# GlaireDaggers/Pretty-Fast-Video

Measured on AMD Instinct MI355X. Metric: macroblocks/s (encode+decode) 1080p YUV420, higher is better.
Workload: dtype i32 (encoder transforms evaluated in exact f32; decoders i32)

## Files before the change

include/pfv_hip_ext.h:

```cpp
#ifndef PFV_HIP_EXT_H
#define PFV_HIP_EXT_H

#include "pfv_hip_core.h"

#ifdef __cplusplus
extern "C" {
#endif

PFV_API int pfv_ctx_create_prio(int device, int priority, pfv_ctx **out);
PFV_API int pfv_ctx_pci_bus_id(pfv_ctx *ctx, char *out, int len);
PFV_API int pfv_device_sync(pfv_ctx *ctx);
PFV_API void *pfv_ctx_stream(pfv_ctx *ctx);

typedef enum pfv_option {
    PFV_OPT_ENC_TRANSFORM = 1, PFV_OPT_TILE_COMPACTION = 2, PFV_OPT_LANE_MAPPING = 3, PFV_OPT_ENTROPY_DECODE = 4,
    PFV_OPT_ENTDEC_LANE_BITS = 5, PFV_OPT_ENTDEC_LAUNCHES = 6, PFV_OPT_ENTDEC_INNER_ROUNDS = 7
} pfv_option;
enum { PFV_ENTROPY_DECODE_AUTO = 0, PFV_ENTROPY_DECODE_HOST = 1, PFV_ENTROPY_DECODE_DEVICE = 2 };
enum { PFV_LANES_AUTO = 0, PFV_LANES_PER_MB_8 = 1, PFV_LANES_PER_MB_16 = 2 };
enum { PFV_ENC_TRANSFORM_AUTO = 0, PFV_ENC_TRANSFORM_INT = 1 };
PFV_API int pfv_ctx_set_option(pfv_ctx *ctx, int option, int value);
PFV_API int pfv_ctx_get_option(pfv_ctx *ctx, int option, int *value);

typedef struct pfv_event pfv_event;
PFV_API int pfv_event_create(pfv_ctx *ctx, pfv_event **out);
PFV_API int pfv_event_record(pfv_event *e);
PFV_API int pfv_event_elapsed_ms(pfv_event *start, pfv_event *stop, float *ms);
PFV_API void pfv_event_destroy(pfv_event *e);
PFV_API int pfv_ctx_wait_event(pfv_ctx *ctx, pfv_event *e);

typedef struct pfv_graph pfv_graph;
PFV_API int pfv_graph_begin(pfv_ctx *ctx);
PFV_API int pfv_graph_end(pfv_ctx *ctx, pfv_graph **out);
PFV_API int pfv_graph_launch(pfv_graph *g);
PFV_API void pfv_graph_destroy(pfv_graph *g);

PFV_API int pfv_blit_dev(pfv_ctx *ctx, uint8_t *dst, int dst_w, int dst_h, const uint8_t *src, int src_w, int src_h,
                         int dx, int dy, int sx, int sy, int sw, int sh);

PFV_API int pfv_reduce_dev(pfv_ctx *ctx, uint8_t *dst, const uint8_t *src, int src_w, int src_h);
PFV_API int pfv_double_dev(pfv_ctx *ctx, uint8_t *dst, const uint8_t *src, int src_w, int src_h);
PFV_API int pfv_rgb_to_yuv420_dev(pfv_ctx *ctx, const uint8_t *rgb_dev, int width, int height, uint8_t *frame_dev);
PFV_API int pfv_yuv420_to_rgb_dev(pfv_ctx *ctx, const uint8_t *frame_dev, int width, int height, uint8_t *rgb_dev);

typedef struct pfv_comm pfv_comm;
enum { PFV_COMM_SUM = 0, PFV_COMM_MAX = 1 };
PFV_API int pfv_comm_unique_id(uint8_t id_out[128]);
PFV_API int pfv_comm_init(pfv_ctx *ctx, int rank, int world, const uint8_t id[128], pfv_comm **out);
PFV_API int pfv_comm_rank(const pfv_comm *c);
PFV_API int pfv_comm_world(const pfv_comm *c);
PFV_API int pfv_comm_broadcast_dev(pfv_comm *c, void *buf_dev, size_t bytes, int root);
PFV_API int pfv_comm_allreduce_f64_dev(pfv_comm *c, double *buf_dev, size_t count, int op);
PFV_API int pfv_comm_allgather_dev(pfv_comm *c, const void *send_dev, void *recv_dev, size_t bytes_per_rank);
PFV_API int pfv_comm_allreduce_f64(pfv_comm *c, double *values, size_t count, int op);
PFV_API int pfv_comm_barrier(pfv_comm *c);
PFV_API void pfv_comm_destroy(pfv_comm *c);

PFV_API int pfv_synth_frames_dev(pfv_ctx *ctx, int width, int height, int n_streams, const uint64_t *seeds, int t,
                                 uint8_t *frames_dev);
enum { PFV_SYNTH_PAN = 0, PFV_SYNTH_LOW_MOTION = 1, PFV_SYNTH_STATIC = 2 };
PFV_API int pfv_synth_frames_kind_dev(pfv_ctx *ctx, int width, int height, int n_streams, const uint64_t *seeds, int t, int kind,
                                      uint8_t *frames_dev);

PFV_API int pfv_dev_alloc(pfv_ctx *ctx, size_t bytes, void **out);
PFV_API int pfv_dev_free(pfv_ctx *ctx, void *p);
PFV_API int pfv_dev_copy(pfv_ctx *ctx, void *dst_dev, const void *src_dev, size_t bytes);
PFV_API int pfv_host_alloc(pfv_ctx *ctx, size_t bytes, void **out);
PFV_API int pfv_host_free(pfv_ctx *ctx, void *p);
PFV_API int pfv_dev_upload(pfv_ctx *ctx, void *dst_dev, const void *src_host, size_t bytes);
PFV_API int pfv_dev_download(pfv_ctx *ctx, void *dst_host, const void *src_dev, size_t bytes);

PFV_API int pfv_enc_iframe_dev(pfv_enc_session *s, const uint8_t *frames_dev, int16_t *coef_dev);
PFV_API int pfv_enc_pframe_dev(pfv_enc_session *s, const uint8_t *frames_dev, int8_t *mv_dev, uint8_t *has_coef_dev,
                               int16_t *coef_dev);
PFV_API int pfv_enc_session_set_frame_stride(pfv_enc_session *s, size_t stride_bytes);
PFV_API int pfv_enc_session_set_window(pfv_enc_session *s, int first, int count);
PFV_API const uint8_t *pfv_enc_prev_frame_dev(pfv_enc_session *s, int stream);

PFV_API size_t pfv_payload_worst_case(int width, int height);
PFV_API int pfv_enc_entropy_enable(pfv_enc_session *s, size_t payload_cap);
PFV_API int pfv_enc_entropy_set_async(pfv_enc_session *s, int on);
PFV_API int pfv_enc_entropy_join(pfv_enc_session *s);
PFV_API int pfv_enc_pack_iframe_dev(pfv_enc_session *s, const int16_t *coef_dev);
PFV_API int pfv_enc_pack_pframe_dev(pfv_enc_session *s, const int8_t *mv_dev, const uint8_t *has_coef_dev,
                                    const int16_t *coef_dev);
PFV_API int pfv_enc_payload_sizes(pfv_enc_session *s, uint32_t *sizes_out);
PFV_API int pfv_enc_payloads_fetch(pfv_enc_session *s, uint8_t *out, size_t cap, uint32_t *sizes_out, uint64_t *offsets_out);
PFV_API const uint8_t *pfv_enc_payload_dev(pfv_enc_session *s, int stream);
PFV_API size_t pfv_enc_payload_capacity(pfv_enc_session *s);
PFV_API int pfv_enc_payload_fetch(pfv_enc_session *s, int stream, uint8_t *out_host, size_t nbytes);
PFV_API int pfv_dec_iframe_dev(pfv_dec_session *s, const int16_t *coef_dev, const uint8_t qidx[3]);
PFV_API int pfv_dec_pframe_dev(pfv_dec_session *s, const int8_t *mv_dev, const uint8_t *has_coef_dev,
                               const int16_t *coef_dev, const uint8_t qidx[3]);
PFV_API int pfv_dec_iframe_sparse(pfv_dec_session *s, const uint32_t *idx, const int16_t *val, size_t n, const uint8_t qidx[3]);
PFV_API int pfv_dec_pframe_sparse(pfv_dec_session *s, const int8_t *mv, const uint8_t *has_coef, const uint32_t *idx,
                                  const int16_t *val, size_t n, const uint8_t qidx[3]);
PFV_API int pfv_dec_iframe_lists_dev(pfv_dec_session *s, const uint32_t *const *entries_dev, const uint32_t *counts_dev, const uint8_t qidx[3]);
PFV_API int pfv_dec_pframe_lists_dev(pfv_dec_session *s, const int8_t *mv_dev, const uint8_t *has_coef_dev, const uint32_t *const *entries_dev,
                                     const uint32_t *counts_dev, const uint8_t qidx[3]);
PFV_API int pfv_coef_lists_from_dense(const int16_t *coef, const uint8_t *has_coef, int total_blocks, uint32_t *entries_out, size_t cap,
                                      uint32_t *counts_out, size_t *n_out);
PFV_API int pfv_dec_get_frame_dev(pfv_dec_session *s, uint8_t *frames_out_dev);
PFV_API int pfv_dec_set_output_dev(pfv_dec_session *s, uint8_t *frames_out_dev);
PFV_API int pfv_dec_set_output_strided_dev(pfv_dec_session *s, uint8_t *frames_out_dev, size_t stride_bytes);
PFV_API int pfv_dec_session_set_window(pfv_dec_session *s, int first, int count);
PFV_API int pfv_encoder_set_device_entropy(pfv_encoder *e, int on);
enum { PFV_FRAME_PACKED = 0, PFV_FRAME_PADDED = 1 };
PFV_API int pfv_frames_sse_dev(pfv_ctx *ctx, int width, int height, int n_streams, const uint8_t *a_dev, int a_layout, size_t a_stride,
                               const uint8_t *b_dev, int b_layout, size_t b_stride, uint64_t *sse_dev, uint32_t *mb_sse_dev);
PFV_API int pfv_frames_sse(pfv_ctx *ctx, int width, int height, int n_streams, const uint8_t *a, const uint8_t *b, uint64_t *sse_out,
                           uint32_t *mb_sse_out);
PFV_API double pfv_psnr(uint64_t sse, uint64_t n_samples);
PFV_API int pfv_enc_distortion_dev(pfv_enc_session *s, const uint8_t *frames_dev, uint64_t *sse_dev, uint32_t *mb_sse_dev);
PFV_API int pfv_dec_distortion_dev(pfv_dec_session *s, const uint8_t *frames_dev, uint64_t *sse_dev, uint32_t *mb_sse_dev);
typedef struct pfv_frame_report {
    int32_t  type;
    uint32_t packet_bytes;
    uint64_t sse[3];
    double   psnr[3];
    double   psnr_yuv;
} pfv_frame_report;
PFV_API int pfv_encoder_set_frame_report(pfv_encoder *e, int on);
PFV_API int pfv_encoder_frame_report(pfv_encoder *e, pfv_frame_report *out);

PFV_API int pfv_frames_ssim_dev(pfv_ctx *ctx, int width, int height, int n_streams, const uint8_t *a_dev, int a_layout, size_t a_stride,
                                const uint8_t *b_dev, int b_layout, size_t b_stride, int64_t *ssim_q24_dev, int32_t *mb_ssim_q24_dev);
PFV_API int pfv_frames_ssim(pfv_ctx *ctx, int width, int height, int n_streams, const uint8_t *a, const uint8_t *b, int64_t *ssim_q24_out,
                            int32_t *mb_out);
PFV_API int pfv_ssim_windows(int width, int height, uint32_t out[3]);
PFV_API double pfv_ssim(int64_t q24_sum, uint64_t windows);
PFV_API int pfv_enc_ssim_dev(pfv_enc_session *s, const uint8_t *frames_dev, int64_t *ssim_q24_dev, int32_t *mb_dev);
PFV_API int pfv_dec_ssim_dev(pfv_dec_session *s, const uint8_t *frames_dev, int64_t *ssim_q24_dev, int32_t *mb_dev);
typedef struct pfv_frame_ssim {
    int64_t  q24[3];
    uint32_t windows[3];
    double   ssim[3];
    double   ssim_all;
} pfv_frame_ssim;
PFV_API int pfv_encoder_set_frame_ssim(pfv_encoder *e, int on);
PFV_API int pfv_encoder_frame_ssim(pfv_encoder *e, pfv_frame_ssim *out);

PFV_API int pfv_deblock_strength(const int32_t qtable[64]);
PFV_API int pfv_frames_deblock_dev(pfv_ctx *ctx, int width, int height, int n_streams, const uint8_t *src_dev, int src_layout, size_t src_stride,
                                   uint8_t *dst_dev, size_t dst_stride, const uint8_t strength[3]);
PFV_API int pfv_frames_deblock(pfv_ctx *ctx, int width, int height, int n_streams, const uint8_t *src, uint8_t *dst, const uint8_t strength[3]);
enum { PFV_DEBLOCK_OFF = 0, PFV_DEBLOCK_AUTO = 1, PFV_DEBLOCK_FIXED = 2 };
PFV_API int pfv_dec_set_deblock(pfv_dec_session *s, int mode, const uint8_t strength[3]);
PFV_API int pfv_decoder_set_deblock(pfv_decoder *d, int mode, const uint8_t strength[3]);

enum { PFV_PIX_RGB8 = 0, PFV_PIX_RGBA8 = 1, PFV_PIX_BGRA8 = 2 };
PFV_API size_t pfv_rgb_row_bytes(int width, int format);
PFV_API int pfv_frames_to_rgb_dev(pfv_ctx *ctx, int width, int height, int n_streams, const uint8_t *src_dev, int src_layout, size_t src_stride,
                                  uint8_t *dst_dev, int format, size_t dst_pitch, size_t dst_stride);
PFV_API int pfv_frames_to_rgb(pfv_ctx *ctx, int width, int height, int n_streams, const uint8_t *src, uint8_t *dst, int format);
PFV_API int pfv_dec_get_frame_rgb_dev(pfv_dec_session *s, uint8_t *dst_dev, int format, size_t pitch, size_t stride);
PFV_API int pfv_dec_get_frame_rgb(pfv_dec_session *s, uint8_t *dst_host, int format);
PFV_API int pfv_dec_set_output_rgb_dev(pfv_dec_session *s, uint8_t *dst_dev, int format, size_t pitch, size_t stride);
PFV_API int pfv_decoder_set_output_rgb(pfv_decoder *d, int on, int format);

enum { PFV_CHROMA_POINT = 0, PFV_CHROMA_BOX = 1 };
PFV_API int pfv_frames_from_rgb_dev(pfv_ctx *ctx, int width, int height, int n_streams, const uint8_t *src_dev, int format, size_t src_pitch,
                                    size_t src_stride, uint8_t *dst_dev, size_t dst_stride, int chroma);
PFV_API int pfv_frames_from_rgb(pfv_ctx *ctx, int width, int height, int n_streams, const uint8_t *src, uint8_t *dst, int format, int chroma);
PFV_API int pfv_enc_ingest_rgb_dev(pfv_enc_session *s, const uint8_t *pictures_dev, int format, size_t pitch, size_t stride, int chroma,
                                   const uint8_t **frames_dev_out);
PFV_API int pfv_encoder_set_input_rgb(pfv_encoder *e, int on, int format, int chroma);

enum { PFV_SCALE_BILINEAR = 0, PFV_SCALE_BICUBIC = 1, PFV_SCALE_LANCZOS3 = 2 };
typedef struct pfv_scaler pfv_scaler;
PFV_API int pfv_scale_taps(int kind, int n_src, int n_dst);
PFV_API int pfv_scale_table(int kind, int n_src, int n_dst, int32_t *first, int16_t *coef);
PFV_API pfv_scaler *pfv_scaler_create(pfv_ctx *ctx, int sw, int sh, int dw, int dh, int kind, int *err);
PFV_API void pfv_scaler_destroy(pfv_scaler *sc);
PFV_API int pfv_scaler_run_dev(pfv_scaler *sc, int n_streams, const uint8_t *src_dev, int src_layout, size_t src_stride, uint8_t *dst_dev,
                               size_t dst_stride);
PFV_API int pfv_frames_scale(pfv_ctx *ctx, int sw, int sh, int dw, int dh, int n_streams, const uint8_t *src, uint8_t *dst, int kind);
PFV_API int pfv_dec_set_output_scaled_dev(pfv_dec_session *s, pfv_scaler *sc, uint8_t *dst_dev, size_t stride);
PFV_API int pfv_decoder_set_output_size(pfv_decoder *d, int w, int h, int kind);
PFV_API int pfv_enc_scale_dev(pfv_enc_session *s, pfv_scaler *sc, const uint8_t *frames_dev, size_t src_stride, const uint8_t **frames_dev_out);
PFV_API int pfv_encoder_set_input_size(pfv_encoder *e, int src_w, int src_h, int kind);

typedef struct pfv_denoiser pfv_denoiser;
PFV_API pfv_denoiser *pfv_denoiser_create(pfv_ctx *ctx, int width, int height, int n_streams, int *err);
PFV_API void pfv_denoiser_destroy(pfv_denoiser *dn);
PFV_API int pfv_denoiser_set_strength(pfv_denoiser *dn, const uint8_t spatial[3], const uint8_t temporal[3]);
PFV_API int pfv_denoiser_reset(pfv_denoiser *dn, int first_stream, int n);
PFV_API int pfv_denoiser_run_dev(pfv_denoiser *dn, int first_stream, int n, const uint8_t *src_dev, int src_layout, size_t src_stride, uint8_t *dst_dev,
                                 size_t dst_stride, int commit);
// ... 160 lines not shown
```

pretty-fast-video_amd/_lib.py:

```python
from __future__ import annotations

import ctypes
import os
from ctypes import POINTER, c_char_p, c_float, c_int, c_size_t, c_uint8, c_void_p

_HERE = os.path.dirname(os.path.abspath(__file__))
DEFAULT_LIB = os.path.join(_HERE, "libpfv_hip.so")

PFV_OK = 0
PFV_ERR_BAD_ARG = -1
PFV_ERR_HIP = -2
PFV_ERR_NOMEM = -3
PFV_ERR_BAD_MV = -4
PFV_ERR_NO_DEVICE = -5
PFV_ERR_FORMAT = -6
PFV_ERR_VERSION = -7
PFV_ERR_IO = -8
PFV_ERR_STATE = -9

PFV_COMM_SUM, PFV_COMM_MAX = 0, 1
PFV_OPT_ENC_TRANSFORM = 1
PFV_OPT_TILE_COMPACTION = 2
PFV_OPT_LANE_MAPPING = 3
PFV_LANES_AUTO, PFV_LANES_PER_MB_8, PFV_LANES_PER_MB_16 = 0, 1, 2
PFV_OPT_ENTROPY_DECODE = 4
PFV_OPT_ENTDEC_LANE_BITS, PFV_OPT_ENTDEC_LAUNCHES, PFV_OPT_ENTDEC_INNER_ROUNDS = 5, 6, 7
PFV_ENTROPY_DECODE_AUTO, PFV_ENTROPY_DECODE_HOST, PFV_ENTROPY_DECODE_DEVICE = 0, 1, 2
PFV_ENC_TRANSFORM_AUTO, PFV_ENC_TRANSFORM_INT = 0, 1
PFV_FRAME_PACKED, PFV_FRAME_PADDED = 0, 1
PFV_DEBLOCK_OFF, PFV_DEBLOCK_AUTO, PFV_DEBLOCK_FIXED = 0, 1, 2
PFV_PIX_RGB8, PFV_PIX_RGBA8, PFV_PIX_BGRA8 = 0, 1, 2
PFV_CHROMA_POINT, PFV_CHROMA_BOX = 0, 1
PFV_SCALE_BILINEAR, PFV_SCALE_BICUBIC, PFV_SCALE_LANCZOS3 = 0, 1, 2
PFV_SEARCH_FOURSTEP, PFV_SEARCH_FULL, PFV_SEARCH_HIER = 0, 1, 2


SEARCH_MODES = {"fourstep": PFV_SEARCH_FOURSTEP, "full": PFV_SEARCH_FULL, "hier": PFV_SEARCH_HIER}


def search_mode(mode) -> int:
    return SEARCH_MODES[mode] if isinstance(mode, str) else int(mode)


class PfvError(RuntimeError):
    def __init__(self, code: int, msg: str):
        super().__init__(f"pfv_hip error {code}: {msg}")
        self.code = code


_P = c_void_p
SIGNATURES = [
    ("pfv_device_count", c_int, []),
    ("pfv_ctx_create", c_int, [c_int, POINTER(_P)]),
    ("pfv_ctx_create_prio", c_int, [c_int, c_int, POINTER(_P)]),
    ("pfv_ctx_destroy", None, [_P]),
    ("pfv_ctx_pci_bus_id", c_int, [_P, _P, c_int]),
    ("pfv_ctx_sync", c_int, [_P]),
    ("pfv_device_sync", c_int, [_P]),
    ("pfv_ctx_stream", _P, [_P]),
    ("pfv_last_error", c_char_p, [_P]),
    ("pfv_version", c_char_p, []),
    ("pfv_ctx_set_option", c_int, [_P, c_int, c_int]),
    ("pfv_ctx_get_option", c_int, [_P, c_int, POINTER(c_int)]),
    ("pfv_event_create", c_int, [_P, POINTER(_P)]),
    ("pfv_event_record", c_int, [_P]),
    ("pfv_event_elapsed_ms", c_int, [_P, _P, POINTER(c_float)]),
    ("pfv_event_destroy", None, [_P]),
    ("pfv_ctx_wait_event", c_int, [_P, _P]),
    ("pfv_graph_begin", c_int, [_P]),
    ("pfv_graph_end", c_int, [_P, POINTER(_P)]),
    ("pfv_graph_launch", c_int, [_P]),
    ("pfv_graph_destroy", None, [_P]),
    ("pfv_pad16", c_int, [c_int]),
    ("pfv_qtables_from_quality", c_int, [c_int, _P, _P, _P, _P, POINTER(c_float)]),
    ("pfv_encode_plane", c_int, [_P, _P, c_int, c_int, _P, c_uint8, _P]),
    ("pfv_encode_plane_delta", c_int, [_P, _P, c_int, c_int, _P, _P, c_float, c_uint8, _P, _P, _P]),
    ("pfv_decode_plane_into", c_int, [_P, _P, c_int, c_int, _P, _P]),
    ("pfv_decode_plane_delta", c_int, [_P, _P, _P, _P, c_int, c_int, _P, _P, _P]),
    ("pfv_decode_plane_delta_into", c_int, [_P, _P, _P, _P, c_int, c_int, _P, _P]),
    ("pfv_blit_dev", c_int, [_P, _P, c_int, c_int, _P, c_int, c_int, c_int, c_int, c_int, c_int, c_int, c_int]),
    ("pfv_reduce_dev", c_int, [_P, _P, _P, c_int, c_int]),
    ("pfv_double_dev", c_int, [_P, _P, _P, c_int, c_int]),
    ("pfv_rgb_to_yuv420_dev", c_int, [_P, _P, c_int, c_int, _P]),
    ("pfv_yuv420_to_rgb_dev", c_int, [_P, _P, c_int, c_int, _P]),
    ("pfv_comm_unique_id", c_int, [_P]),
    ("pfv_comm_init", c_int, [_P, c_int, c_int, _P, POINTER(_P)]),
    ("pfv_comm_rank", c_int, [_P]),
    ("pfv_comm_world", c_int, [_P]),
    ("pfv_comm_broadcast_dev", c_int, [_P, _P, c_size_t, c_int]),
    ("pfv_comm_allreduce_f64_dev", c_int, [_P, _P, c_size_t, c_int]),
    ("pfv_comm_allgather_dev", c_int, [_P, _P, _P, c_size_t]),
    ("pfv_comm_allreduce_f64", c_int, [_P, _P, c_size_t, c_int]),
    ("pfv_comm_barrier", c_int, [_P]),
    ("pfv_comm_destroy", None, [_P]),
    ("pfv_synth_frames_dev", c_int, [_P, c_int, c_int, c_int, _P, c_int, _P]),
    ("pfv_synth_frames_kind_dev", c_int, [_P, c_int, c_int, c_int, _P, c_int, c_int, _P]),
    ("pfv_dev_alloc", c_int, [_P, c_size_t, POINTER(_P)]),
    ("pfv_dev_copy", c_int, [_P, _P, _P, c_size_t]),
    ("pfv_dev_free", c_int, [_P, _P]),
    ("pfv_host_alloc", c_int, [_P, c_size_t, POINTER(_P)]),
    ("pfv_host_free", c_int, [_P, _P]),
    ("pfv_dev_upload", c_int, [_P, _P, _P, c_size_t]),
    ("pfv_dev_download", c_int, [_P, _P, _P, c_size_t]),
    ("pfv_frame_bytes", c_size_t, [c_int, c_int]),
    ("pfv_padded_frame_bytes", c_size_t, [c_int, c_int]),
    ("pfv_total_blocks", c_int, [c_int, c_int]),
    ("pfv_enc_session_create", c_int, [_P, c_int, c_int, c_int, c_int, POINTER(_P)]),
    ("pfv_enc_session_destroy", None, [_P]),
    ("pfv_enc_iframe_dev", c_int, [_P, _P, _P]),
    ("pfv_enc_pframe_dev", c_int, [_P, _P, _P, _P, _P]),
    ("pfv_enc_iframe", c_int, [_P, _P, _P]),
    ("pfv_enc_pframe", c_int, [_P, _P, _P, _P, _P]),
    ("pfv_enc_session_set_frame_stride", c_int, [_P, c_size_t]),
    ("pfv_enc_session_set_window", c_int, [_P, c_int, c_int]),
    ("pfv_enc_prev_frame_dev", _P, [_P, c_int]),
    ("pfv_enc_prev_frame", c_int, [_P, _P]),
    ("pfv_payload_worst_case", c_size_t, [c_int, c_int]),
    ("pfv_enc_entropy_enable", c_int, [_P, c_size_t]),
    ("pfv_enc_entropy_set_async", c_int, [_P, c_int]),
    ("pfv_enc_entropy_join", c_int, [_P]),
    ("pfv_enc_pack_iframe_dev", c_int, [_P, _P]),
    ("pfv_enc_pack_pframe_dev", c_int, [_P, _P, _P, _P]),
    ("pfv_enc_payload_sizes", c_int, [_P, _P]),
    ("pfv_enc_payloads_fetch", c_int, [_P, _P, c_size_t, _P, _P]),
    ("pfv_enc_payload_dev", _P, [_P, c_int]),
    ("pfv_enc_payload_capacity", c_size_t, [_P]),
    ("pfv_enc_payload_fetch", c_int, [_P, c_int, _P, c_size_t]),
    ("pfv_dec_iframe_sparse", c_int, [_P, _P, _P, c_size_t, _P]),
    ("pfv_dec_pframe_sparse", c_int, [_P, _P, _P, _P, _P, c_size_t, _P]),
    ("pfv_dec_iframe_lists_dev", c_int, [_P, _P, _P, _P]),
    ("pfv_dec_pframe_lists_dev", c_int, [_P, _P, _P, _P, _P, _P]),
    ("pfv_coef_lists_from_dense", c_int, [_P, _P, c_int, _P, c_size_t, _P, POINTER(c_size_t)]),
    ("pfv_dec_session_create", c_int, [_P, c_int, c_int, _P, c_int, c_int, POINTER(_P)]),
    ("pfv_dec_session_destroy", None, [_P]),
    ("pfv_dec_iframe_dev", c_int, [_P, _P, _P]),
    ("pfv_dec_pframe_dev", c_int, [_P, _P, _P, _P, _P]),
    ("pfv_dec_iframe", c_int, [_P, _P, _P]),
    ("pfv_dec_pframe", c_int, [_P, _P, _P, _P, _P]),
    ("pfv_dec_get_frame_dev", c_int, [_P, _P]),
    ("pfv_dec_set_output_dev", c_int, [_P, _P]),
    ("pfv_dec_set_output_strided_dev", c_int, [_P, _P, c_size_t]),
    ("pfv_dec_session_set_window", c_int, [_P, c_int, c_int]),
    ("pfv_dec_get_frame", c_int, [_P, _P]),
    ("pfv_dec_framebuffer", c_int, [_P, _P]),
    ("pfv_dec_check", c_int, [_P]),
    ("pfv_encoder_create", c_int, [_P, c_int, c_int, c_int, c_int, POINTER(_P)]),
    ("pfv_encoder_encode_iframe", c_int, [_P, _P, _P, _P]),
    ("pfv_encoder_encode_pframe", c_int, [_P, _P, _P, _P]),
    ("pfv_encoder_encode_dropframe", c_int, [_P]),
    ("pfv_encoder_finish", c_int, [_P]),
    ("pfv_encoder_bytes", c_int, [_P, POINTER(_P), POINTER(c_size_t)]),
    ("pfv_encoder_drain", c_int, [_P, POINTER(_P), POINTER(c_size_t)]),
    ("pfv_encoder_destroy", None, [_P]),
    ("pfv_encoder_set_device_entropy", c_int, [_P, c_int]),
    ("pfv_frames_sse_dev", c_int, [_P, c_int, c_int, c_int, _P, c_int, c_size_t, _P, c_int, c_size_t, _P, _P]),
    ("pfv_frames_sse", c_int, [_P, c_int, c_int, c_int, _P, _P, _P, _P]),
    ("pfv_psnr", ctypes.c_double, [ctypes.c_uint64, ctypes.c_uint64]),
    ("pfv_enc_distortion_dev", c_int, [_P, _P, _P, _P]),
    ("pfv_dec_distortion_dev", c_int, [_P, _P, _P, _P]),
    ("pfv_encoder_set_frame_report", c_int, [_P, c_int]),
    ("pfv_encoder_frame_report", c_int, [_P, _P]),
    ("pfv_frames_ssim_dev", c_int, [_P, c_int, c_int, c_int, _P, c_int, c_size_t, _P, c_int, c_size_t, _P, _P]),
    ("pfv_frames_ssim", c_int, [_P, c_int, c_int, c_int, _P, _P, _P, _P]),
    ("pfv_ssim_windows", c_int, [c_int, c_int, _P]),
    ("pfv_ssim", ctypes.c_double, [ctypes.c_int64, ctypes.c_uint64]),
    ("pfv_enc_ssim_dev", c_int, [_P, _P, _P, _P]),
    ("pfv_dec_ssim_dev", c_int, [_P, _P, _P, _P]),
    ("pfv_encoder_set_frame_ssim", c_int, [_P, c_int]),
    ("pfv_encoder_frame_ssim", c_int, [_P, _P]),
    ("pfv_deblock_strength", c_int, [_P]),
    ("pfv_frames_deblock_dev", c_int, [_P, c_int, c_int, c_int, _P, c_int, c_size_t, _P, c_size_t, _P]),
    ("pfv_frames_deblock", c_int, [_P, c_int, c_int, c_int, _P, _P, _P]),
    ("pfv_dec_set_deblock", c_int, [_P, c_int, _P]),
    ("pfv_decoder_set_deblock", c_int, [_P, c_int, _P]),
    ("pfv_rgb_row_bytes", c_size_t, [c_int, c_int]),
    ("pfv_frames_to_rgb_dev", c_int, [_P, c_int, c_int, c_int, _P, c_int, c_size_t, _P, c_int, c_size_t, c_size_t]),
    ("pfv_frames_to_rgb", c_int, [_P, c_int, c_int, c_int, _P, _P, c_int]),
    ("pfv_dec_get_frame_rgb_dev", c_int, [_P, _P, c_int, c_size_t, c_size_t]),
    ("pfv_dec_get_frame_rgb", c_int, [_P, _P, c_int]),
    ("pfv_dec_set_output_rgb_dev", c_int, [_P, _P, c_int, c_size_t, c_size_t]),
    ("pfv_decoder_set_output_rgb", c_int, [_P, c_int, c_int]),
    ("pfv_frames_from_rgb_dev", c_int, [_P, c_int, c_int, c_int, _P, c_int, c_size_t, c_size_t, _P, c_size_t, c_int]),
    ("pfv_frames_from_rgb", c_int, [_P, c_int, c_int, c_int, _P, _P, c_int, c_int]),
    ("pfv_enc_ingest_rgb_dev", c_int, [_P, _P, c_int, c_size_t, c_size_t, c_int, _P]),
    ("pfv_encoder_set_input_rgb", c_int, [_P, c_int, c_int, c_int]),
    ("pfv_scale_taps", c_int, [c_int, c_int, c_int]),
    ("pfv_scale_table", c_int, [c_int, c_int, c_int, _P, _P]),
    ("pfv_scaler_create", _P, [_P, c_int, c_int, c_int, c_int, c_int, POINTER(c_int)]),
    ("pfv_scaler_destroy", None, [_P]),
    ("pfv_scaler_run_dev", c_int, [_P, c_int, _P, c_int, c_size_t, _P, c_size_t]),
    ("pfv_frames_scale", c_int, [_P, c_int, c_int, c_int, c_int, c_int, _P, _P, c_int]),
    ("pfv_dec_set_output_scaled_dev", c_int, [_P, _P, _P, c_size_t]),
    ("pfv_decoder_set_output_size", c_int, [_P, c_int, c_int, c_int]),
    ("pfv_enc_scale_dev", c_int, [_P, _P, _P, c_size_t, _P]),
    ("pfv_encoder_set_input_size", c_int, [_P, c_int, c_int, c_int]),
    ("pfv_denoiser_create", _P, [_P, c_int, c_int, c_int, POINTER(c_int)]),
    ("pfv_denoiser_destroy", None, [_P]),
    ("pfv_denoiser_set_strength", c_int, [_P, _P, _P]),
    ("pfv_denoiser_reset", c_int, [_P, c_int, c_int]),
    ("pfv_denoiser_run_dev", c_int, [_P, c_int, c_int, _P, c_int, c_size_t, _P, c_size_t, c_int]),
    ("pfv_frames_denoise", c_int, [_P, c_int, c_int, c_int, c_int, _P, _P, _P, _P]),
    ("pfv_enc_denoise_dev", c_int, [_P, _P, _P, c_size_t, c_int, _P]),
    ("pfv_encoder_set_denoise", c_int, [_P, c_int, _P, _P]),
    ("pfv_scene_score_q8", ctypes.c_uint32, [_P]),
    ("pfv_scene_plan", c_int, [_P, c_int, ctypes.c_uint32, c_int, c_int, _P]),
    ("pfv_scene_detector_create", _P, [_P, c_int, c_int, c_int, c_int, POINTER(c_int)]),
    ("pfv_scene_detector_destroy", None, [_P]),
    ("pfv_scene_detector_set_radius", c_int, [_P, c_int]),
    ("pfv_scene_detector_reset", c_int, [_P, c_int, c_int]),
    ("pfv_scene_detector_run_dev", c_int, [_P, c_int, c_int, _P, c_int, c_size_t, c_int, _P]),
    ("pfv_scene_detector_run_clip_dev", c_int, [_P, c_int, c_int, _P, c_int, c_size_t, c_int, _P]),
    ("pfv_scene_detector_maps", c_int, [_P, c_int, c_int, _P, _P]),
    ("pfv_scene_detector_run_timed_dev", c_int, [_P, c_int, c_int, c_int, _P, c_int, c_size_t, _P, _P]),
    ("pfv_frames_scene", c_int, [_P, c_int, c_int, c_int, c_int, _P, c_int, _P]),
    ("pfv_encoder_set_scene_cut", c_int, [_P, c_int, ctypes.c_uint32, c_int, c_int]),
    ("pfv_encoder_last_scene", c_int, [_P, _P]),
    ("pfv_enc_session_create_ladder", c_int, [_P, c_int, c_int, _P, c_int, c_int, POINTER(_P)]),
    ("pfv_enc_session_set_motion_search", c_int, [_P, c_int, c_int]),
    ("pfv_enc_session_get_motion_search", c_int, [_P, _P, _P]),
    ("pfv_encoder_set_motion_search", c_int, [_P, c_int, c_int]),
    ("pfv_enc_session_coarse_vectors", c_int, [_P, _P, c_size_t]),
    ("pfv_enc_pframe_hier_timed_dev", c_int, [_P, _P, _P, _P, _P, _P]),
    ("pfv_enc_session_set_rung", c_int, [_P, c_int]),
    ("pfv_enc_session_rung", c_int, [_P]),
    ("pfv_enc_session_rungs", c_int, [_P]),
# ... 121 lines not shown
```

pretty-fast-video_amd/csrc/pfv_context.hip:

```cpp
constexpr int kCtxScratch = 9;
struct pfv_ctx {
    int device = 0;
    hipStream_t stream = nullptr;
    std::string err;
    void *scratch[kCtxScratch] = {};
    size_t scratch_cap[kCtxScratch] = {};
    QTab *qtab_dev = nullptr;
    QTab *qtab_host = nullptr;
    int *flag_dev = nullptr;
    int n_cus = 256;
    bool capturing = false;
    int opt_enc_transform = PFV_ENC_TRANSFORM_AUTO;
    int opt_tile_compaction = 1;
    int opt_lane_mapping = PFV_LANES_AUTO;
    int opt_entropy_decode = PFV_ENTROPY_DECODE_AUTO;
    int opt_entdec_lane_bits = (int)kEdSubBits, opt_entdec_launches = 3, opt_entdec_inner = kEdInner;
    std::vector<struct pfv_comm *> comms;
    std::mutex comms_m;
    pfv_ctx *owner = nullptr;
    std::vector<pfv_ctx *> children;
    int priority = 0;
};
static int ctx_create_child(pfv_ctx *user, pfv_ctx **out)
{
    int rc = pfv_ctx_create_prio(user->device, user->priority, out);
    if (rc) return rc;
    (*out)->owner = user;
    std::lock_guard<std::mutex> lk(user->comms_m);
    user->children.push_back(*out);
    return PFV_OK;
}
static void comm_teardown(struct pfv_comm *c);

static thread_local std::string g_tls_err;

static int fail(pfv_ctx *ctx, int code, const std::string &msg)
{
    if (ctx) ctx->err = msg;
    if (ctx && ctx->owner) ctx->owner->err = msg;
    g_tls_err = msg;
    return code;
}
static int hip_fail(pfv_ctx *ctx, hipError_t e, const char *what)
{
    (void)hipGetLastError();
    return fail(ctx, e == hipErrorOutOfMemory ? PFV_ERR_NOMEM : PFV_ERR_HIP,
                std::string(what) + ": " + hipGetErrorString(e));
}
#define HIP_TRY(ctx, expr)                                        \
    do {                                                          \
        hipError_t e__ = (expr);                                  \
        if (e__ != hipSuccess) return hip_fail(ctx, e__, #expr);  \
    } while (0)

static inline int pad16(int x) { return x + (16 - (x % 16)) % 16; }

extern "C" {

#ifndef PFV_BUILD_ID
#define PFV_BUILD_ID "unstamped"
#endif
PFV_API const char *pfv_version(void) { return "pfv-hip 0.2 (gfx950; pfv-rs 0.2.2 / codec 2.1.1 hot path; src " PFV_BUILD_ID ")"; }
PFV_API int pfv_pad16(int x) { return pad16(x); }

PFV_API const char *pfv_last_error(pfv_ctx *ctx) { return ctx ? ctx->err.c_str() : g_tls_err.c_str(); }

PFV_API int pfv_ctx_set_option(pfv_ctx *ctx, int option, int value)
{
    if (!ctx) return fail(nullptr, PFV_ERR_BAD_ARG, "null ctx");
    switch (option) {
    case PFV_OPT_ENC_TRANSFORM:
        if (value != PFV_ENC_TRANSFORM_AUTO && value != PFV_ENC_TRANSFORM_INT) return fail(ctx, PFV_ERR_BAD_ARG, "PFV_OPT_ENC_TRANSFORM: unknown value");
        ctx->opt_enc_transform = value;
        return PFV_OK;
    case PFV_OPT_TILE_COMPACTION:
        if (value < 0 || value > 2) return fail(ctx, PFV_ERR_BAD_ARG, "PFV_OPT_TILE_COMPACTION: 0, 1 or 2");
        ctx->opt_tile_compaction = value;
        return PFV_OK;
    case PFV_OPT_LANE_MAPPING:
        if (value != PFV_LANES_AUTO && value != PFV_LANES_PER_MB_8 && value != PFV_LANES_PER_MB_16) return fail(ctx, PFV_ERR_BAD_ARG, "PFV_OPT_LANE_MAPPING: unknown value");
        ctx->opt_lane_mapping = value;
        return PFV_OK;
    case PFV_OPT_ENTROPY_DECODE:
        if (value != PFV_ENTROPY_DECODE_AUTO && value != PFV_ENTROPY_DECODE_HOST && value != PFV_ENTROPY_DECODE_DEVICE) return fail(ctx, PFV_ERR_BAD_ARG, "PFV_OPT_ENTROPY_DECODE: unknown value");
        ctx->opt_entropy_decode = value;
        return PFV_OK;
    case PFV_OPT_ENTDEC_LANE_BITS:
        if (value < 32 || value > (int)kEdMaxSubBits || value % 32) return fail(ctx, PFV_ERR_BAD_ARG, "PFV_OPT_ENTDEC_LANE_BITS: a multiple of 32 in 32..256");
        ctx->opt_entdec_lane_bits = value;
        return PFV_OK;
    case PFV_OPT_ENTDEC_LAUNCHES:
        if (value < 1 || value > 64) return fail(ctx, PFV_ERR_BAD_ARG, "PFV_OPT_ENTDEC_LAUNCHES: 1..64");
        ctx->opt_entdec_launches = value;
        return PFV_OK;
    case PFV_OPT_ENTDEC_INNER_ROUNDS:
        if (value < 1 || value > 1024) return fail(ctx, PFV_ERR_BAD_ARG, "PFV_OPT_ENTDEC_INNER_ROUNDS: 1..1024");
        ctx->opt_entdec_inner = value;
        return PFV_OK;
    default:
        return fail(ctx, PFV_ERR_BAD_ARG, "pfv_ctx_set_option: unknown option");
    }
}
PFV_API int pfv_ctx_get_option(pfv_ctx *ctx, int option, int *value)
{
    if (!ctx || !value) return fail(ctx, PFV_ERR_BAD_ARG, "pfv_ctx_get_option: bad argument");
    switch (option) {
    case PFV_OPT_ENC_TRANSFORM: *value = ctx->opt_enc_transform; return PFV_OK;
    case PFV_OPT_TILE_COMPACTION: *value = ctx->opt_tile_compaction; return PFV_OK;
    case PFV_OPT_LANE_MAPPING: *value = ctx->opt_lane_mapping; return PFV_OK;
    case PFV_OPT_ENTROPY_DECODE: *value = ctx->opt_entropy_decode; return PFV_OK;
    case PFV_OPT_ENTDEC_LANE_BITS: *value = ctx->opt_entdec_lane_bits; return PFV_OK;
    case PFV_OPT_ENTDEC_LAUNCHES: *value = ctx->opt_entdec_launches; return PFV_OK;
    case PFV_OPT_ENTDEC_INNER_ROUNDS: *value = ctx->opt_entdec_inner; return PFV_OK;
    default: return fail(ctx, PFV_ERR_BAD_ARG, "pfv_ctx_get_option: unknown option");
    }
}

PFV_API int pfv_device_count(void)
{
    int n = 0;
    if (hipGetDeviceCount(&n) != hipSuccess) { (void)hipGetLastError(); return 0; }
    return n;
}

PFV_API int pfv_ctx_create(int device, pfv_ctx **out) { return pfv_ctx_create_prio(device, 0, out); }

PFV_API int pfv_ctx_create_prio(int device, int priority, pfv_ctx **out)
{
    if (!out) return fail(nullptr, PFV_ERR_BAD_ARG, "pfv_ctx_create: out is null");
    *out = nullptr;
    int n = 0;
    hipError_t e = hipGetDeviceCount(&n);
    if (e != hipSuccess || n <= 0) {
        (void)hipGetLastError();
        return fail(nullptr, PFV_ERR_NO_DEVICE, "pfv_ctx_create: no HIP device visible (the HIP path has no CPU fallback)");
    }
    if (device < 0 || device >= n) return fail(nullptr, PFV_ERR_BAD_ARG, "pfv_ctx_create: device ordinal out of range");
    HIP_TRY(nullptr, hipSetDevice(device));
    pfv_ctx *ctx = new pfv_ctx();
    ctx->device = device;
    ctx->priority = priority;
    {
        int cus = 0;
        if (hipDeviceGetAttribute(&cus, hipDeviceAttributeMultiprocessorCount, device) == hipSuccess && cus > 0) ctx->n_cus = cus;
    }
    if (priority == 0) {
        e = hipStreamCreateWithFlags(&ctx->stream, hipStreamNonBlocking);
    } else {
        int least = 0, greatest = 0;
        e = hipDeviceGetStreamPriorityRange(&least, &greatest);
        if (e == hipSuccess) e = hipStreamCreateWithPriority(&ctx->stream, hipStreamNonBlocking, priority > 0 ? greatest : least);
    }
    if (e == hipSuccess) e = hipMalloc((void **)&ctx->qtab_dev, 4 * sizeof(QTab));
    if (e == hipSuccess) e = hipHostMalloc((void **)&ctx->qtab_host, 4 * sizeof(QTab), hipHostMallocDefault);
    if (e == hipSuccess) e = hipMalloc((void **)&ctx->flag_dev, sizeof(int));
    if (e == hipSuccess) e = hipMemsetAsync(ctx->flag_dev, 0, sizeof(int), ctx->stream);
    if (e != hipSuccess) {
        int rc = hip_fail(nullptr, e, "pfv_ctx_create");
        pfv_ctx_destroy(ctx);
        return rc;
    }
    *out = ctx;
    return PFV_OK;
}

PFV_API void pfv_ctx_destroy(pfv_ctx *ctx)
{
    if (!ctx) return;
    (void)hipSetDevice(ctx->device);
    if (ctx->stream) (void)hipStreamSynchronize(ctx->stream);
    {
        std::vector<pfv_comm *> live;
        { std::lock_guard<std::mutex> lk(ctx->comms_m); live.swap(ctx->comms); }
        for (pfv_comm *c : live) comm_teardown(c);
    }
    {
        std::lock_guard<std::mutex> lk(ctx->comms_m);
        for (pfv_ctx *c : ctx->children) c->owner = nullptr;
        ctx->children.clear();
    }
    if (ctx->owner) {
        std::lock_guard<std::mutex> lk(ctx->owner->comms_m);
        auto &v = ctx->owner->children;
        v.erase(std::remove(v.begin(), v.end(), ctx), v.end());
    }
    for (int i = 0; i < kCtxScratch; i++)
        if (ctx->scratch[i]) (void)hipFree(ctx->scratch[i]);
    if (ctx->qtab_dev) (void)hipFree(ctx->qtab_dev);
    if (ctx->qtab_host) (void)hipHostFree(ctx->qtab_host);
    if (ctx->flag_dev) (void)hipFree(ctx->flag_dev);
// ... 136 lines not shown
```

pretty-fast-video_amd/csrc/pfv_kernels.hip:

```cpp
#include <hip/hip_runtime.h>
#include <stdint.h>

#include "pfv_device.h"
#include "pfv_prof.h"


namespace pfv {

namespace {
__constant__ int kScale[64] = {
    32, 37, 34, 26, 32, 26, 34, 37, 37, 43, 39, 31, 37, 31, 39, 43, 34, 39, 35, 28, 34, 28, 35, 39, 26, 31, 28, 22, 26, 22,
    28, 31, 32, 37, 34, 26, 32, 26, 34, 37, 26, 31, 28, 22, 26, 22, 28, 31, 34, 39, 35, 28, 34, 28, 35, 39, 37, 43, 39, 31,
    37, 31, 39, 43,
};
__constant__ int kInvZigzag[64] = {
    0,  1,  5,  6,  14, 15, 27, 28, 2,  4,  7,  13, 16, 26, 29, 42, 3,  8,  12, 17, 25, 30, 41, 43, 9,  11, 18, 24, 31, 40,
    44, 53, 10, 19, 23, 32, 39, 45, 52, 54, 20, 22, 33, 38, 46, 51, 55, 60, 21, 34, 37, 47, 50, 56, 59, 61, 35, 36, 48, 49,
    57, 58, 62, 63,
};
}

constexpr int kWinRows = 16 * kStripsPerWG + 30;
constexpr int kWinStride = 176;
constexpr int kWinBytes = kWinRows * kWinStride;
// ... 306 lines not shown
        int ch = j * 64 + lane;
        int mb = half_strip * 4 + (ch >> 5);
        if (mb < n_mb) st_stream(&reinterpret_cast<uint4 *>(coef_mb0)[half_strip * 128 + ch], reinterpret_cast<const uint4 *>(stage)[stage_chunk(ch)]);
    }
}
__device__ __forceinline__ void fetch_coef_quads(uint4 (&buf)[2], const int16_t *coef_mb0, int n_mb, int lane, int half_strip)
{
#pragma unroll
    for (int j = 0; j < 2; j++) {
        int ch = j * 64 + lane;
        int mb = half_strip * 4 + (ch >> 5);
        buf[j] = make_uint4(0, 0, 0, 0);
        if (mb < n_mb) buf[j] = ld_stream(&reinterpret_cast<const uint4 *>(coef_mb0)[half_strip * 128 + ch]);
    }
}
__device__ __forceinline__ void stage_coef_half(int *stage, const uint4 (&buf)[2], int lane)
{
#pragma unroll
    for (int j = 0; j < 2; j++) reinterpret_cast<uint4 *>(stage)[stage_chunk(j * 64 + lane)] = buf[j];
}

struct ListSpan {
    const uint32_t *ent;
    uint32_t lo, hi;
    uint32_t e0, e1;
};
__device__ __forceinline__ ListSpan list_span(const uint32_t *ent, uint32_t begin, uint32_t end, int last_lane, int lane)
{
    ListSpan sp{ent, 0u, 0u, 0u, 0u};
    sp.lo = (uint32_t)__builtin_amdgcn_readlane((int)begin, 0);
    sp.hi = (uint32_t)__builtin_amdgcn_readlane((int)end, last_lane);
    if (sp.hi < sp.lo) sp.hi = sp.lo;
    const uint32_t k = sp.lo + (uint32_t)lane;
    if (k < sp.hi) sp.e0 = ent[k];
    if (k + 64u < sp.hi) sp.e1 = ent[k + 64u];
    return sp;
}
template <int LPM>
__device__ __forceinline__ void stage_list_put(int16_t *stage, uint32_t e, int mb_low, int h)
{
    const int pos = (int)(e & 255u), mbl = (int)(((e >> 8) - (uint32_t)mb_low) & 255u);
    if (LPM == 8) {
        if ((pos >> 7) == h && mbl < kStripMB) stage[mbl * (2 * kStagePitch) + (pos & 127)] = (int16_t)(e >> 16);
    } else {
        if (mbl < kStripMB / 2) stage[(mbl * 2 + (pos >> 7)) * (2 * kStagePitch) + (pos & 127)] = (int16_t)(e >> 16);
    }
}
template <int LPM>
__device__ __forceinline__ void stage_list_half(int *xw, const ListSpan &sp, int lane, int mb_low, int h)
{
#pragma unroll
    for (int j = 0; j < 2; j++) reinterpret_cast<uint4 *>(xw)[stage_chunk(j * 64 + lane)] = make_uint4(0, 0, 0, 0);
    wave_lds_sync();
    int16_t *stage = reinterpret_cast<int16_t *>(xw);
    const uint32_t k = sp.lo + (uint32_t)lane;
    if (k < sp.hi) stage_list_put<LPM>(stage, sp.e0, mb_low, h);
    if (k + 64u < sp.hi) stage_list_put<LPM>(stage, sp.e1, mb_low, h);
    for (uint32_t j = k + 128u; j < sp.hi; j += 64u) stage_list_put<LPM>(stage, sp.ent[j], mb_low, h);
}

__device__ __forceinline__ void forward_half(int (&v)[2][8], int *xw, int m, int i, const LaneQ &lq, bool keep)
{
    const int keepmask = keep ? -1 : 0;
    int *mb = xw + m * kMBPitch;
    fdct8(v[0]);
    fdct8(v[1]);
    rows_to_cols2(v, mb, i, m & 3);
    fdct8(v[0]);
    fdct8(v[1]);
    int16_t *stage = reinterpret_cast<int16_t *>(xw) + m * (2 * kStagePitch);
#pragma unroll
    for (int k = 0; k < 8; k++) {
        const int scale = lq.scale(k), zz = lq.zz(k);
        const float rcp = lq.rcp(k);
#pragma unroll
        for (int s = 0; s < 2; s++) {
            int n = wmul24(v[s][k], scale) >> 16;
            v[s][k] = (int)((float)n * rcp) & keepmask;
            stage[s * 64 + zz] = (int16_t)v[s][k];
        }
    }
    wave_lds_sync();
}
__device__ __forceinline__ void inverse_half(int (&v)[2][8], int *xw, int m, int i, const LaneQ &lq)
{
    int *mb = xw + m * kMBPitch;
#pragma unroll
    for (int k = 0; k < 8; k++) {
        const int deq = lq.deq(k);
        v[0][k] = wmul24(v[0][k], deq);
        v[1][k] = wmul24(v[1][k], deq);
    }
    idct8(v[0]);
    idct8(v[1]);
    cols_to_rows2(v, mb, i, m & 3);
#pragma unroll
    for (int s = 0; s < 2; s++) {
        idct8(v[s]);
#pragma unroll
        for (int k = 0; k < 8; k++) v[s][k] = min(v[s][k] >> 8, 127);
    }
}
__device__ __forceinline__ void gather_half(int (&v)[2][8], const int *xw, int m, const LaneQ &lq)
{
    const int16_t *stage = reinterpret_cast<const int16_t *>(xw) + m * (2 * kStagePitch);
#pragma unroll
    for (int k = 0; k < 8; k++) {
        const int zz = lq.zz(k);
        v[0][k] = (int)stage[zz];
        v[1][k] = (int)stage[64 + zz];
    }
    wave_lds_sync();
}

typedef float f2 __attribute__((vector_size(8)));
__device__ __forceinline__ f2 f2s(float x) { return f2{x, x}; }
__device__ __forceinline__ f2 f2trunc(f2 x) { return f2{__builtin_truncf(x[0]), __builtin_truncf(x[1])}; }
__device__ __forceinline__ f2 f2floor(f2 x) { return f2{__builtin_floorf(x[0]), __builtin_floorf(x[1])}; }

__device__ __forceinline__ void ffdct8(f2 (&v)[8])
{
    const f2 a0 = v[0] + v[7], a1 = v[1] + v[6], a2 = v[2] + v[5], a3 = v[3] + v[4];
    const f2 a4 = v[0] - v[7], a5 = v[1] - v[6], a6 = v[2] - v[5], a7 = v[3] - v[4];
    const f2 b0 = a0 + a3, b1 = a1 + a2, b2 = a0 - a3, b3 = a1 - a2;
    const f2 c0 = b0 + b1, c1 = b0 - b1;
    const f2 c2 = b2 * f2s(1.25f) + b3 * f2s(0.5f);
    const f2 c3 = b2 * f2s(0.5f) - b3 * f2s(1.25f);
    const f2 b4 = a4 * f2s(1.1875f) + a7 * f2s(0.25f);
    const f2 b7 = a4 * f2s(0.25f) - a7 * f2s(1.1875f);
    const f2 b5 = a5 + a6 * f2s(0.6875f);
    const f2 b6 = a6 - a5 * f2s(0.6875f);
    const f2 c4 = b4 + b5, c5 = b4 - b5, c6 = b6 + b7, c7 = b6 - b7;
    v[0] = c0; v[1] = c4; v[2] = c2; v[3] = c5 - c7;
    v[4] = c1; v[5] = c5 + c7; v[6] = c3; v[7] = c6;
}
__device__ __forceinline__ void fidct8(f2 (&v)[8])
{
    const f2 c0 = v[0], d4 = v[1], c2 = v[2], d6 = v[3], c1 = v[4], d5 = v[5], c3 = v[6], d7 = v[7];
    const f2 c5 = d5 + d6, c7 = d5 - d6;
    const f2 b4 = d4 + c5, b5 = d4 - c5, b6 = d7 + c7, b7 = d7 - c7;
    const f2 b0 = c0 + c1, b1 = c0 - c1;
    const f2 half = f2s(0.5f), quarter = f2s(0.25f);
    const f2 c2h = f2trunc(c2 * half), c2q = f2trunc(c2h * half), c3h = f2trunc(c3 * half), c3q = f2trunc(c3h * half);
    const f2 b4q = f2trunc(b4 * quarter), b4s = f2trunc(b4q * quarter), b5q = f2trunc(b5 * quarter), b5s = f2trunc(b5q * quarter);
    const f2 b6q = f2trunc(b6 * quarter), b6s = f2trunc(b6q * quarter), b7q = f2trunc(b7 * quarter), b7s = f2trunc(b7q * quarter);
    const f2 b2 = c2 + c2q + c3h, b3 = c2h - c3 - c3q;
    const f2 a4 = b7q + b4 + b4q - b4s;
    const f2 a7 = b4q - b7 - b7q + b7s;
    const f2 a5 = b5 - b6 + b6q + b6s;
    const f2 a6 = b6 + b5 - b5q - b5s;
    const f2 a0 = b0 + b2, a1 = b1 + b3, a2 = b1 - b3, a3 = b0 - b2;
    v[0] = a0 + a4; v[1] = a1 + a5; v[2] = a2 + a6; v[3] = a3 + a7;
    v[4] = a3 - a7; v[5] = a2 - a6; v[6] = a1 - a5; v[7] = a0 - a4;
}
__device__ __forceinline__ int f_chunk(int p, int j) { return j ^ ((p >> 1) & 3); }
__device__ __forceinline__ void f_rows_to_cols(f2 (&x)[8], int *mb, int i, int mx)
{
    {
        const int p = i ^ mx;
        float4 *row = reinterpret_cast<float4 *>(mb + p * 16);
#pragma unroll
        for (int j = 0; j < 4; j++) row[f_chunk(p, j)] = make_float4(x[2 * j][0], x[2 * j][1], x[2 * j + 1][0], x[2 * j + 1][1]);
    }
    wave_lds_sync();
#pragma unroll
    for (int r = 0; r < 8; r++) {
        const int p = r ^ mx;
        x[r] = *reinterpret_cast<const f2 *>(mb + p * 16 + f_chunk(p, i >> 1) * 4 + (i & 1) * 2);
    }
    wave_lds_sync();
}
__device__ __forceinline__ void f_cols_to_rows(f2 (&x)[8], int *mb, int i, int mx)
{
#pragma unroll
    for (int r = 0; r < 8; r++) {
        const int p = r ^ mx;
        *reinterpret_cast<f2 *>(mb + p * 16 + f_chunk(p, i >> 1) * 4 + (i & 1) * 2) = x[r];
    }
    wave_lds_sync();
    {
        const int p = i ^ mx;
        const float4 *row = reinterpret_cast<const float4 *>(mb + p * 16);
#pragma unroll
        for (int j = 0; j < 4; j++) {
            const float4 c = row[f_chunk(p, j)];
            x[2 * j] = f2{c.x, c.y};
            x[2 * j + 1] = f2{c.z, c.w};
        }
    }
    wave_lds_sync();
}
__device__ __forceinline__ f2 quant_scale(f2 m, int scale16)
{
    f2 n;
#pragma unroll
    for (int s = 0; s < 2; s++) n[s] = (float)mulhi24((int)m[s], scale16);
    return n;
}
constexpr float kQuantMagic = 12582912.0f;
__device__ __forceinline__ f2 quant_div(f2 n, float rcp, float magic, f2 &biased)
{
    const f2 q = f2trunc(n * f2s(rcp));
    biased = q + f2s(magic);
    return q;
}
__device__ __forceinline__ f2 quant_pair_f(f2 m, int scale16, float rcp, float magic, f2 &biased)
{
    return quant_div(quant_scale(m, scale16), rcp, magic, biased);
}
__device__ __forceinline__ f2 residual_f(f2 src, f2 pred)
{
    const f2 d = src - pred;
    const float c = 0.5f - 1.0f / 2048.0f;
    const f2 r = f2{__builtin_fmaf(d[0], c, kQuantMagic), __builtin_fmaf(d[1], c, kQuantMagic)};
    return f2{__builtin_fmaf(r[0], 256.0f, -256.0f * kQuantMagic), __builtin_fmaf(r[1], 256.0f, -256.0f * kQuantMagic)};
}
__device__ __forceinline__ int16_t quant_low16(float biased) { return (int16_t)__float_as_int(biased); }
__device__ __forceinline__ void forward_half_f(f2 (&x)[8], int *xw, int m, int i, const LaneQ &lq, float magic)
{
    int *mb = xw + m * kMBPitch;
    ffdct8(x);
    f_rows_to_cols(x, mb, i, m & 3);
    ffdct8(x);
    int16_t *stage = reinterpret_cast<int16_t *>(xw) + m * (2 * kStagePitch);
#pragma unroll
    for (int k = 0; k < 8; k++) {
        const int zz = lq.zz(k);
        f2 biased;
        x[k] = quant_pair_f(x[k], lq.scale(k), lq.rcp(k), magic, biased);
#pragma unroll
        for (int s = 0; s < 2; s++) stage[s * 64 + zz] = quant_low16(biased[s]);
    }
    wave_lds_sync();
}
constexpr float kPixelBias = 127.501953125f;
__device__ __forceinline__ f2 iframe_pixel_f(f2 x) { return x * f2s(1.0f / 256.0f) + f2s(kPixelBias); }
template <bool PIXEL>
__device__ __forceinline__ void inverse_half_f(f2 (&c)[8], int *xw, int m, int i, const LaneQ &lq)
{
    int *mb = xw + m * kMBPitch;
#pragma unroll
    for (int k = 0; k < 8; k++) c[k] = c[k] * f2s(lq.deqf(k));
    fidct8(c);
    f_cols_to_rows(c, mb, i, m & 3);
    fidct8(c);
#pragma unroll
    for (int k = 0; k < 8; k++) c[k] = PIXEL ? iframe_pixel_f(c[k]) : f2floor(c[k] * f2s(1.0f / 256.0f));
}
__device__ __forceinline__ uint4 pack_row_f(const f2 (&px)[8])
{
    unsigned w[4] = {0, 0, 0, 0};
#pragma unroll
    for (int k = 0; k < 8; k++) {
        w[k >> 2] = __builtin_amdgcn_cvt_pk_u8_f32(px[k][0], (unsigned)(k & 3), w[k >> 2]);
        w[2 + (k >> 2)] = __builtin_amdgcn_cvt_pk_u8_f32(px[k][1], (unsigned)(k & 3), w[2 + (k >> 2)]);
    }
    return make_uint4(w[0], w[1], w[2], w[3]);
}
__device__ __forceinline__ void unpack_row_f(const uint4 &row, f2 (&px)[8])
{
#pragma unroll
    for (int k = 0; k < 4; k++) {
        px[k] = f2{(float)byte_of(row.x, k), (float)byte_of(row.z, k)};
        px[k + 4] = f2{(float)byte_of(row.y, k), (float)byte_of(row.w, k)};
    }
}

template <bool FLT, int LPM = 8>
__global__ __launch_bounds__(kThreads) void k_enc_iframe(FrameGeom g, const uint8_t *__restrict__ src,
                                                          int16_t *__restrict__ coef, uint8_t *__restrict__ recon,
                                                          const QTab *__restrict__ qtabs, float qmagic)
{
    __shared__ __attribute__((aligned(16))) int xchg[kStripsPerWG][kXchgDwords];
    __shared__ __attribute__((aligned(16))) int qtab_lds[kStripsPerWG][kQTabDwords];
    constexpr int kPasses = LPM == 8 ? 2 : 1;

    const int lane = threadIdx.x & 63, wave = __builtin_amdgcn_readfirstlane((int)(threadIdx.x >> 6));
    const int gw = xcd_remap((int)blockIdx.x, (int)gridDim.x) * kStripsPerWG + wave;
    const int gstrip = LPM == 8 ? gw : gw >> 1, half_strip = LPM == 8 ? 0 : gw & 1;
    if (gstrip >= g.strips_per_frame * g.n_streams) return;
    const StripPos sp = locate_strip(g, gstrip);
    if (half_strip * 4 >= sp.n_mb) return;
    const PlaneGeom &p = g.p[sp.plane];
    const int slot = lane >> 3, i = lane & 7;
    const int m = LPM == 8 ? slot : half_strip * 4 + (slot >> 1);
    int *xw = xchg[wave];

    fill_qtable<true, FLT>(qtab_lds[wave], qtabs + p.qsel, lane);
    const uint8_t *plane = frame_src(g, src, sp.stream) + p.src_off;
    uint4 rows[kPasses];
#pragma unroll
    for (int pass = 0; pass < kPasses; pass++) rows[pass] = load_src16(plane, p, sp.x0 + m * 16, sp.y0 + i + 8 * (LPM == 8 ? pass : (slot & 1)));

    wave_lds_sync();
    const LaneQ lq{qtab_lds[wave], i};
    int16_t *coef_mb0 = coef + ((long)sp.stream * g.mbs_per_frame + sp.mb_first) * 256;
    uint8_t *dst = recon ? recon + (long)sp.stream * g.pad_frame_bytes + p.pad_off + (long)(sp.y0 + i) * p.pw + sp.x0 + m * 16
                         : nullptr;
#pragma unroll
    for (int pass = 0; pass < kPasses; pass++) {
        const int h = LPM == 8 ? pass : (slot & 1);
        if (FLT) {
            f2 x[8];
            unpack_row_f(rows[pass], x);
#pragma unroll
            for (int k = 0; k < 8; k++) x[k] = x[k] * f2s(256.0f) - f2s(32768.0f);
            forward_half_f(x, xw, slot, i, lq, qmagic);
            if (LPM == 8) store_coef_half(xw, coef_mb0, sp.n_mb, lane, h);
            else store_coef_quads(xw, coef_mb0, sp.n_mb, lane, half_strip);
            wave_lds_sync();
            if (recon) {
                inverse_half_f<true>(x, xw, slot, i, lq);
                if (m < sp.n_mb) *reinterpret_cast<uint4 *>(dst + (long)(8 * h) * p.pw) = pack_row_f(x);
            }
        } else {
            int v[2][8];
            unpack_row(rows[pass], v);
#pragma unroll
            for (int s = 0; s < 2; s++) {
#pragma unroll
                for (int k = 0; k < 8; k++) v[s][k] = (int)((unsigned)(v[s][k] - 128) << 8);
            }
            forward_half(v, xw, slot, i, lq, true);
            if (LPM == 8) store_coef_half(xw, coef_mb0, sp.n_mb, lane, h);
            else store_coef_quads(xw, coef_mb0, sp.n_mb, lane, half_strip);
            wave_lds_sync();
            if (recon) {
                inverse_half(v, xw, slot, i, lq);
#pragma unroll
                for (int s = 0; s < 2; s++)
#pragma unroll
                    for (int k = 0; k < 8; k++) v[s][k] = min(max(v[s][k] + 128, 0), 255);
                if (m < sp.n_mb) *reinterpret_cast<uint4 *>(dst + (long)(8 * h) * p.pw) = pack_row(v);
            }
        }
    }
}

struct SearchState {
    int cx, cy;
    int err;
};

__device__ __forceinline__ unsigned dot_ab(const uint4 &a, unsigned b0, unsigned b1, unsigned b2, unsigned b3, unsigned acc)
{
    acc = __builtin_amdgcn_udot4(a.x, b0, acc, false);
    acc = __builtin_amdgcn_udot4(a.y, b1, acc, false);
    acc = __builtin_amdgcn_udot4(a.z, b2, acc, false);
// ... 228 lines not shown
                                             int lane)
{
    const int q0 = win_first_issue(wave), q1 = win_first_issue(wave + 1);
#pragma unroll 5
    for (int q = q0; q < q1; q++) {
        const int c = q * 64 + lane;
        const int row = c / kWinChunksPerRow, col = c - row * kWinChunksPerRow;
        const int y = min(max(t.winy0 + row, 0), p.ph - 1), x = min(max(t.winx0 + col * 16, 0), p.pw - 16);
        __builtin_amdgcn_global_load_lds((gbl_cvoid_t *)(refp + (long)y * p.pw + x), (lds_void_t *)(winbuf + c * 16), 16, 0, 0);
    }
}

struct SearchOut {
    int cx, cy;
    int err;
    bool coded;
    uint4 patch[2];
};

template <bool DPPRED = false>
__device__ __forceinline__ void penc_search(const FrameGeom &g, const TilePos &tp, const uint8_t *win, int *red, const uint4 (&rows)[2], int lane,
                                            float min_err, int neg2, SearchOut &so)
{
    const StripPos &sp = tp.sp;
    const PlaneGeom &p = g.p[sp.plane];
    const int m = lane >> 3, i = lane & 7;
    const bool mb_valid = m < sp.n_mb;
    const int mbx = sp.x0 + m * 16, mby = sp.y0;
    const int wcol0 = mbx - tp.winx0;
    const int wrow0 = mby - tp.winy0 + i;

    unsigned s2 = 0;
#pragma unroll
    for (int h = 0; h < 2; h++) {
        s2 = __builtin_amdgcn_udot4(rows[h].x, rows[h].x, s2, false);
        s2 = __builtin_amdgcn_udot4(rows[h].y, rows[h].y, s2, false);
        s2 = __builtin_amdgcn_udot4(rows[h].z, rows[h].z, s2, false);
        s2 = __builtin_amdgcn_udot4(rows[h].w, rows[h].w, s2, false);
    }
    const int a2 = mb_sum((int)s2);

    SearchState st;
    st.cx = 0; st.cy = 0; st.err = 0;
    const SearchLane sl = make_search_lane(red, m, i, neg2);
    const bool interior = sp.x0 >= 16 && sp.x0 + kStripMB * 16 + 16 <= p.pw && sp.y0 >= 16 && sp.y0 + 32 <= p.ph;
    if (interior) {
        search_level<8, true, false, DPPRED>(win, wrow0, wcol0, rows[0], rows[1], a2, mbx, mby, p.pw, p.ph, st, sl);
        KMARK(3);
        search_level<4, false, false, DPPRED>(win, wrow0, wcol0, rows[0], rows[1], a2, mbx, mby, p.pw, p.ph, st, sl);
        KMARK(4);
        search_level<2, false, false, DPPRED>(win, wrow0, wcol0, rows[0], rows[1], a2, mbx, mby, p.pw, p.ph, st, sl);
        KMARK(5);
        search_level<1, false, false, DPPRED>(win, wrow0, wcol0, rows[0], rows[1], a2, mbx, mby, p.pw, p.ph, st, sl);
        KMARK(6);
    } else {
        search_level<8, true, true, DPPRED>(win, wrow0, wcol0, rows[0], rows[1], a2, mbx, mby, p.pw, p.ph, st, sl);
        search_level<4, false, true, DPPRED>(win, wrow0, wcol0, rows[0], rows[1], a2, mbx, mby, p.pw, p.ph, st, sl);
        search_level<2, false, true, DPPRED>(win, wrow0, wcol0, rows[0], rows[1], a2, mbx, mby, p.pw, p.ph, st, sl);
        search_level<1, false, true, DPPRED>(win, wrow0, wcol0, rows[0], rows[1], a2, mbx, mby, p.pw, p.ph, st, sl);
    }

    so.coded = mb_valid && !((float)st.err <= min_err);
    so.cx = st.cx; so.cy = st.cy;
    so.err = st.err;

    const int wx = wcol0 + st.cx, shp = wx & 3;
    const uint8_t *rp = win + (wrow0 + st.cy) * kWinStride + (wx & ~3);
#pragma unroll
    for (int h = 0; h < 2; h++) {
        const unsigned *d = reinterpret_cast<const unsigned *>(rp + 8 * h * kWinStride);
        unsigned d0 = d[0], d1 = d[1], d2 = d[2], d3 = d[3], d4 = d[4];
        so.patch[h] = make_uint4(__builtin_amdgcn_alignbyte(d1, d0, shp), __builtin_amdgcn_alignbyte(d2, d1, shp),
                                 __builtin_amdgcn_alignbyte(d3, d2, shp), __builtin_amdgcn_alignbyte(d4, d3, shp));
    }
}

__device__ __forceinline__ void opaque_row(uint4 &r)
{
#ifndef PFV_HIPEMU
    asm volatile("" : "+v"(r.x), "+v"(r.y), "+v"(r.z), "+v"(r.w));
#else
    (void)r;
#endif
}
template <bool FLT, bool REUNPACK = false, class Store>
__device__ __forceinline__ uint4 penc_half(const uint4 &srow, const uint4 &prow, int *xw, int m, int i, const LaneQ &lq, float qmagic, bool want_recon,
                                           Store &&store)
{
    uint4 out = prow;
    if (FLT) {
        f2 x[8], pp[8];
        unpack_row_f(srow, x);
        unpack_row_f(prow, pp);
#pragma unroll
        for (int k = 0; k < 8; k++) x[k] = residual_f(x[k], pp[k]);
        forward_half_f(x, xw, m, i, lq, qmagic);
        store();
        wave_lds_sync();
        if (want_recon) {
            inverse_half_f<false>(x, xw, m, i, lq);
            if (REUNPACK) {
                uint4 again = prow;
                opaque_row(again);
                unpack_row_f(again, pp);
            }
#pragma unroll
            for (int k = 0; k < 8; k++) {
                const f2 t = f2{__builtin_fminf(x[k][0], 127.0f), __builtin_fminf(x[k][1], 127.0f)};
                pp[k] = pp[k] + t * f2s(2.0f);
            }
            out = pack_row_f(pp);
        }
    } else {
        int v[2][8], pp[2][8];
        unpack_row(srow, v);
        unpack_row(prow, pp);
#pragma unroll
        for (int s = 0; s < 2; s++) {
#pragma unroll
            for (int k = 0; k < 8; k++) {
                int d = v[s][k] - pp[s][k];
                v[s][k] = (int)((unsigned)tdiv2(d) << 8);
            }
        }
        forward_half(v, xw, m, i, lq, true);
        store();
        wave_lds_sync();
        if (want_recon) {
            inverse_half(v, xw, m, i, lq);
#pragma unroll
            for (int s = 0; s < 2; s++) {
#pragma unroll
                for (int k = 0; k < 8; k++)
                    pp[s][k] = min(max(pp[s][k] + 2 * v[s][k], 0), 255);
            }
            out = pack_row(pp);
        }
    }
    return out;
}

__device__ __forceinline__ void penc_store_skipped(int16_t *coef_mb, uint8_t *dst, long pw, int i, const uint4 (&patch)[2])
{
#pragma unroll
    for (int j = 0; j < 4; j++) st_stream(&reinterpret_cast<uint4 *>(coef_mb)[j * 8 + i], make_uint4(0, 0, 0, 0));
    if (dst) {
        *reinterpret_cast<uint4 *>(dst) = patch[0];
        *reinterpret_cast<uint4 *>(dst + 8 * pw) = patch[1];
    }
}

template <bool FLT>
__device__ __forceinline__ void penc_transform(const FrameGeom &g, const TilePos &tp, const SearchOut &so, const uint4 (&rows)[2], int *xw,
                                               int lane, int16_t *__restrict__ coef, uint8_t *__restrict__ recon, const int *qtab_lds, float qmagic)
{
    const StripPos &sp = tp.sp;
    const PlaneGeom &p = g.p[sp.plane];
    const int m = lane >> 3, i = lane & 7;
    const bool mb_valid = m < sp.n_mb, coded = so.coded;
    const int mbx = sp.x0 + m * 16;
    int16_t *coef_mb0 = coef + ((long)sp.stream * g.mbs_per_frame + sp.mb_first) * 256;
    uint8_t *dst = recon ? recon + (long)sp.stream * g.pad_frame_bytes + p.pad_off + (long)(sp.y0 + i) * p.pw + mbx : nullptr;

    if (__any(coded)) {
        const LaneQ lq{qtab_lds, i};
#pragma unroll
// ... 411 lines not shown
    __shared__ __attribute__((aligned(16))) uint8_t win_lds[16 + kWinAlloc];
    __shared__ __attribute__((aligned(16))) int red_lds[kWaves16][kRedDwords];
    __shared__ __attribute__((aligned(16))) int qtab_lds[kQTabDwords];
    uint8_t *win = win_lds + 16;

    const int lane = threadIdx.x & 63, wave = __builtin_amdgcn_readfirstlane((int)(threadIdx.x >> 6));
    const int strip = wave >> 1, half_strip = wave & 1;
    const int slot = lane >> 3, i = lane & 7, mb = lane >> 4, r = lane & 15;
    const int m = half_strip * 4 + mb;
    const int vt = xcd_remap((int)blockIdx.x, (int)gridDim.x);
    const TilePos cur = locate_tile(g, vt, strip);
    const PlaneGeom &p = g.p[cur.sp.plane];
    if (wave == 0) fill_qtable<true, FLT>(qtab_lds, qtabs + p.qsel, lane);
    {
        const uint8_t *refp = ref + (long)cur.sp.stream * g.pad_frame_bytes + p.pad_off;
        for (int q = win_first_issue16(wave); q < win_first_issue16(wave + 1); q++) {
            const int c = q * 64 + lane;
            const int row = c / kWinChunksPerRow, col = c - row * kWinChunksPerRow;
            const int y = min(max(cur.winy0 + row, 0), p.ph - 1), x = min(max(cur.winx0 + col * 16, 0), p.pw - 16);
            __builtin_amdgcn_global_load_lds((gbl_cvoid_t *)(refp + (long)y * p.pw + x), (lds_void_t *)(win + c * 16), 16, 0, 0);
        }
    }
    const bool wave_valid = cur.wave_valid && half_strip * 4 < cur.sp.n_mb;
    const bool mb_valid = wave_valid && m < cur.sp.n_mb;
    uint4 row = make_uint4(0, 0, 0, 0);
    if (wave_valid) row = load_src16(frame_src(g, src, cur.sp.stream) + p.src_off, p, cur.sp.x0 + m * 16, cur.sp.y0 + r);
    __syncthreads();
    int cx = 0, cy = 0;
    bool coded = false;
    uint4 patch = make_uint4(0, 0, 0, 0);
    if (wave_valid) {
        const int mbx = cur.sp.x0 + m * 16, mby = cur.sp.y0;
        const int wcol0 = mbx - cur.winx0, wrow0 = mby - cur.winy0 + r;
        unsigned s2 = __builtin_amdgcn_udot4(row.w, row.w, __builtin_amdgcn_udot4(row.z, row.z, __builtin_amdgcn_udot4(row.y, row.y, __builtin_amdgcn_udot4(row.x, row.x, 0, false), false), false), false);
        const int a2 = mb_sum16((int)s2);
        SearchState st;
        st.cx = 0; st.cy = 0; st.err = 0;
        const SearchLane16 sl = make_search_lane16(red_lds[wave], mb, r, neg2);
        const int hx0 = cur.sp.x0 + half_strip * 64;
        const bool interior = hx0 >= 16 && hx0 + 64 + 16 <= p.pw && cur.sp.y0 >= 16 && cur.sp.y0 + 32 <= p.ph;
        if (interior) {
            search_level16<8, true, false>(win, wrow0, wcol0, row, a2, mbx, mby, p.pw, p.ph, st, sl);
            search_level16<4, false, false>(win, wrow0, wcol0, row, a2, mbx, mby, p.pw, p.ph, st, sl);
            search_level16<2, false, false>(win, wrow0, wcol0, row, a2, mbx, mby, p.pw, p.ph, st, sl);
            search_level16<1, false, false>(win, wrow0, wcol0, row, a2, mbx, mby, p.pw, p.ph, st, sl);
        } else {
            search_level16<8, true, true>(win, wrow0, wcol0, row, a2, mbx, mby, p.pw, p.ph, st, sl);
            search_level16<4, false, true>(win, wrow0, wcol0, row, a2, mbx, mby, p.pw, p.ph, st, sl);
            search_level16<2, false, true>(win, wrow0, wcol0, row, a2, mbx, mby, p.pw, p.ph, st, sl);
            search_level16<1, false, true>(win, wrow0, wcol0, row, a2, mbx, mby, p.pw, p.ph, st, sl);
        }
        coded = mb_valid && !((float)st.err <= min_err);
        cx = st.cx; cy = st.cy;
        const int wx = wcol0 + cx, shp = wx & 3;
        const unsigned *d = reinterpret_cast<const unsigned *>(win + (wrow0 + cy) * kWinStride + (wx & ~3));
        const unsigned d0 = d[0], d1 = d[1], d2 = d[2], d3 = d[3], d4 = d[4];
        patch = make_uint4(__builtin_amdgcn_alignbyte(d1, d0, shp), __builtin_amdgcn_alignbyte(d2, d1, shp), __builtin_amdgcn_alignbyte(d3, d2, shp),
                           __builtin_amdgcn_alignbyte(d4, d3, shp));
    }
    const long mbi = (long)cur.sp.stream * g.mbs_per_frame + cur.sp.mb_first + m;
    if (r == 0 && mb_valid) {
        mv_out[mbi * 2 + 0] = (int8_t)cx;
        mv_out[mbi * 2 + 1] = (int8_t)cy;
        has_out[mbi] = coded ? 1 : 0;
    }
    __syncthreads();
    if (!wave_valid) return;
    int *xw = wave < kStripsPerWG ? reinterpret_cast<int *>(win) + wave * kXchgDwords : &red_lds[0][0] + (wave - kStripsPerWG) * kXchgDwords;
    int16_t *coef_mb0 = coef + ((long)cur.sp.stream * g.mbs_per_frame + cur.sp.mb_first) * 256;
    uint8_t *dst = recon ? recon + (long)cur.sp.stream * g.pad_frame_bytes + p.pad_off + (long)(cur.sp.y0 + r) * p.pw + cur.sp.x0 + m * 16 : nullptr;
    if (__any(coded)) {
        const LaneQ lq{qtab_lds, i};
        const uint4 o = penc_half<FLT>(coded ? row : patch, patch, xw, slot, i, lq, qmagic, recon != nullptr,
                                       [&]() { store_coef_quads(xw, coef_mb0, cur.sp.n_mb, lane, half_strip); });
        if (recon && mb_valid) *reinterpret_cast<uint4 *>(dst) = o;
    } else if (mb_valid) {
        uint4 *cm = reinterpret_cast<uint4 *>(coef_mb0 + m * 256);
        st_stream(&cm[r], make_uint4(0, 0, 0, 0));
        st_stream(&cm[16 + r], make_uint4(0, 0, 0, 0));
        if (dst) *reinterpret_cast<uint4 *>(dst) = patch;
    }
}

template <int LPM = 8, bool LISTS = false>
__global__ __launch_bounds__(kThreads) void k_dec_iframe(FrameGeom g, const int16_t *__restrict__ coef, CoefLists cl,
                                                          uint8_t *__restrict__ out, const QTab *__restrict__ qtabs,
                                                          uint8_t *__restrict__ frames_out)
{
    __shared__ __attribute__((aligned(16))) int xchg[kStripsPerWG][kXchgDwords];
    __shared__ __attribute__((aligned(16))) int qtab_lds[kStripsPerWG][kQTabDwords];
    constexpr int kPasses = LPM == 8 ? 2 : 1;

    const int lane = threadIdx.x & 63, wave = __builtin_amdgcn_readfirstlane((int)(threadIdx.x >> 6));
    const int gw = xcd_remap((int)blockIdx.x, (int)gridDim.x) * kStripsPerWG + wave;
    const int gstrip = LPM == 8 ? gw : gw >> 1, half_strip = LPM == 8 ? 0 : gw & 1;
    if (gstrip >= g.strips_per_frame * g.n_streams) return;
    const StripPos sp = locate_strip(g, gstrip);
    if (half_strip * 4 >= sp.n_mb) return;
    const PlaneGeom &p = g.p[sp.plane];
    const int slot = lane >> 3, i = lane & 7;
    const int m = LPM == 8 ? slot : half_strip * 4 + (slot >> 1);
    int *xw = xchg[wave];

    const int16_t *coef_mb0 = coef + ((long)sp.stream * g.mbs_per_frame + sp.mb_first) * 256;
    uint4 cbuf[kPasses][2];
    ListSpan span;
    if (LISTS) {
        const int last = min(sp.n_mb - half_strip * 4, LPM == 8 ? 8 : 4) - 1;
        const uint32_t *cnt = cl.counts + (long)sp.stream * (g.mbs_per_frame + 1) + sp.mb_first + half_strip * 4;
        const int mw = min(LPM == 8 ? slot : (slot >> 1), last);
        span = list_span(cl.entries[sp.stream], cnt[mw], cnt[mw + 1], last * (LPM == 8 ? 8 : 16), lane);
    } else if (LPM == 8) {
        fetch_coef_half(cbuf[0], coef_mb0, sp.n_mb, lane, 0);
        fetch_coef_half(cbuf[kPasses - 1], coef_mb0, sp.n_mb, lane, 1);
    } else {
        fetch_coef_quads(cbuf[0], coef_mb0, sp.n_mb, lane, half_strip);
    }
    fill_qtable<false>(qtab_lds[wave], qtabs + p.qsel, lane);
    wave_lds_sync();
    const LaneQ lq{qtab_lds[wave], i};
    uint8_t *dst = out + (long)sp.stream * g.pad_frame_bytes + p.pad_off + (long)(sp.y0 + i) * p.pw + sp.x0 + m * 16;
#pragma unroll
    for (int pass = 0; pass < kPasses; pass++) {
        const int h = LPM == 8 ? pass : (slot & 1);
        if (LISTS) stage_list_half<LPM>(xw, span, lane, sp.mb_first + half_strip * 4, pass);
        else stage_coef_half(xw, cbuf[pass], lane);
        wave_lds_sync();
        int v[2][8];
        gather_half(v, xw, slot, lq);
        inverse_half(v, xw, slot, i, lq);
#pragma unroll
        for (int s = 0; s < 2; s++)
#pragma unroll
            for (int k = 0; k < 8; k++) v[s][k] = min(max(v[s][k] + 128, 0), 255);
        if (m < sp.n_mb) {
            const uint4 o = pack_row(v);
            *reinterpret_cast<uint4 *>(dst + (long)(8 * h) * p.pw) = o;
            if (frames_out)
                store_cropped16(frames_out + (long)sp.stream * g.src_frame_bytes + p.src_off, p, sp.x0 + m * 16, sp.y0 + i + 8 * h, o);
        }
    }
}

template <int LPM = 8, bool LISTS = false>
__global__ __launch_bounds__(kThreads) void k_dec_pframe(FrameGeom g, const int8_t *__restrict__ mv,
                                                          const uint8_t *__restrict__ has, const int16_t *__restrict__ coef, CoefLists cl,
                                                          const uint8_t *__restrict__ ref, uint8_t *__restrict__ out,
                                                          const QTab *__restrict__ qtabs, int *__restrict__ err_flag,
                                                          uint8_t *__restrict__ frames_out)
{
    __shared__ __attribute__((aligned(16))) int xchg[kStripsPerWG][kXchgDwords];
    __shared__ __attribute__((aligned(16))) int qtab_lds[kStripsPerWG][kQTabDwords];
    constexpr int kPasses = LPM == 8 ? 2 : 1;

    const int lane = threadIdx.x & 63, wave = __builtin_amdgcn_readfirstlane((int)(threadIdx.x >> 6));
    const int gw = xcd_remap((int)blockIdx.x, (int)gridDim.x) * kStripsPerWG + wave;
    const int gstrip = LPM == 8 ? gw : gw >> 1, half_strip = LPM == 8 ? 0 : gw & 1;
    if (gstrip >= g.strips_per_frame * g.n_streams) return;
    const StripPos sp = locate_strip(g, gstrip);
    if (half_strip * 4 >= sp.n_mb) return;
    const PlaneGeom &p = g.p[sp.plane];
    const int slot = lane >> 3, i = lane & 7;
    const int m = LPM == 8 ? slot : half_strip * 4 + (slot >> 1);
    int *xw = xchg[wave];
    const bool mb_valid = m < sp.n_mb;
    const long mbi = (long)sp.stream * g.mbs_per_frame + sp.mb_first + (mb_valid ? m : 0);

    int mx = mv[mbi * 2 + 0], my = mv[mbi * 2 + 1];
    const bool coded = mb_valid && has[mbi] != 0;
    uint32_t cnt0 = 0, cnt1 = 0;
    int last_mb = 0;
    if (LISTS) {
        last_mb = min(sp.n_mb - half_strip * 4, LPM == 8 ? 8 : 4) - 1;
        const uint32_t *cnt = cl.counts + (long)sp.stream * (g.mbs_per_frame + 1) + sp.mb_first + half_strip * 4;
        const int mw = min(LPM == 8 ? slot : (slot >> 1), last_mb);
        cnt0 = cnt[mw]; cnt1 = cnt[mw + 1];
    }
    fill_qtable<false>(qtab_lds[wave], qtabs + p.qsel, lane);

    const int mbx = sp.x0 + m * 16, mby = sp.y0;
    if (mb_valid) {
        int sx = mbx + mx, sy = mby + my;
        if (sx < 0 || sx > p.pw - 16 || sy < 0 || sy > p.ph - 16) {
            if (i == 0) atomicOr(err_flag + sp.stream, 1);
            mx = 0; my = 0;
        }
    }
    const bool any_coded = __any(coded);
    const int16_t *coef_mb0 = coef + ((long)sp.stream * g.mbs_per_frame + sp.mb_first) * 256;
    uint4 cbuf[kPasses][2];
    ListSpan span;
    if (any_coded) {
        if (LISTS) {
            span = list_span(cl.entries[sp.stream], cnt0, cnt1, last_mb * (LPM == 8 ? 8 : 16), lane);
        } else if (LPM == 8) {
            fetch_coef_half(cbuf[0], coef_mb0, sp.n_mb, lane, 0);
            fetch_coef_half(cbuf[kPasses - 1], coef_mb0, sp.n_mb, lane, 1);
        } else {
            fetch_coef_quads(cbuf[0], coef_mb0, sp.n_mb, lane, half_strip);
        }
    }
    uint4 patch[kPasses];
#pragma unroll
    for (int pass = 0; pass < kPasses; pass++) patch[pass] = make_uint4(0, 0, 0, 0);
    if (mb_valid) {
        const uint8_t *rp = ref + (long)sp.stream * g.pad_frame_bytes + p.pad_off + (long)(mby + my + i) * p.pw + (mbx + mx);
#pragma unroll
        for (int pass = 0; pass < kPasses; pass++) patch[pass] = load_unaligned16(rp + 8 * (long)(LPM == 8 ? pass : (slot & 1)) * p.pw);
    }
    uint8_t *dst = out + (long)sp.stream * g.pad_frame_bytes + p.pad_off + (long)(sp.y0 + i) * p.pw + mbx;
    uint8_t *crop = frames_out ? frames_out + (long)sp.stream * g.src_frame_bytes + p.src_off : nullptr;

    if (any_coded) {
        wave_lds_sync();
        const LaneQ lq{qtab_lds[wave], i};
#pragma unroll
        for (int pass = 0; pass < kPasses; pass++) {
            const int h = LPM == 8 ? pass : (slot & 1);
            if (LISTS) stage_list_half<LPM>(xw, span, lane, sp.mb_first + half_strip * 4, pass);
            else stage_coef_half(xw, cbuf[pass], lane);
            wave_lds_sync();
            int v[2][8], pp[2][8];
            const int codedmask = coded ? -1 : 0;
            gather_half(v, xw, slot, lq);
            inverse_half(v, xw, slot, i, lq);
            unpack_row(patch[pass], pp);
#pragma unroll
            for (int s = 0; s < 2; s++)
#pragma unroll
                for (int k = 0; k < 8; k++)
                    pp[s][k] = min(max(pp[s][k] + 2 * (v[s][k] & codedmask), 0), 255);
            if (mb_valid) {
                const uint4 o = pack_row(pp);
                *reinterpret_cast<uint4 *>(dst + (long)(8 * h) * p.pw) = o;
                if (crop) store_cropped16(crop, p, mbx, sp.y0 + i + 8 * h, o);
            }
        }
    } else if (mb_valid) {
#pragma unroll
        for (int pass = 0; pass < kPasses; pass++) {
            const int h = LPM == 8 ? pass : (slot & 1);
            *reinterpret_cast<uint4 *>(dst + (long)(8 * h) * p.pw) = patch[pass];
            if (crop) store_cropped16(crop, p, mbx, sp.y0 + i + 8 * h, patch[pass]);
        }
    }
}

#ifndef PFV_PENC_TU
__global__ __launch_bounds__(kThreads) void k_blit(uint8_t *__restrict__ dst, int dst_w, const uint8_t *__restrict__ src,
                                                    int src_w, int dx, int dy, int sx, int sy, int sw, int sh)
{
    long n = (long)sw * sh;
    for (long idx = (long)blockIdx.x * blockDim.x + threadIdx.x; idx < n; idx += (long)gridDim.x * blockDim.x) {
        int row = (int)(idx / sw), col = (int)(idx - (long)row * sw);
        dst[(long)(row + dy) * dst_w + dx + col] = src[(long)(row + sy) * src_w + sx + col];
    }
}

__global__ __launch_bounds__(kThreads) void k_crop_frames(FrameGeom g, const uint8_t *__restrict__ padded,
                                                           uint8_t *__restrict__ frames)
{
    const int plane = blockIdx.y, stream = blockIdx.z;
    const PlaneGeom &p = g.p[plane];
    const uint8_t *src = padded + (long)stream * g.pad_frame_bytes + p.pad_off;
    uint8_t *dst = frames + (long)stream * g.src_frame_bytes + p.src_off;
    if (p.fast_src) {
        int cpr = p.w >> 4;
        long n = (long)cpr * p.h;
        for (long idx = (long)blockIdx.x * blockDim.x + threadIdx.x; idx < n; idx += (long)gridDim.x * blockDim.x) {
            int row = (int)(idx / cpr), ch = (int)(idx - (long)row * cpr);
            *reinterpret_cast<uint4 *>(dst + (long)row * p.w + ch * 16) =
                *reinterpret_cast<const uint4 *>(src + (long)row * p.pw + ch * 16);
        }
    } else {
        long n = (long)p.w * p.h;
        for (long idx = (long)blockIdx.x * blockDim.x + threadIdx.x; idx < n; idx += (long)gridDim.x * blockDim.x) {
            int row = (int)(idx / p.w), col = (int)(idx - (long)row * p.w);
            dst[idx] = src[(long)row * p.pw + col];
        }
    }
}

__global__ __launch_bounds__(kThreads) void k_reduce2x(uint8_t *__restrict__ dst, const uint8_t *__restrict__ src, int src_w,
                                                        int src_h)
{
    const int dw = src_w >> 1, dh = src_h >> 1;
    const long n = (long)dw * dh;
    for (long idx = (long)blockIdx.x * blockDim.x + threadIdx.x; idx < n; idx += (long)gridDim.x * blockDim.x) {
        int y = (int)(idx / dw), x = (int)(idx - (long)y * dw);
        dst[idx] = src[(long)(2 * y) * src_w + 2 * x];
    }
}
__global__ __launch_bounds__(kThreads) void k_double2x(uint8_t *__restrict__ dst, const uint8_t *__restrict__ src, int src_w,
                                                        int src_h)
{
    const int dw = src_w * 2;
    const long n = (long)dw * src_h * 2;
    for (long idx = (long)blockIdx.x * blockDim.x + threadIdx.x; idx < n; idx += (long)gridDim.x * blockDim.x) {
        int y = (int)(idx / dw), x = (int)(idx - (long)y * dw);
        dst[idx] = src[(long)(y >> 1) * src_w + (x >> 1)];
    }
}

__device__ __forceinline__ uint32_t f32_as_u8(float x)
{
    return x >= 255.0f ? 255u : (x > 0.0f ? (uint32_t)(int)x : 0u);
}
__global__ __launch_bounds__(kThreads) void k_rgb_to_yuv420(const uint8_t *__restrict__ rgb, int w, int h, uint8_t *__restrict__ frame)
{
#pragma clang fp contract(off)
    const long n = (long)w * h;
    const int cw = w >> 1, ch = h >> 1;
    uint8_t *py = frame, *pu = frame + n, *pv = pu + (long)cw * ch;
    for (long idx = (long)blockIdx.x * blockDim.x + threadIdx.x; idx < n; idx += (long)gridDim.x * blockDim.x) {
        const int y = (int)(idx / w), x = (int)(idx - (long)y * w);
        const float r = (float)rgb[3 * idx], g = (float)rgb[3 * idx + 1], b = (float)rgb[3 * idx + 2];
        py[idx] = (uint8_t)f32_as_u8((0.299f * r) + (0.587f * g) + (0.114f * b));
        if (!(x & 1) && !(y & 1) && (x >> 1) < cw && (y >> 1) < ch) {
            const long c = (long)(y >> 1) * cw + (x >> 1);
            pu[c] = (uint8_t)f32_as_u8(128.0f - (0.168736f * r) - (0.331264f * g) + (0.5f * b));
            pv[c] = (uint8_t)f32_as_u8(128.0f + (0.5f * r) - (0.418688f * g) - (0.081312f * b));
        }
    }
}
__global__ __launch_bounds__(kThreads) void k_yuv420_to_rgb(const uint8_t *__restrict__ frame, int w, int h, uint8_t *__restrict__ rgb)
{
// ... 49 lines not shown
```

pretty-fast-video_amd/csrc/pfv_launch.hip:

```cpp
static float biased_rcp(int q)
{
    volatile float r = q ? 1.0f / (float)q : 0.0f;
    r = r * 1.000000476837158203125f;
    return r;
}
static int make_qtab(pfv_ctx *ctx, const int32_t q[64], QTab *out, bool decode_only = false)
{
    if (!q) return fail(ctx, PFV_ERR_BAD_ARG, "q-table is null");
    for (int i = 0; i < 64; i++)
        if (q[i] < (decode_only ? 0 : 1) || q[i] > 65535)
            return fail(ctx, PFV_ERR_BAD_ARG, decode_only ? "q-table entry outside [0,65535]" : "q-table entry outside [1,65535]");
    for (int i = 0; i < 64; i++) {
        out->rcp[i] = biased_rcp(q[i]);
        int z = H_INV_ZIGZAG[i];
        out->deq[i] = (int32_t)((uint32_t)H_SCALE[z] * (uint32_t)q[z]);
    }
    return PFV_OK;
}

static int ensure_scratch(pfv_ctx *ctx, int slot, size_t bytes, void **out)
{
    if (bytes == 0) bytes = 16;
    if (ctx->scratch_cap[slot] < bytes) {
        if (ctx->scratch[slot]) {
// ... 94 lines not shown
}
static inline unsigned half_strip_blocks(const FrameGeom &g)
{
    long waves = 2 * (long)g.strips_per_frame * g.n_streams;
    return (unsigned)((waves + kStripsPerWG - 1) / kStripsPerWG);
}
static void launch_enc_iframe(pfv_ctx *ctx, bool flt, bool small, const FrameGeom &g, const uint8_t *src, int16_t *coef, uint8_t *recon, const QTab *qt)
{
    if (small) {
        if (flt) hipLaunchKernelGGL((k_enc_iframe<true, 16>), dim3(half_strip_blocks(g)), dim3(kThreads), 0, ctx->stream, g, src, coef, recon, qt, kQuantMagic);
        else hipLaunchKernelGGL((k_enc_iframe<false, 16>), dim3(half_strip_blocks(g)), dim3(kThreads), 0, ctx->stream, g, src, coef, recon, qt, kQuantMagic);
    } else {
        if (flt) hipLaunchKernelGGL((k_enc_iframe<true, 8>), dim3(strip_blocks(g)), dim3(kThreads), 0, ctx->stream, g, src, coef, recon, qt, kQuantMagic);
        else hipLaunchKernelGGL((k_enc_iframe<false, 8>), dim3(strip_blocks(g)), dim3(kThreads), 0, ctx->stream, g, src, coef, recon, qt, kQuantMagic);
    }
}
static void launch_enc_pframe(pfv_ctx *ctx, bool flt, bool small, int compaction, const FrameGeom &g, const uint8_t *src, const uint8_t *ref, int8_t *mv,
                              uint8_t *has, int16_t *coef, uint8_t *recon, const QTab *qt, float min_err)
{
    const bool split = compaction == 2 && !small;
    launch_enc_pframe_kernels(ctx->stream, flt, small, split ? kPencSplit : (compaction ? kPencCompactMax : 0), g, penc_blocks(ctx, g), src, ref, mv, has, coef, recon, qt, min_err);
    if (split) {
        const unsigned tf = (unsigned)((long)g.n_streams * tf_groups_per_frame(g));
        if (flt) hipLaunchKernelGGL(k_pf_transform<true>, dim3(tf), dim3(64), 0, ctx->stream, g, src, ref, (const int8_t *)mv, (const uint8_t *)has, coef, recon, qt, kQuantMagic);
        else hipLaunchKernelGGL(k_pf_transform<false>, dim3(tf), dim3(64), 0, ctx->stream, g, src, ref, (const int8_t *)mv, (const uint8_t *)has, coef, recon, qt, kQuantMagic);
    }
}
static void launch_enc_pframe_full(pfv_ctx *ctx, bool flt, int radius, const FrameGeom &g, const uint8_t *src, const uint8_t *ref, int8_t *mv, uint8_t *has,
                                   int16_t *coef, uint8_t *recon, const QTab *qt, float min_err)
{
    hipLaunchKernelGGL(k_pf_search_full, dim3(penc_blocks(ctx, g)), dim3(kThreads), 0, ctx->stream, g, src, ref, mv, has, coef, recon, min_err, radius);
    const unsigned tf = (unsigned)((long)g.n_streams * tf_groups_per_frame(g));
    if (flt) hipLaunchKernelGGL(k_pf_transform<true>, dim3(tf), dim3(64), 0, ctx->stream, g, src, ref, (const int8_t *)mv, (const uint8_t *)has, coef, recon, qt, kQuantMagic);
    else hipLaunchKernelGGL(k_pf_transform<false>, dim3(tf), dim3(64), 0, ctx->stream, g, src, ref, (const int8_t *)mv, (const uint8_t *)has, coef, recon, qt, kQuantMagic);
}
static HalfGeom half_geom(const FrameGeom &g)
{
    HalfGeom hg{};
    long off = 0;
    for (int i = 0; i < g.n_planes; i++) {
        hg.pitch[i] = (g.p[i].pw / 2 + 15) & ~15;
        hg.off[i] = off;
        off += (long)hg.pitch[i] * (g.p[i].ph / 2);
    }
    hg.frame_bytes = off;
    return hg;
}
static void launch_enc_pframe_hier(pfv_ctx *ctx, bool flt, int radius, const FrameGeom &g, const uint8_t *src, const uint8_t *ref, uint8_t *hsrc, uint8_t *href,
                                   int8_t *cmv, int8_t *mv, uint8_t *has, int16_t *coef, uint8_t *recon, const QTab *qt, float min_err,
                                   const hipEvent_t *marks = nullptr )
{
    const HalfGeom hg = half_geom(g);
    const unsigned hb = (unsigned)(((hg.frame_bytes / 4) * g.n_streams + kThreads - 1) / kThreads);
    auto mark = [&](int k) { if (marks) (void)hipEventRecord(marks[k], ctx->stream); };
    mark(0);
    hipLaunchKernelGGL(k_halve<false>, dim3(hb), dim3(kThreads), 0, ctx->stream, g, hg, src, hsrc);
    mark(1);
    hipLaunchKernelGGL(k_halve<true>, dim3(hb), dim3(kThreads), 0, ctx->stream, g, hg, ref, href);
    mark(2);
    hipLaunchKernelGGL(k_pf_search_coarse, dim3(penc_blocks(ctx, g)), dim3(kThreads), 0, ctx->stream, g, hg, (const uint8_t *)hsrc, (const uint8_t *)href, cmv, radius / 2);
    mark(3);
    hipLaunchKernelGGL(k_pf_refine, dim3(strip_blocks(g)), dim3(kThreads), 0, ctx->stream, g, src, ref, (const int8_t *)cmv, mv, has, coef, recon, min_err);
    mark(4);
    const unsigned tf = (unsigned)((long)g.n_streams * tf_groups_per_frame(g));
    if (flt) hipLaunchKernelGGL(k_pf_transform<true>, dim3(tf), dim3(64), 0, ctx->stream, g, src, ref, (const int8_t *)mv, (const uint8_t *)has, coef, recon, qt, kQuantMagic);
    else hipLaunchKernelGGL(k_pf_transform<false>, dim3(tf), dim3(64), 0, ctx->stream, g, src, ref, (const int8_t *)mv, (const uint8_t *)has, coef, recon, qt, kQuantMagic);
    mark(5);
}
struct DecCoefs {
    const int16_t *dense = nullptr;
    CoefLists lists{nullptr, nullptr};
    DecCoefs() = default;
    DecCoefs(const int16_t *d) : dense(d) {}
    DecCoefs(const uint32_t *const *entries, const uint32_t *counts) : lists{entries, counts} {}
    bool is_lists() const { return lists.entries != nullptr; }
    DecCoefs shifted(size_t slot, size_t mbs_per_frame) const
    {
        DecCoefs c;
        if (dense) c.dense = dense + slot * mbs_per_frame * 256;
        if (lists.entries) c.lists = CoefLists{lists.entries + slot, lists.counts + slot * (mbs_per_frame + 1)};
        return c;
    }
};
static void launch_dec_iframe(pfv_ctx *ctx, bool small, const FrameGeom &g, const DecCoefs &c, uint8_t *out, const QTab *qt, uint8_t *frames_out)
{
    const dim3 grid(small ? half_strip_blocks(g) : strip_blocks(g)), block(kThreads);
    if (c.is_lists()) {
        if (small) hipLaunchKernelGGL((k_dec_iframe<16, true>), grid, block, 0, ctx->stream, g, c.dense, c.lists, out, qt, frames_out);
        else hipLaunchKernelGGL((k_dec_iframe<8, true>), grid, block, 0, ctx->stream, g, c.dense, c.lists, out, qt, frames_out);
    } else {
        if (small) hipLaunchKernelGGL((k_dec_iframe<16, false>), grid, block, 0, ctx->stream, g, c.dense, c.lists, out, qt, frames_out);
        else hipLaunchKernelGGL((k_dec_iframe<8, false>), grid, block, 0, ctx->stream, g, c.dense, c.lists, out, qt, frames_out);
    }
}
static void launch_dec_pframe(pfv_ctx *ctx, bool small, const FrameGeom &g, const int8_t *mv, const uint8_t *has, const DecCoefs &c, const uint8_t *ref,
                              uint8_t *out, const QTab *qt, int *flag, uint8_t *frames_out)
{
    const dim3 grid(small ? half_strip_blocks(g) : strip_blocks(g)), block(kThreads);
    if (c.is_lists()) {
        if (small) hipLaunchKernelGGL((k_dec_pframe<16, true>), grid, block, 0, ctx->stream, g, mv, has, c.dense, c.lists, ref, out, qt, flag, frames_out);
        else hipLaunchKernelGGL((k_dec_pframe<8, true>), grid, block, 0, ctx->stream, g, mv, has, c.dense, c.lists, ref, out, qt, flag, frames_out);
    } else {
        if (small) hipLaunchKernelGGL((k_dec_pframe<16, false>), grid, block, 0, ctx->stream, g, mv, has, c.dense, c.lists, ref, out, qt, flag, frames_out);
        else hipLaunchKernelGGL((k_dec_pframe<8, false>), grid, block, 0, ctx->stream, g, mv, has, c.dense, c.lists, ref, out, qt, flag, frames_out);
    }
}

static int launch_check(pfv_ctx *ctx, const char *what)
{
    hipError_t e = hipGetLastError();
    if (e != hipSuccess) return hip_fail(ctx, e, what);
    return PFV_OK;
}

static int upload_qtabs(pfv_ctx *ctx, const int32_t *const *tables, int n, bool decode_only)
{
    for (int i = 0; i < n; i++) {
        int rc = make_qtab(ctx, tables[i], &ctx->qtab_host[i], decode_only);
        if (rc) return rc;
    }
    HIP_TRY(ctx, hipMemcpyAsync(ctx->qtab_dev, ctx->qtab_host, n * sizeof(QTab), hipMemcpyHostToDevice, ctx->stream));
    return PFV_OK;
}
```

pretty-fast-video_amd/csrc/pfv_plane_ops.hip:

```cpp
extern "C" {

PFV_API int pfv_encode_plane(pfv_ctx *ctx, const uint8_t *px, int w, int h, const int32_t q[64], uint8_t clear,
                             int16_t *coef_out)
{
    if (!ctx) return fail(nullptr, PFV_ERR_BAD_ARG, "null ctx");
    if (!px || !coef_out || w <= 0 || h <= 0) return fail(ctx, PFV_ERR_BAD_ARG, "pfv_encode_plane: bad argument");
    HIP_TRY(ctx, hipSetDevice(ctx->device));
    FrameGeom g = plane_geom(w, h, clear);
    const int32_t *tabs[1] = {q};
    int rc = upload_qtabs(ctx, tabs, 1, false);
    if (rc) return rc;
    void *d_src, *d_coef;
    size_t coef_bytes = (size_t)g.mbs_per_frame * 512;
    if ((rc = ensure_scratch(ctx, 0, (size_t)w * h, &d_src))) return rc;
    if ((rc = ensure_scratch(ctx, 1, coef_bytes, &d_coef))) return rc;
    HIP_TRY(ctx, hipMemcpyAsync(d_src, px, (size_t)w * h, hipMemcpyHostToDevice, ctx->stream));
    launch_enc_iframe(ctx, ctx->opt_enc_transform != PFV_ENC_TRANSFORM_INT, use_small_grid(ctx->opt_lane_mapping, g), g, (const uint8_t *)d_src, (int16_t *)d_coef,
                      nullptr, ctx->qtab_dev);
    if ((rc = launch_check(ctx, "k_enc_iframe"))) return rc;
    HIP_TRY(ctx, hipMemcpyAsync(coef_out, d_coef, coef_bytes, hipMemcpyDeviceToHost, ctx->stream));
    HIP_TRY(ctx, hipStreamSynchronize(ctx->stream));
    return PFV_OK;
}

PFV_API int pfv_encode_plane_delta(pfv_ctx *ctx, const uint8_t *px, int w, int h, const uint8_t *ref,
                                   const int32_t q[64], float px_err, uint8_t clear, int8_t *mv_out,
                                   uint8_t *has_coef_out, int16_t *coef_out)
{
    if (!ctx) return fail(nullptr, PFV_ERR_BAD_ARG, "null ctx");
    if (!px || !ref || !mv_out || !has_coef_out || !coef_out || w <= 0 || h <= 0)
        return fail(ctx, PFV_ERR_BAD_ARG, "pfv_encode_plane_delta: bad argument");
    HIP_TRY(ctx, hipSetDevice(ctx->device));
    FrameGeom g = plane_geom(w, h, clear);
    const int32_t *tabs[1] = {q};
    int rc = upload_qtabs(ctx, tabs, 1, false);
    if (rc) return rc;
    size_t n = (size_t)g.mbs_per_frame, coef_bytes = n * 512, pad_bytes = (size_t)g.pad_frame_bytes;
    void *d_src, *d_coef, *d_ref, *d_mv, *d_has;
    if ((rc = ensure_scratch(ctx, 0, (size_t)w * h, &d_src))) return rc;
    if ((rc = ensure_scratch(ctx, 1, coef_bytes, &d_coef))) return rc;
    if ((rc = ensure_scratch(ctx, 2, pad_bytes, &d_ref))) return rc;
    if ((rc = ensure_scratch(ctx, 3, n * 2, &d_mv))) return rc;
    if ((rc = ensure_scratch(ctx, 4, n, &d_has))) return rc;
    HIP_TRY(ctx, hipMemcpyAsync(d_src, px, (size_t)w * h, hipMemcpyHostToDevice, ctx->stream));
    HIP_TRY(ctx, hipMemcpyAsync(d_ref, ref, pad_bytes, hipMemcpyHostToDevice, ctx->stream));
    float min_err = px_err * px_err * 256.0f;
    launch_enc_pframe(ctx, ctx->opt_enc_transform != PFV_ENC_TRANSFORM_INT, use_small_grid(ctx->opt_lane_mapping, g), ctx->opt_tile_compaction, g,
                      (const uint8_t *)d_src, (const uint8_t *)d_ref, (int8_t *)d_mv, (uint8_t *)d_has, (int16_t *)d_coef, nullptr, ctx->qtab_dev, min_err);
    if ((rc = launch_check(ctx, "k_enc_pframe"))) return rc;
    HIP_TRY(ctx, hipMemcpyAsync(coef_out, d_coef, coef_bytes, hipMemcpyDeviceToHost, ctx->stream));
    HIP_TRY(ctx, hipMemcpyAsync(mv_out, d_mv, n * 2, hipMemcpyDeviceToHost, ctx->stream));
    HIP_TRY(ctx, hipMemcpyAsync(has_coef_out, d_has, n, hipMemcpyDeviceToHost, ctx->stream));
    HIP_TRY(ctx, hipStreamSynchronize(ctx->stream));
    return PFV_OK;
}

PFV_API int pfv_decode_plane_into(pfv_ctx *ctx, const int16_t *coef, int bw, int bh, const int32_t q[64],
                                  uint8_t *target)
{
    if (!ctx) return fail(nullptr, PFV_ERR_BAD_ARG, "null ctx");
    if (!coef || !target || bw <= 0 || bh <= 0) return fail(ctx, PFV_ERR_BAD_ARG, "pfv_decode_plane_into: bad argument");
    HIP_TRY(ctx, hipSetDevice(ctx->device));
    FrameGeom g = plane_geom(bw * 16, bh * 16, 0);
    const int32_t *tabs[1] = {q};
    int rc = upload_qtabs(ctx, tabs, 1, true);
    if (rc) return rc;
    size_t n = (size_t)bw * bh, coef_bytes = n * 512, pad_bytes = (size_t)g.pad_frame_bytes;
    void *d_coef, *d_out;
    if ((rc = ensure_scratch(ctx, 1, coef_bytes, &d_coef))) return rc;
    if ((rc = ensure_scratch(ctx, 5, pad_bytes, &d_out))) return rc;
    HIP_TRY(ctx, hipMemcpyAsync(d_coef, coef, coef_bytes, hipMemcpyHostToDevice, ctx->stream));
    launch_dec_iframe(ctx, use_small_grid(ctx->opt_lane_mapping, g), g, (const int16_t *)d_coef, (uint8_t *)d_out, ctx->qtab_dev, nullptr);
    if ((rc = launch_check(ctx, "k_dec_iframe"))) return rc;
    HIP_TRY(ctx, hipMemcpyAsync(target, d_out, pad_bytes, hipMemcpyDeviceToHost, ctx->stream));
    HIP_TRY(ctx, hipStreamSynchronize(ctx->stream));
    return PFV_OK;
}

PFV_API int pfv_decode_plane_delta(pfv_ctx *ctx, const int8_t *mv, const uint8_t *has_coef, const int16_t *coef,
                                   int bw, int bh, const int32_t q[64], const uint8_t *ref, uint8_t *out)
{
    if (!ctx) return fail(nullptr, PFV_ERR_BAD_ARG, "null ctx");
    if (!mv || !has_coef || !coef || !ref || !out || bw <= 0 || bh <= 0)
        return fail(ctx, PFV_ERR_BAD_ARG, "pfv_decode_plane_delta: bad argument");
    HIP_TRY(ctx, hipSetDevice(ctx->device));
    FrameGeom g = plane_geom(bw * 16, bh * 16, 0);
    const int32_t *tabs[1] = {q};
    int rc = upload_qtabs(ctx, tabs, 1, true);
    if (rc) return rc;
    size_t n = (size_t)bw * bh, coef_bytes = n * 512, pad_bytes = (size_t)g.pad_frame_bytes;
    void *d_coef, *d_ref, *d_mv, *d_has, *d_out;
    if ((rc = ensure_scratch(ctx, 1, coef_bytes, &d_coef))) return rc;
    if ((rc = ensure_scratch(ctx, 2, pad_bytes, &d_ref))) return rc;
    if ((rc = ensure_scratch(ctx, 3, n * 2, &d_mv))) return rc;
    if ((rc = ensure_scratch(ctx, 4, n, &d_has))) return rc;
    if ((rc = ensure_scratch(ctx, 5, pad_bytes, &d_out))) return rc;
    HIP_TRY(ctx, hipMemcpyAsync(d_coef, coef, coef_bytes, hipMemcpyHostToDevice, ctx->stream));
    HIP_TRY(ctx, hipMemcpyAsync(d_ref, ref, pad_bytes, hipMemcpyHostToDevice, ctx->stream));
    HIP_TRY(ctx, hipMemcpyAsync(d_mv, mv, n * 2, hipMemcpyHostToDevice, ctx->stream));
    HIP_TRY(ctx, hipMemcpyAsync(d_has, has_coef, n, hipMemcpyHostToDevice, ctx->stream));
    HIP_TRY(ctx, hipMemsetAsync(ctx->flag_dev, 0, sizeof(int), ctx->stream));
    launch_dec_pframe(ctx, use_small_grid(ctx->opt_lane_mapping, g), g, (const int8_t *)d_mv, (const uint8_t *)d_has, (const int16_t *)d_coef, (const uint8_t *)d_ref,
                      (uint8_t *)d_out, ctx->qtab_dev, ctx->flag_dev, nullptr);
    if ((rc = launch_check(ctx, "k_dec_pframe"))) return rc;
    int flag = 0;
    HIP_TRY(ctx, hipMemcpyAsync(&flag, ctx->flag_dev, sizeof(int), hipMemcpyDeviceToHost, ctx->stream));
    HIP_TRY(ctx, hipStreamSynchronize(ctx->stream));
    if (flag) return fail(ctx, PFV_ERR_BAD_MV, "motion vector points outside the reference plane (src/common.rs:258-259)");
    HIP_TRY(ctx, hipMemcpy(out, d_out, pad_bytes, hipMemcpyDeviceToHost));
    return PFV_OK;
}

PFV_API int pfv_decode_plane_delta_into(pfv_ctx *ctx, const int8_t *mv, const uint8_t *has_coef,
                                        const int16_t *coef, int bw, int bh, const int32_t q[64],
                                        uint8_t *ref_and_target)
{
    return pfv_decode_plane_delta(ctx, mv, has_coef, coef, bw, bh, q, ref_and_target, ref_and_target);
}

PFV_API int pfv_blit_dev(pfv_ctx *ctx, uint8_t *dst, int dst_w, int dst_h, const uint8_t *src, int src_w, int src_h,
                         int dx, int dy, int sx, int sy, int sw, int sh)
{
    if (!ctx) return fail(nullptr, PFV_ERR_BAD_ARG, "null ctx");
    if (!dst || !src || sw < 0 || sh < 0 || dx < 0 || dy < 0 || sx < 0 || sy < 0 || dx + sw > dst_w || dy + sh > dst_h ||
        sx + sw > src_w || sy + sh > src_h)
        return fail(ctx, PFV_ERR_BAD_ARG, "pfv_blit_dev: rectangle outside a plane (the reference panics on slice bounds)");
    if (sw == 0 || sh == 0) return PFV_OK;
    HIP_TRY(ctx, hipSetDevice(ctx->device));
    long n = (long)sw * sh;
    int blocks = (int)((n + kThreads - 1) / kThreads);
    if (blocks > 4096) blocks = 4096;
    hipLaunchKernelGGL(k_blit, dim3(blocks), dim3(kThreads), 0, ctx->stream, dst, dst_w, src, src_w, dx, dy, sx, sy, sw, sh);
    return launch_check(ctx, "k_blit");
}

PFV_API int pfv_reduce_dev(pfv_ctx *ctx, uint8_t *dst, const uint8_t *src, int src_w, int src_h)
{
    if (!ctx) return fail(nullptr, PFV_ERR_BAD_ARG, "null ctx");
    if (!dst || !src || src_w < 0 || src_h < 0) return fail(ctx, PFV_ERR_BAD_ARG, "pfv_reduce_dev: bad argument");
    long n = (long)(src_w / 2) * (src_h / 2);
    if (n == 0) return PFV_OK;
    HIP_TRY(ctx, hipSetDevice(ctx->device));
    int blocks = (int)((n + kThreads - 1) / kThreads);
    if (blocks > 4096) blocks = 4096;
    hipLaunchKernelGGL(k_reduce2x, dim3(blocks), dim3(kThreads), 0, ctx->stream, dst, src, src_w, src_h);
    return launch_check(ctx, "k_reduce2x");
}
PFV_API int pfv_double_dev(pfv_ctx *ctx, uint8_t *dst, const uint8_t *src, int src_w, int src_h)
{
    if (!ctx) return fail(nullptr, PFV_ERR_BAD_ARG, "null ctx");
    if (!dst || !src || src_w < 0 || src_h < 0) return fail(ctx, PFV_ERR_BAD_ARG, "pfv_double_dev: bad argument");
    long n = (long)src_w * src_h * 4;
    if (n == 0) return PFV_OK;
    HIP_TRY(ctx, hipSetDevice(ctx->device));
    int blocks = (int)((n + kThreads - 1) / kThreads);
    if (blocks > 4096) blocks = 4096;
    hipLaunchKernelGGL(k_double2x, dim3(blocks), dim3(kThreads), 0, ctx->stream, dst, src, src_w, src_h);
    return launch_check(ctx, "k_double2x");
}

PFV_API int pfv_rgb_to_yuv420_dev(pfv_ctx *ctx, const uint8_t *rgb_dev, int width, int height, uint8_t *frame_dev)
{
    if (!ctx) return fail(nullptr, PFV_ERR_BAD_ARG, "null ctx");
    if (!rgb_dev || !frame_dev || width <= 0 || height <= 0 || (width & 1) || (height & 1))
        return fail(ctx, PFV_ERR_BAD_ARG, "pfv_rgb_to_yuv420_dev: null buffer or odd / non-positive size (src/frame.rs:13)");
    HIP_TRY(ctx, hipSetDevice(ctx->device));
    long n = (long)width * height;
    int blocks = (int)std::min<long>((n + kThreads - 1) / kThreads, 8192);
    hipLaunchKernelGGL(k_rgb_to_yuv420, dim3(blocks), dim3(kThreads), 0, ctx->stream, rgb_dev, width, height, frame_dev);
    return launch_check(ctx, "k_rgb_to_yuv420");
}
PFV_API int pfv_yuv420_to_rgb_dev(pfv_ctx *ctx, const uint8_t *frame_dev, int width, int height, uint8_t *rgb_dev)
{
    if (!ctx) return fail(nullptr, PFV_ERR_BAD_ARG, "null ctx");
    if (!rgb_dev || !frame_dev || width <= 0 || height <= 0 || (width & 1) || (height & 1))
        return fail(ctx, PFV_ERR_BAD_ARG, "pfv_yuv420_to_rgb_dev: null buffer or odd / non-positive size (src/frame.rs:13)");
    HIP_TRY(ctx, hipSetDevice(ctx->device));
    long n = (long)width * height;
    int blocks = (int)std::min<long>((n + kThreads - 1) / kThreads, 8192);
    hipLaunchKernelGGL(k_yuv420_to_rgb, dim3(blocks), dim3(kThreads), 0, ctx->stream, frame_dev, width, height, rgb_dev);
    return launch_check(ctx, "k_yuv420_to_rgb");
}

PFV_API int pfv_synth_frames_dev(pfv_ctx *ctx, int width, int height, int n_streams, const uint64_t *seeds, int t, uint8_t *frames_dev)
{
// ... 95 lines not shown
```

pretty-fast-video_amd/csrc/pfv_sessions.hip:

```cpp
static int init_padded(pfv_ctx *ctx, const FrameGeom &g, uint8_t *buf)
{
    dim3 grid(64, 3, g.n_streams);
    hipLaunchKernelGGL(k_init_padded, grid, dim3(kThreads), 0, ctx->stream, g, buf);
    return launch_check(ctx, "k_init_padded");
}

struct XformNorms {
    double F1[8];
    double Iabs[8][8];
    signed char fsign[64];
    signed char isign[64];
};
static const XformNorms &xform_norms()
{
    static const XformNorms t = [] {
        XformNorms n{};
        for (int k = 0; k < 8; k++) {
            int f[8] = {0, 0, 0, 0, 0, 0, 0, 0}, i8[8] = {0, 0, 0, 0, 0, 0, 0, 0};
            f[k] = i8[k] = 1 << 20;
            fdct8(f);
            idct8(i8);
            for (int u = 0; u < 8; u++) {
                n.F1[u] += fabs((double)f[u]) / (1 << 20);
                n.Iabs[u][k] = fabs((double)i8[u]) / (1 << 20);
// ... 24 lines not shown
    }
    double col[8][8];
    for (int u = 0; u < 8; u++)
        for (int v = 0; v < 8; v++) {
            double a = 16;
            for (int k = 0; k < 8; k++) a += nm.Iabs[u][k] * D[k][v];
            col[u][v] = a;
            worst = std::max(worst, a);
        }
    for (int u = 0; u < 8; u++)
        for (int v = 0; v < 8; v++) {
            double a = 16;
            for (int k = 0; k < 8; k++) a += col[u][k] * nm.Iabs[v][k];
            worst = std::max(worst, a);
        }
    return worst < 8388608.0;
}

constexpr int kMaxRungs = 11;
struct pfv_enc_session {
    pfv_ctx *ctx = nullptr;
    int width = 0, height = 0, n_streams = 0;
    FrameGeom geom;
    QTab *qtab_dev = nullptr;
    int n_rungs = 1, rung = 0;
    int qualities[kMaxRungs] = {0};
    float px_err[kMaxRungs] = {0.0f};
    bool flt = false;
    int tile_compaction = 1;
    int lane_mapping = PFV_LANES_AUTO;
    int search_mode = PFV_SEARCH_FOURSTEP;
    int search_radius = 0;
    uint8_t *hier_src = nullptr, *hier_ref = nullptr;
    int8_t *hier_cmv = nullptr;
    bool hier_launched = false;
    uint8_t *prev[2] = {nullptr, nullptr};
    int cur = 0;
    int win_first = 0, win_count = 0;
    size_t in_stride = 0;
    uint8_t *st_frames = nullptr;
    int16_t *st_coef = nullptr;
    int8_t *st_mv = nullptr;
    uint8_t *st_has = nullptr;
    uint8_t *ingest_frames = nullptr;
    uint8_t *scale_frames = nullptr;
    uint8_t *denoise_frames = nullptr;
    uint32_t *q_map = nullptr;
    uint64_t *q_sse = nullptr;
    uint64_t *report_host = nullptr;
    int32_t *ssim_map = nullptr;
    int64_t *ssim_sums = nullptr;
    int64_t *ssim_host = nullptr;
    uint32_t *probe_acc = nullptr;
    uint32_t *probe_sizes = nullptr;
    uint64_t *rd_acc = nullptr;
    uint64_t *rd_out = nullptr;
    uint32_t *pprobe_acc = nullptr;
    uint32_t *pprobe_out = nullptr;
    uint64_t *prd_out = nullptr;
    uint32_t *ssim_probe_map = nullptr;
    uint64_t *ssim_probe_out = nullptr;
    bool ent_on = false;
    uint32_t ent_cap = 0;
    EntBufs ent{};
    std::vector<void *> ent_allocs;
    std::vector<uint32_t> ent_sizes;
    uint8_t *ent_packed = nullptr;
    uint32_t *ent_offsets_dev = nullptr;
    size_t ent_packed_cap = 0;
    hipStream_t ent_stream = nullptr;
    hipEvent_t ev_encoded = nullptr;
    hipEvent_t ev_packed[2] = {nullptr, nullptr};
    int ev_cur = 0;
    bool ev_prev_valid = false;
};

struct pfv_dec_session {
    pfv_ctx *ctx = nullptr;
    int width = 0, height = 0, n_streams = 0, n_qtables = 0;
    FrameGeom geom;
    QTab *qtab_dev = nullptr;
    uint8_t *fb[2] = {nullptr, nullptr};
    int lane_mapping = PFV_LANES_AUTO;
    int cur = 0;
    int *flag_dev = nullptr;
    std::vector<int> flags_host;
    uint8_t *frames_out = nullptr;
    size_t out_stride = 0;
    int win_first = 0, win_count = 0;
    int16_t *st_coef = nullptr;
    int8_t *st_mv = nullptr;
    uint8_t *st_has = nullptr;
    uint8_t *st_frames = nullptr;
    uint32_t *st_idx = nullptr;
    int16_t *st_val = nullptr;
    size_t st_sparse_cap = 0;
    uint32_t *q_map = nullptr;
    int32_t *ssim_map = nullptr;
    int db_mode = 0;
    uint8_t db_fixed[3] = {0, 0, 0};
    uint8_t db_auto[3] = {0, 0, 0};
    std::vector<uint8_t> db_table;
    uint8_t *rgb_out = nullptr;
    int rgb_format = 0;
    size_t rgb_pitch = 0, rgb_stride = 0;
    uint8_t *db_scratch = nullptr;
    uint8_t *st_rgb = nullptr;
    pfv_scaler *scaled_sc = nullptr;
    uint8_t *scaled_out = nullptr;
    size_t scaled_stride = 0;
};
static int enc_report_enqueue(pfv_enc_session *s);
static int dec_deblock_win(pfv_dec_session *s, int first, int count, uint8_t *frames_out_dev, size_t out_stride);
static int enc_ssim_enqueue(pfv_enc_session *s);
static int dec_present_scratch(pfv_dec_session *s, const char *what);
static int dec_present_step(pfv_dec_session *s);
struct pfv_scaler;

extern "C" {

PFV_API int pfv_enc_session_create_ladder(pfv_ctx *ctx, int width, int height, const int *qualities, int n_rungs, int n_streams,
                                          pfv_enc_session **out)
{
    if (!ctx || !out) return fail(ctx, PFV_ERR_BAD_ARG, "pfv_enc_session_create: bad argument");
    *out = nullptr;
    if (width <= 0 || height <= 0 || (width & 1) || (height & 1) || width > 65535 || height > 65535)
        return fail(ctx, PFV_ERR_BAD_ARG, "width/height must be even (src/frame.rs:13) and fit u16 (src/enc.rs:195-196)");
    if (!qualities || n_rungs < 1 || n_rungs > kMaxRungs) return fail(ctx, PFV_ERR_BAD_ARG, "a quality ladder has 1..11 rungs");
    for (int r = 0; r < n_rungs; r++) {
        if (qualities[r] < 0 || qualities[r] > 10) return fail(ctx, PFV_ERR_BAD_ARG, "quality must be in 0..10 (src/enc.rs:38)");
        if (r && qualities[r] <= qualities[r - 1]) return fail(ctx, PFV_ERR_BAD_ARG, "the qualities of a ladder must be strictly ascending");
    }
    if (n_streams <= 0) return fail(ctx, PFV_ERR_BAD_ARG, "n_streams must be positive");
    HIP_TRY(ctx, hipSetDevice(ctx->device));
    pfv_enc_session *s = new pfv_enc_session();
    s->ctx = ctx; s->width = width; s->height = height; s->n_streams = n_streams;
    s->win_count = n_streams;
    s->geom = frame_geom(width, height, n_streams);
    s->n_rungs = n_rungs;
    std::vector<QTab> tabs((size_t)4 * n_rungs);
    bool exact = true;
    for (int r = 0; r < n_rungs; r++) {
        int32_t q[4][64];
        s->qualities[r] = qualities[r];
        pfv_qtables_from_quality(qualities[r], q[0], q[1], q[2], q[3], &s->px_err[r]);
        for (int i = 0; i < 4; i++) {
            int rc = make_qtab(ctx, q[i], &tabs[(size_t)4 * r + i]);
            if (rc) { delete s; return rc; }
        }
        exact = exact && enc_float_exact(q[0], 128.0 * 256.0) && enc_float_exact(q[1], 128.0 * 256.0) && enc_float_exact(q[2], 127.0 * 256.0) &&
                enc_float_exact(q[3], 127.0 * 256.0);
    }
    s->tile_compaction = ctx->opt_tile_compaction;
    s->lane_mapping = ctx->opt_lane_mapping;
    s->flt = ctx->opt_enc_transform != PFV_ENC_TRANSFORM_INT && exact;
    size_t pad_bytes = (size_t)s->geom.pad_frame_bytes * n_streams;
    hipError_t e = hipMalloc((void **)&s->qtab_dev, tabs.size() * sizeof(QTab));
    if (e == hipSuccess) e = hipMemcpy(s->qtab_dev, tabs.data(), tabs.size() * sizeof(QTab), hipMemcpyHostToDevice);
    if (e == hipSuccess) e = hipMalloc((void **)&s->prev[0], pad_bytes);
    if (e == hipSuccess) e = hipMalloc((void **)&s->prev[1], pad_bytes);
    if (e != hipSuccess) {
        int rc = hip_fail(ctx, e, "pfv_enc_session_create");
        pfv_enc_session_destroy(s);
        return rc;
    }
    int rc = init_padded(ctx, s->geom, s->prev[0]);
// ... 423 lines not shown
        else if (v == kEntErrCapacity) { if (rc == PFV_OK) rc = PFV_ERR_NOMEM; v = 0; }
        s->ent_sizes[i] = sizes_out[i] = v;
    }
    if (rc == PFV_ERR_FORMAT) return fail(ctx, rc, "coefficient needs more than 15 size bits (src/rle.rs:44)");
    if (rc == PFV_ERR_NOMEM) return fail(ctx, rc, "payload exceeds the capacity given to pfv_enc_entropy_enable");
    return PFV_OK;
}
PFV_API int pfv_enc_payloads_fetch(pfv_enc_session *s, uint8_t *out, size_t cap, uint32_t *sizes_out, uint64_t *offsets_out)
{
    if (!s || !out || !sizes_out || !offsets_out) return fail(s ? s->ctx : nullptr, PFV_ERR_BAD_ARG, "pfv_enc_payloads_fetch: bad argument");
    pfv_ctx *ctx = s->ctx;
    int rc = pfv_enc_payload_sizes(s, sizes_out);
    if (rc) return rc;
    const int S = s->n_streams;
    std::vector<uint32_t> off((size_t)S);
    size_t total = 0;
    for (int i = 0; i < S; i++) {
        off[(size_t)i] = (uint32_t)total;
        offsets_out[i] = total;
        total += ((size_t)sizes_out[i] + 15) & ~(size_t)15;
    }
    if (total > cap || total > 0xfffffff0u) return fail(ctx, PFV_ERR_NOMEM, "pfv_enc_payloads_fetch: output buffer too small");
    if (total == 0) return PFV_OK;
    hipStream_t st = s->ent_stream ? s->ent_stream : ctx->stream;
    if (total > s->ent_packed_cap) {
        HIP_TRY(ctx, hipStreamSynchronize(st));
        if (s->ent_packed) (void)hipFree(s->ent_packed);
        s->ent_packed = nullptr; s->ent_packed_cap = 0;
        const size_t want = total + total / 2;
        HIP_TRY(ctx, hipMalloc((void **)&s->ent_packed, want));
        s->ent_packed_cap = want;
    }
    if (!s->ent_offsets_dev) HIP_TRY(ctx, hipMalloc((void **)&s->ent_offsets_dev, (size_t)S * 4));
    HIP_TRY(ctx, hipMemcpyAsync(s->ent_offsets_dev, off.data(), (size_t)S * 4, hipMemcpyHostToDevice, st));
    EntFrame f{};
    f.n_streams = S;
    f.cap_bytes = s->ent_cap;
    f.ones16 = 0x00010001u;
    hipLaunchKernelGGL(k_ent_gather, dim3(32, (unsigned)S), dim3(kEntThreads), 0, st, f, s->ent, s->ent_offsets_dev, s->ent_packed);
    if ((rc = launch_check(ctx, "k_ent_gather"))) return rc;
    HIP_TRY(ctx, hipMemcpyAsync(out, s->ent_packed, total, hipMemcpyDeviceToHost, st));
    HIP_TRY(ctx, hipStreamSynchronize(st));
    return PFV_OK;
}

PFV_API const uint8_t *pfv_enc_payload_dev(pfv_enc_session *s, int stream)
{
    if (!s || !s->ent_on || stream < 0 || stream >= s->n_streams) return nullptr;
    return s->ent.payload + (size_t)stream * s->ent_cap;
}
PFV_API size_t pfv_enc_payload_capacity(pfv_enc_session *s) { return s && s->ent_on ? s->ent_cap : 0; }
PFV_API int pfv_enc_payload_fetch(pfv_enc_session *s, int stream, uint8_t *out, size_t nbytes)
{
    if (!s || !out) return fail(s ? s->ctx : nullptr, PFV_ERR_BAD_ARG, "pfv_enc_payload_fetch: bad argument");
    pfv_ctx *ctx = s->ctx;
    if (!s->ent_on) return fail(ctx, PFV_ERR_STATE, "call pfv_enc_entropy_enable first");
    if (stream < 0 || stream >= s->n_streams || nbytes > s->ent_cap) return fail(ctx, PFV_ERR_BAD_ARG, "pfv_enc_payload_fetch: out of range");
    hipStream_t st = s->ent_stream ? s->ent_stream : ctx->stream;
    if (nbytes) HIP_TRY(ctx, hipMemcpyAsync(out, s->ent.payload + (size_t)stream * s->ent_cap, nbytes, hipMemcpyDeviceToHost, st));
    HIP_TRY(ctx, hipStreamSynchronize(st));
    return PFV_OK;
}

PFV_API int pfv_dec_session_create(pfv_ctx *ctx, int width, int height, const int32_t *qtables, int n_qtables,
                                   int n_streams, pfv_dec_session **out)
{
    if (!ctx || !out) return fail(ctx, PFV_ERR_BAD_ARG, "pfv_dec_session_create: bad argument");
    *out = nullptr;
    if (width <= 0 || height <= 0 || (width & 1) || (height & 1) || width > 65535 || height > 65535)
        return fail(ctx, PFV_ERR_BAD_ARG, "width/height must be even (src/frame.rs:13) and fit u16");
    if ((!qtables && n_qtables > 0) || n_qtables < 0 || n_qtables > 65535 || n_streams <= 0)
        return fail(ctx, PFV_ERR_BAD_ARG, "pfv_dec_session_create: bad q-table set or stream count");
    HIP_TRY(ctx, hipSetDevice(ctx->device));
    const int n_dev = std::min(n_qtables, 256);
    std::vector<QTab> tabs((size_t)std::max(n_dev, 1));
    for (int i = 0; i < n_dev; i++) {
        int rc = make_qtab(ctx, qtables + (size_t)i * 64, &tabs[i], true);
        if (rc) return rc;
    }
    pfv_dec_session *s = new pfv_dec_session();
    s->ctx = ctx; s->width = width; s->height = height; s->n_streams = n_streams; s->n_qtables = n_qtables;
    s->win_count = n_streams;
    s->lane_mapping = ctx->opt_lane_mapping;
    s->geom = frame_geom(width, height, n_streams);
    s->db_table.resize((size_t)n_dev);
    for (int i = 0; i < n_dev; i++) s->db_table[(size_t)i] = (uint8_t)pfv_deblock_strength(qtables + (size_t)i * 64);
    size_t pad_bytes = (size_t)s->geom.pad_frame_bytes * n_streams;
    hipError_t e = hipMalloc((void **)&s->qtab_dev, tabs.size() * sizeof(QTab));
    if (e == hipSuccess) e = hipMemcpy(s->qtab_dev, tabs.data(), tabs.size() * sizeof(QTab), hipMemcpyHostToDevice);
    if (e == hipSuccess) e = hipMalloc((void **)&s->fb[0], pad_bytes);
    if (e == hipSuccess) e = hipMalloc((void **)&s->fb[1], pad_bytes);
    if (e == hipSuccess) e = hipMalloc((void **)&s->flag_dev, (size_t)n_streams * sizeof(int));
    if (e == hipSuccess) e = hipMemset(s->flag_dev, 0, (size_t)n_streams * sizeof(int));
    if (e != hipSuccess) {
        int rc = hip_fail(ctx, e, "pfv_dec_session_create");
        pfv_dec_session_destroy(s);
        return rc;
    }
    int rc = init_padded(ctx, s->geom, s->fb[0]);
    if (!rc) rc = init_padded(ctx, s->geom, s->fb[1]);
    if (rc) { pfv_dec_session_destroy(s); return rc; }
    *out = s;
    return PFV_OK;
}

PFV_API void pfv_dec_session_destroy(pfv_dec_session *s)
{
    if (!s) return;
    (void)hipSetDevice(s->ctx->device);
    (void)hipStreamSynchronize(s->ctx->stream);
    void *bufs[] = {s->qtab_dev, s->fb[0], s->fb[1], s->flag_dev, s->st_coef, s->st_mv, s->st_has, s->st_frames, s->st_idx, s->st_val, s->q_map, s->ssim_map, s->db_scratch, s->st_rgb};
    for (void *b : bufs)
        if (b) (void)hipFree(b);
    delete s;
}

PFV_API int pfv_dec_set_output_dev(pfv_dec_session *s, uint8_t *frames_out_dev)
{
    if (!s) return fail(nullptr, PFV_ERR_BAD_ARG, "null session");
    s->frames_out = frames_out_dev;
    s->out_stride = 0;
    return PFV_OK;
}
PFV_API int pfv_dec_set_output_strided_dev(pfv_dec_session *s, uint8_t *frames_out_dev, size_t stride_bytes)
{
    if (!s) return fail(nullptr, PFV_ERR_BAD_ARG, "null session");
    if (stride_bytes && stride_bytes < (size_t)s->geom.src_frame_bytes)
        return fail(s->ctx, PFV_ERR_BAD_ARG, "pfv_dec_set_output_strided_dev: stride below pfv_frame_bytes (the slots' frames would overlap)");
    s->frames_out = frames_out_dev;
    s->out_stride = stride_bytes;
    return PFV_OK;
}
PFV_API int pfv_dec_session_set_window(pfv_dec_session *s, int first, int count)
{
    if (!s) return fail(nullptr, PFV_ERR_BAD_ARG, "null session");
    if (first < 0 || count <= 0 || first > s->n_streams - count) return fail(s->ctx, PFV_ERR_BAD_ARG, "pfv_dec_session_set_window: window outside [0, n_streams)");
    s->win_first = first; s->win_count = count;
    return PFV_OK;
}
static bool dec_full_window(const pfv_dec_session *s) { return s->win_first == 0 && s->win_count == s->n_streams && s->out_stride == 0; }

static FrameGeom dec_out_geom(const pfv_dec_session *s, FrameGeom g, const uint8_t *out_base)
{
    if (s->out_stride) {
        g.src_frame_bytes = (long)s->out_stride;
        if (s->out_stride % 16)
            for (int i = 0; i < 3; i++) g.p[i].fast_src = 0;
    }
    return with_base_alignment(g, out_base);
}
static bool fused_output_ok(const pfv_dec_session *s)
{
    if (!s->frames_out) return false;
    FrameGeom g = dec_out_geom(s, s->geom, s->frames_out);
    return g.p[0].fast_src && g.p[1].fast_src && g.p[2].fast_src;
}

static int dec_geom(pfv_dec_session *s, const uint8_t qidx[3], FrameGeom *g)
{
    if (!qidx) return fail(s->ctx, PFV_ERR_BAD_ARG, "qidx is null");
    *g = s->geom;
    for (int i = 0; i < 3; i++) {
        if (qidx[i] >= s->n_qtables)
            return fail(s->ctx, PFV_ERR_FORMAT, "q-table index out of range (the reference panics: src/dec.rs:249-251)");
        g->p[i].qsel = qidx[i];
    }
    return PFV_OK;
}
static int dec_crop_win(pfv_dec_session *s, int first, int count, uint8_t *frames_out_dev, size_t out_stride);

static int dec_launch(pfv_dec_session *s, bool pframe, int first, int count, const int8_t *mv_dev, const uint8_t *has_dev, const DecCoefs &coefs,
                      const uint8_t qidx[3])
{
    pfv_ctx *ctx = s->ctx;
    FrameGeom g;
    int rc = dec_geom(s, qidx, &g);
    if (rc) return rc;
    const size_t ostride = s->out_stride ? s->out_stride : (size_t)s->geom.src_frame_bytes;
    const size_t mb0 = (size_t)first * (size_t)s->geom.mbs_per_frame, pad0 = (size_t)first * (size_t)s->geom.pad_frame_bytes;
    const bool fused = !s->db_mode && fused_output_ok(s);
    uint8_t *crop = fused ? s->frames_out + (size_t)first * ostride : nullptr;
    g = dec_out_geom(s, g, s->frames_out);
    g.n_streams = count;
    const int nxt = s->cur ^ 1;
    if (pframe) {
        launch_dec_pframe(ctx, use_small_grid(s->lane_mapping, g), g, mv_dev + mb0 * 2, has_dev + mb0, coefs.shifted((size_t)first, (size_t)s->geom.mbs_per_frame),
                          s->fb[s->cur] + pad0, s->fb[nxt] + pad0, s->qtab_dev, s->flag_dev + first, crop);
        rc = launch_check(ctx, "k_dec_pframe");
    } else {
        launch_dec_iframe(ctx, use_small_grid(s->lane_mapping, g), g, coefs.shifted((size_t)first, (size_t)s->geom.mbs_per_frame), s->fb[nxt] + pad0, s->qtab_dev, crop);
        rc = launch_check(ctx, "k_dec_iframe");
    }
    return rc;
}

}
static int dec_step(pfv_dec_session *s, bool pframe, const int8_t *mv_dev, const uint8_t *has_coef_dev, const DecCoefs &coefs, const uint8_t qidx[3])
{
    pfv_ctx *ctx = s->ctx;
    HIP_TRY(ctx, hipSetDevice(ctx->device));
    int rc = dec_launch(s, pframe, s->win_first, s->win_count, mv_dev, has_coef_dev, coefs, qidx);
    if (rc) return rc;
    s->cur ^= 1;
    for (int i = 0; i < 3; i++) s->db_auto[i] = s->db_table[qidx[i]];
    if (s->frames_out && s->db_mode) rc = dec_deblock_win(s, s->win_first, s->win_count, s->frames_out, s->out_stride);
    else if (s->frames_out && !fused_output_ok(s)) rc = dec_crop_win(s, s->win_first, s->win_count, s->frames_out, s->out_stride);
    if (rc || (!s->rgb_out && !s->scaled_out)) return rc;
    return dec_present_step(s);
}
extern "C" {

PFV_API int pfv_dec_iframe_dev(pfv_dec_session *s, const int16_t *coef_dev, const uint8_t qidx[3])
{
    if (!s) return fail(nullptr, PFV_ERR_BAD_ARG, "null session");
    if (!coef_dev) return fail(s->ctx, PFV_ERR_BAD_ARG, "pfv_dec_iframe_dev: null buffer");
    return dec_step(s, false, nullptr, nullptr, coef_dev, qidx);
}

PFV_API int pfv_dec_pframe_dev(pfv_dec_session *s, const int8_t *mv_dev, const uint8_t *has_coef_dev,
                               const int16_t *coef_dev, const uint8_t qidx[3])
{
    if (!s) return fail(nullptr, PFV_ERR_BAD_ARG, "null session");
    if (!mv_dev || !has_coef_dev || !coef_dev) return fail(s->ctx, PFV_ERR_BAD_ARG, "pfv_dec_pframe_dev: null buffer");
    return dec_step(s, true, mv_dev, has_coef_dev, coef_dev, qidx);
}

PFV_API int pfv_dec_iframe_lists_dev(pfv_dec_session *s, const uint32_t *const *entries_dev, const uint32_t *counts_dev, const uint8_t qidx[3])
{
    if (!s) return fail(nullptr, PFV_ERR_BAD_ARG, "null session");
    if (!entries_dev || !counts_dev) return fail(s->ctx, PFV_ERR_BAD_ARG, "pfv_dec_iframe_lists_dev: null buffer");
    return dec_step(s, false, nullptr, nullptr, DecCoefs(entries_dev, counts_dev), qidx);
}
PFV_API int pfv_dec_pframe_lists_dev(pfv_dec_session *s, const int8_t *mv_dev, const uint8_t *has_coef_dev, const uint32_t *const *entries_dev,
                                     const uint32_t *counts_dev, const uint8_t qidx[3])
{
    if (!s) return fail(nullptr, PFV_ERR_BAD_ARG, "null session");
    if (!mv_dev || !has_coef_dev || !entries_dev || !counts_dev) return fail(s->ctx, PFV_ERR_BAD_ARG, "pfv_dec_pframe_lists_dev: null buffer");
    return dec_step(s, true, mv_dev, has_coef_dev, DecCoefs(entries_dev, counts_dev), qidx);
}
PFV_API int pfv_coef_lists_from_dense(const int16_t *coef, const uint8_t *has_coef, int total_blocks, uint32_t *entries_out, size_t cap, uint32_t *counts_out,
                                      size_t *n_out)
{
    if (!coef || !entries_out || !counts_out || !n_out || total_blocks <= 0) return fail(nullptr, PFV_ERR_BAD_ARG, "pfv_coef_lists_from_dense: bad argument");
    ListSink sink{entries_out, cap, counts_out, (size_t)total_blocks};
    bool full = false;
    for (size_t b = 0; b < (size_t)total_blocks && !full; b++) {
        if (has_coef && !has_coef[b]) continue;
        for (size_t i = 0; i < 256 && !full; i++)
            if (coef[b * 256 + i]) full = !sink.put(b * 256 + i, coef[b * 256 + i]);
    }
    sink.finish();
    *n_out = sink.n;
    return full ? 1 : PFV_OK;
}

static int dec_check_flags(pfv_dec_session *s, std::vector<int> *which)
{
    pfv_ctx *ctx = s->ctx;
    s->flags_host.assign((size_t)s->n_streams, 0);
    HIP_TRY(ctx, hipMemcpyAsync(s->flags_host.data(), s->flag_dev, (size_t)s->n_streams * sizeof(int), hipMemcpyDeviceToHost, ctx->stream));
    HIP_TRY(ctx, hipStreamSynchronize(ctx->stream));
    bool any = false;
    for (int k = 0; k < s->n_streams; k++) any = any || s->flags_host[(size_t)k] != 0;
    if (which) *which = s->flags_host;
    if (any) {
        HIP_TRY(ctx, hipMemsetAsync(s->flag_dev, 0, (size_t)s->n_streams * sizeof(int), ctx->stream));
        return fail(ctx, PFV_ERR_BAD_MV, "motion vector points outside the reference plane (src/common.rs:258-259)");
    }
    return PFV_OK;
}
PFV_API int pfv_dec_check(pfv_dec_session *s)
{
    if (!s) return fail(nullptr, PFV_ERR_BAD_ARG, "null session");
// ... 159 lines not shown
```

pretty-fast-video_amd/session.py:

```python
from __future__ import annotations

import ctypes

import numpy as np

from . import _lib
from .context import Context, ptr


def qtables_from_quality(quality: int):
    lib = _lib.load()
    t = [np.zeros(64, dtype=np.int32) for _ in range(4)]
    pe = ctypes.c_float()
    rc = lib.pfv_qtables_from_quality(int(quality), ptr(t[0]), ptr(t[1]), ptr(t[2]), ptr(t[3]), ctypes.byref(pe))
    _lib.check(None, rc)
    return t[0], t[1], t[2], t[3], float(pe.value)


class _Geometry:
    def __init__(self, width: int, height: int, n_streams: int):
        lib = _lib.load()
        self.width, self.height, self.n_streams = int(width), int(height), int(n_streams)
        self.frame_bytes = int(lib.pfv_frame_bytes(width, height))
        self.padded_frame_bytes = int(lib.pfv_padded_frame_bytes(width, height))
# ... 273 lines not shown

    def decode_pframe_sparse(self, mv, has_coef, idx, val, qidx=(2, 3, 3)):
        m = np.ascontiguousarray(mv, dtype=np.int8)
        hc = np.ascontiguousarray(has_coef, dtype=np.uint8)
        i = np.ascontiguousarray(idx, dtype=np.uint32)
        v = np.ascontiguousarray(val, dtype=np.int16)
        assert i.shape == v.shape and i.ndim == 1
        self.ctx.check(self.ctx._lib.pfv_dec_pframe_sparse(self.handle, ptr(m), ptr(hc), ptr(i), ptr(v), i.size, ptr(self._qidx(qidx))))

    def decode_pframe(self, mv, has_coef, coef, qidx=(2, 3, 3)):
        m = np.ascontiguousarray(mv, dtype=np.int8)
        hc = np.ascontiguousarray(has_coef, dtype=np.uint8)
        c = np.ascontiguousarray(coef, dtype=np.int16)
        assert c.size == self.n_streams * self.total_blocks * 256
        self.ctx.check(self.ctx._lib.pfv_dec_pframe(self.handle, ptr(m), ptr(hc), ptr(c), ptr(self._qidx(qidx))))

    def coef_lists(self, coef, has_coef=None):
        c = np.ascontiguousarray(coef, dtype=np.int16).reshape(self.n_streams, self.total_blocks * 256)
        hc = None if has_coef is None else np.ascontiguousarray(has_coef, dtype=np.uint8).reshape(self.n_streams, self.total_blocks)
        entries, counts = [], np.zeros((self.n_streams, self.total_blocks + 1), dtype=np.uint32)
        for k in range(self.n_streams):
            e = np.empty(self.total_blocks * 256, dtype=np.uint32)
            n = ctypes.c_size_t(0)
            rc = self.ctx._lib.pfv_coef_lists_from_dense(ptr(c[k]), ptr(hc[k]) if hc is not None else None, self.total_blocks, ptr(e), e.size,
                                                         ptr(counts[k]), ctypes.byref(n))
            assert rc == 0, rc
            entries.append(e[:n.value].copy())
        return entries, counts

    def _upload_lists(self, entries, counts):
        ctx = self.ctx
        sizes = [max(int(e.size), 1) for e in entries]
        ent_dev = ctx.alloc(4 * sum(sizes))
        ptrs = np.zeros(self.n_streams, dtype=np.uint64)
        off = 0
        for k, e in enumerate(entries):
            ptrs[k] = ent_dev + 4 * off
            if e.size:
                ctx.upload(ent_dev + 4 * off, np.ascontiguousarray(e, dtype=np.uint32))
            off += sizes[k]
        ptr_dev = ctx.alloc(8 * self.n_streams)
        ctx.upload(ptr_dev, ptrs)
        r = np.ascontiguousarray(counts, dtype=np.uint32)
        rng_dev = ctx.alloc(r.nbytes)
        ctx.upload(rng_dev, r)
        return ent_dev, ptr_dev, rng_dev

    def decode_iframe_lists(self, entries, counts, qidx=(0, 1, 1)):
        bufs = self._upload_lists(entries, counts)
        try:
            self.ctx.check(self.ctx._lib.pfv_dec_iframe_lists_dev(self.handle, ctypes.c_void_p(bufs[1]), ctypes.c_void_p(bufs[2]), ptr(self._qidx(qidx))))
            self.ctx.sync()
        finally:
            for b in bufs:
                self.ctx.free(b)

    def decode_pframe_lists(self, mv, has_coef, entries, counts, qidx=(2, 3, 3)):
        ctx = self.ctx
        m = np.ascontiguousarray(mv, dtype=np.int8)
        hc = np.ascontiguousarray(has_coef, dtype=np.uint8)
        bufs = list(self._upload_lists(entries, counts))
        try:
            mv_dev = ctx.alloc(m.nbytes); bufs.append(mv_dev)
            has_dev = ctx.alloc(hc.nbytes); bufs.append(has_dev)
            ctx.upload(mv_dev, m)
            ctx.upload(has_dev, hc)
            ctx.check(ctx._lib.pfv_dec_pframe_lists_dev(self.handle, ctypes.c_void_p(mv_dev), ctypes.c_void_p(has_dev), ctypes.c_void_p(bufs[1]),
                                                        ctypes.c_void_p(bufs[2]), ptr(self._qidx(qidx))))
            self.check()
        finally:
            for b in bufs:
                ctx.free(b)

    def decode_iframe_dev(self, coef_dev: int, qidx=(0, 1, 1)):
        self.ctx.check(self.ctx._lib.pfv_dec_iframe_dev(self.handle, ctypes.c_void_p(coef_dev), ptr(self._qidx(qidx))))

    def decode_pframe_dev(self, mv_dev: int, has_dev: int, coef_dev: int, qidx=(2, 3, 3)):
        self.ctx.check(self.ctx._lib.pfv_dec_pframe_dev(self.handle, ctypes.c_void_p(mv_dev), ctypes.c_void_p(has_dev),
                                                        ctypes.c_void_p(coef_dev), ptr(self._qidx(qidx))))

    def check(self):
        self.ctx.check(self.ctx._lib.pfv_dec_check(self.handle))

    def get_frame(self) -> np.ndarray:
        out = np.empty((self.n_streams, self.frame_bytes), dtype=np.uint8)
        self.ctx.check(self.ctx._lib.pfv_dec_get_frame(self.handle, ptr(out)))
        return out

    def set_output_dev(self, frames_dev):
        self.ctx.check(self.ctx._lib.pfv_dec_set_output_dev(self.handle, ctypes.c_void_p(frames_dev or 0)))

    def set_output_strided_dev(self, frames_dev, stride_bytes: int):
        self.ctx.check(self.ctx._lib.pfv_dec_set_output_strided_dev(self.handle, ctypes.c_void_p(frames_dev or 0), int(stride_bytes)))

    def set_window(self, first: int = 0, count: int | None = None):
        self.ctx.check(self.ctx._lib.pfv_dec_session_set_window(self.handle, int(first), int(self.n_streams - first if count is None else count)))

    def get_frame_dev(self, frames_dev: int):
        self.ctx.check(self.ctx._lib.pfv_dec_get_frame_dev(self.handle, ctypes.c_void_p(frames_dev)))

    def set_deblock(self, mode=None, strength=None):
        from .quality import deblock_args
        m, p, _keep = deblock_args(mode, strength)
        self.ctx.check(self.ctx._lib.pfv_dec_set_deblock(self.handle, m, p))

    def get_frame_rgb(self, fmt="rgb8") -> np.ndarray:
        from .quality import pix_format, rgb_shape
        m = pix_format(fmt)
        out = np.empty((self.n_streams,) + rgb_shape(self.ctx, self.width, self.height, m), dtype=np.uint8)
        self.ctx.check(self.ctx._lib.pfv_dec_get_frame_rgb(self.handle, ptr(out), m))
        return out

    def get_frame_rgb_dev(self, dst_dev: int, fmt="rgb8", pitch: int = 0, stride: int = 0):
        from .quality import pix_format
        self.ctx.check(self.ctx._lib.pfv_dec_get_frame_rgb_dev(self.handle, ctypes.c_void_p(dst_dev), pix_format(fmt), int(pitch), int(stride)))

    def set_output_scaled_dev(self, scaler, dst_dev, stride: int = 0):
        self._scaled_keep = scaler if dst_dev else None
        self.ctx.check(self.ctx._lib.pfv_dec_set_output_scaled_dev(self.handle, scaler.handle if (scaler is not None and dst_dev) else None,
                                                                  ctypes.c_void_p(dst_dev or 0), int(stride)))

    def set_output_rgb_dev(self, dst_dev, fmt="rgb8", pitch: int = 0, stride: int = 0):
        from .quality import pix_format
        self.ctx.check(self.ctx._lib.pfv_dec_set_output_rgb_dev(self.handle, ctypes.c_void_p(dst_dev or 0), pix_format(fmt), int(pitch), int(stride)))

    def framebuffer(self) -> np.ndarray:
        out = np.empty((self.n_streams, self.padded_frame_bytes), dtype=np.uint8)
        self.ctx.check(self.ctx._lib.pfv_dec_framebuffer(self.handle, ptr(out)))
        return out

    def distortion_dev(self, frames_dev: int, sse_dev: int, mb_sse_dev: int = 0):
        self.ctx.check(self.ctx._lib.pfv_dec_distortion_dev(self.handle, ctypes.c_void_p(frames_dev), ctypes.c_void_p(sse_dev),
                                                            ctypes.c_void_p(mb_sse_dev or 0)))

    def distortion(self, frames, mb_map: bool = False, out=None, out_map=None):
        from .quality import session_distortion
        return session_distortion(self, self.distortion_dev, frames, mb_map, out, out_map)

    def ssim_dev(self, frames_dev: int, ssim_q24_dev: int, mb_dev: int = 0):
        self.ctx.check(self.ctx._lib.pfv_dec_ssim_dev(self.handle, ctypes.c_void_p(frames_dev), ctypes.c_void_p(ssim_q24_dev),
                                                      ctypes.c_void_p(mb_dev or 0)))

    def ssim(self, frames, mb_map: bool = False, out=None, out_map=None):
        from .quality import session_distortion
        return session_distortion(self, self.ssim_dev, frames, mb_map, out, out_map, sum_dtype=np.int64, map_dtype=np.int32)
```

Baseline: 1.428 billion.

## Run decoder inverse transform in packed float with exact-range guard and int fallback

```diff
diff --git a/include/pfv_hip_ext.h b/include/pfv_hip_ext.h
--- a/include/pfv_hip_ext.h
+++ b/include/pfv_hip_ext.h
@@ -14,11 +14,12 @@
 
 typedef enum pfv_option {
     PFV_OPT_ENC_TRANSFORM = 1, PFV_OPT_TILE_COMPACTION = 2, PFV_OPT_LANE_MAPPING = 3, PFV_OPT_ENTROPY_DECODE = 4,
-    PFV_OPT_ENTDEC_LANE_BITS = 5, PFV_OPT_ENTDEC_LAUNCHES = 6, PFV_OPT_ENTDEC_INNER_ROUNDS = 7
+    PFV_OPT_ENTDEC_LANE_BITS = 5, PFV_OPT_ENTDEC_LAUNCHES = 6, PFV_OPT_ENTDEC_INNER_ROUNDS = 7, PFV_OPT_DEC_TRANSFORM = 8
 } pfv_option;
 enum { PFV_ENTROPY_DECODE_AUTO = 0, PFV_ENTROPY_DECODE_HOST = 1, PFV_ENTROPY_DECODE_DEVICE = 2 };
 enum { PFV_LANES_AUTO = 0, PFV_LANES_PER_MB_8 = 1, PFV_LANES_PER_MB_16 = 2 };
 enum { PFV_ENC_TRANSFORM_AUTO = 0, PFV_ENC_TRANSFORM_INT = 1 };
+enum { PFV_DEC_TRANSFORM_AUTO = 0, PFV_DEC_TRANSFORM_INT = 1 };
 PFV_API int pfv_ctx_set_option(pfv_ctx *ctx, int option, int value);
 PFV_API int pfv_ctx_get_option(pfv_ctx *ctx, int option, int *value);
 
@@ -104,6 +105,9 @@
 PFV_API int pfv_dec_set_output_dev(pfv_dec_session *s, uint8_t *frames_out_dev);
 PFV_API int pfv_dec_set_output_strided_dev(pfv_dec_session *s, uint8_t *frames_out_dev, size_t stride_bytes);
 PFV_API int pfv_dec_session_set_window(pfv_dec_session *s, int first, int count);
+PFV_API int pfv_dec_float_guard(void);
+PFV_API int pfv_dec_session_enable_path_stats(pfv_dec_session *s, int on);
+PFV_API int pfv_dec_session_path_stats(pfv_dec_session *s, int64_t *int_waves, int64_t *total_waves);
 PFV_API int pfv_encoder_set_device_entropy(pfv_encoder *e, int on);
 enum { PFV_FRAME_PACKED = 0, PFV_FRAME_PADDED = 1 };
 PFV_API int pfv_frames_sse_dev(pfv_ctx *ctx, int width, int height, int n_streams, const uint8_t *a_dev, int a_layout, size_t a_stride,
diff --git a/pretty-fast-video_amd/_lib.py b/pretty-fast-video_amd/_lib.py
--- a/pretty-fast-video_amd/_lib.py
+++ b/pretty-fast-video_amd/_lib.py
@@ -27,6 +27,8 @@
 PFV_OPT_ENTDEC_LANE_BITS, PFV_OPT_ENTDEC_LAUNCHES, PFV_OPT_ENTDEC_INNER_ROUNDS = 5, 6, 7
 PFV_ENTROPY_DECODE_AUTO, PFV_ENTROPY_DECODE_HOST, PFV_ENTROPY_DECODE_DEVICE = 0, 1, 2
 PFV_ENC_TRANSFORM_AUTO, PFV_ENC_TRANSFORM_INT = 0, 1
+PFV_OPT_DEC_TRANSFORM = 8
+PFV_DEC_TRANSFORM_AUTO, PFV_DEC_TRANSFORM_INT = 0, 1
 PFV_FRAME_PACKED, PFV_FRAME_PADDED = 0, 1
 PFV_DEBLOCK_OFF, PFV_DEBLOCK_AUTO, PFV_DEBLOCK_FIXED = 0, 1, 2
 PFV_PIX_RGB8, PFV_PIX_RGBA8, PFV_PIX_BGRA8 = 0, 1, 2
@@ -141,6 +143,9 @@
     ("pfv_dec_set_output_dev", c_int, [_P, _P]),
     ("pfv_dec_set_output_strided_dev", c_int, [_P, _P, c_size_t]),
     ("pfv_dec_session_set_window", c_int, [_P, c_int, c_int]),
+    ("pfv_dec_float_guard", c_int, []),
+    ("pfv_dec_session_enable_path_stats", c_int, [_P, c_int]),
+    ("pfv_dec_session_path_stats", c_int, [_P, POINTER(ctypes.c_int64), POINTER(ctypes.c_int64)]),
     ("pfv_dec_get_frame", c_int, [_P, _P]),
     ("pfv_dec_framebuffer", c_int, [_P, _P]),
     ("pfv_dec_check", c_int, [_P]),
diff --git a/pretty-fast-video_amd/csrc/pfv_context.hip b/pretty-fast-video_amd/csrc/pfv_context.hip
--- a/pretty-fast-video_amd/csrc/pfv_context.hip
+++ b/pretty-fast-video_amd/csrc/pfv_context.hip
@@ -1,3 +1,6 @@
+#ifndef PFV_DEC_TRANSFORM_DEFAULT
+#define PFV_DEC_TRANSFORM_DEFAULT PFV_DEC_TRANSFORM_AUTO
+#endif
 constexpr int kCtxScratch = 9;
 struct pfv_ctx {
     int device = 0;
@@ -11,6 +14,7 @@
     int n_cus = 256;
     bool capturing = false;
     int opt_enc_transform = PFV_ENC_TRANSFORM_AUTO;
+    int opt_dec_transform = PFV_DEC_TRANSFORM_DEFAULT;
     int opt_tile_compaction = 1;
     int opt_lane_mapping = PFV_LANES_AUTO;
     int opt_entropy_decode = PFV_ENTROPY_DECODE_AUTO;
@@ -62,6 +66,7 @@
 #endif
 PFV_API const char *pfv_version(void) { return "pfv-hip 0.2 (gfx950; pfv-rs 0.2.2 / codec 2.1.1 hot path; src " PFV_BUILD_ID ")"; }
 PFV_API int pfv_pad16(int x) { return pad16(x); }
+PFV_API int pfv_dec_float_guard(void) { return kDecFloatGuard; }
 
 PFV_API const char *pfv_last_error(pfv_ctx *ctx) { return ctx ? ctx->err.c_str() : g_tls_err.c_str(); }
 
@@ -73,6 +78,10 @@
         if (value != PFV_ENC_TRANSFORM_AUTO && value != PFV_ENC_TRANSFORM_INT) return fail(ctx, PFV_ERR_BAD_ARG, "PFV_OPT_ENC_TRANSFORM: unknown value");
         ctx->opt_enc_transform = value;
         return PFV_OK;
+    case PFV_OPT_DEC_TRANSFORM:
+        if (value != PFV_DEC_TRANSFORM_AUTO && value != PFV_DEC_TRANSFORM_INT) return fail(ctx, PFV_ERR_BAD_ARG, "PFV_OPT_DEC_TRANSFORM: unknown value");
+        ctx->opt_dec_transform = value;
+        return PFV_OK;
     case PFV_OPT_TILE_COMPACTION:
         if (value < 0 || value > 2) return fail(ctx, PFV_ERR_BAD_ARG, "PFV_OPT_TILE_COMPACTION: 0, 1 or 2");
         ctx->opt_tile_compaction = value;
@@ -106,6 +115,7 @@
     if (!ctx || !value) return fail(ctx, PFV_ERR_BAD_ARG, "pfv_ctx_get_option: bad argument");
     switch (option) {
     case PFV_OPT_ENC_TRANSFORM: *value = ctx->opt_enc_transform; return PFV_OK;
+    case PFV_OPT_DEC_TRANSFORM: *value = ctx->opt_dec_transform; return PFV_OK;
     case PFV_OPT_TILE_COMPACTION: *value = ctx->opt_tile_compaction; return PFV_OK;
     case PFV_OPT_LANE_MAPPING: *value = ctx->opt_lane_mapping; return PFV_OK;
     case PFV_OPT_ENTROPY_DECODE: *value = ctx->opt_entropy_decode; return PFV_OK;
diff --git a/pretty-fast-video_amd/csrc/pfv_kernels.hip b/pretty-fast-video_amd/csrc/pfv_kernels.hip
--- a/pretty-fast-video_amd/csrc/pfv_kernels.hip
+++ b/pretty-fast-video_amd/csrc/pfv_kernels.hip
@@ -412,15 +412,18 @@
     }
     wave_lds_sync();
 }
-__device__ __forceinline__ void inverse_half(int (&v)[2][8], int *xw, int m, int i, const LaneQ &lq)
-{
-    int *mb = xw + m * kMBPitch;
+__device__ __forceinline__ void dequant_half(int (&v)[2][8], const LaneQ &lq)
+{
 #pragma unroll
     for (int k = 0; k < 8; k++) {
         const int deq = lq.deq(k);
         v[0][k] = wmul24(v[0][k], deq);
         v[1][k] = wmul24(v[1][k], deq);
     }
+}
+__device__ __forceinline__ void inverse_transform_half(int (&v)[2][8], int *xw, int m, int i)
+{
+    int *mb = xw + m * kMBPitch;
     idct8(v[0]);
     idct8(v[1]);
     cols_to_rows2(v, mb, i, m & 3);
@@ -430,6 +433,11 @@
 #pragma unroll
         for (int k = 0; k < 8; k++) v[s][k] = min(v[s][k] >> 8, 127);
     }
+}
+__device__ __forceinline__ void inverse_half(int (&v)[2][8], int *xw, int m, int i, const LaneQ &lq)
+{
+    dequant_half(v, lq);
+    inverse_transform_half(v, xw, m, i);
 }
 __device__ __forceinline__ void gather_half(int (&v)[2][8], const int *xw, int m, const LaneQ &lq)
 {
@@ -566,17 +574,22 @@
 constexpr float kPixelBias = 127.501953125f;
 __device__ __forceinline__ f2 iframe_pixel_f(f2 x) { return x * f2s(1.0f / 256.0f) + f2s(kPixelBias); }
 template <bool PIXEL>
-__device__ __forceinline__ void inverse_half_f(f2 (&c)[8], int *xw, int m, int i, const LaneQ &lq)
+__device__ __forceinline__ void inverse_transform_half_f(f2 (&c)[8], int *xw, int m, int i)
 {
     int *mb = xw + m * kMBPitch;
-#pragma unroll
-    for (int k = 0; k < 8; k++) c[k] = c[k] * f2s(lq.deqf(k));
     fidct8(c);
     f_cols_to_rows(c, mb, i, m & 3);
     fidct8(c);
 #pragma unroll
     for (int k = 0; k < 8; k++) c[k] = PIXEL ? iframe_pixel_f(c[k]) : f2floor(c[k] * f2s(1.0f / 256.0f));
 }
+template <bool PIXEL>
+__device__ __forceinline__ void inverse_half_f(f2 (&c)[8], int *xw, int m, int i, const LaneQ &lq)
+{
+#pragma unroll
+    for (int k = 0; k < 8; k++) c[k] = c[k] * f2s(lq.deqf(k));
+    inverse_transform_half_f<PIXEL>(c, xw, m, i);
+}
 __device__ __forceinline__ uint4 pack_row_f(const f2 (&px)[8])
 {
     unsigned w[4] = {0, 0, 0, 0};
@@ -594,6 +607,25 @@
         px[k] = f2{(float)byte_of(row.x, k), (float)byte_of(row.z, k)};
         px[k + 4] = f2{(float)byte_of(row.y, k), (float)byte_of(row.w, k)};
     }
+}
+
+constexpr int kDecFloatGuard = 146673;
+static_assert(14641LL * kDecFloatGuard + 256LL * (121 + 16) < 256LL * (1 << 23) && 14641LL * (kDecFloatGuard + 1) + 256LL * (121 + 16) >= 256LL * (1 << 23),
+              "kDecFloatGuard is the largest T with R (R T + s) + s < 2^23, R = 121/16, s = 16");
+__device__ __forceinline__ bool dec_float_guard(const int (&v)[2][8], bool live)
+{
+    int hi = v[0][0], lo = v[0][0];
+#pragma unroll
+    for (int k = 1; k < 16; k++) {
+        hi = max(hi, v[k >> 3][k & 7]);
+        lo = min(lo, v[k >> 3][k & 7]);
+    }
+    return !__any(live && (hi > kDecFloatGuard || lo < -kDecFloatGuard));
+}
+__device__ __forceinline__ void dequantised_to_f(const int (&v)[2][8], f2 (&c)[8])
+{
+#pragma unroll
+    for (int k = 0; k < 8; k++) c[k] = f2{(float)v[0][k], (float)v[1][k]};
 }
 
 template <bool FLT, int LPM = 8>
@@ -988,6 +1020,13 @@
 #else
     (void)r;
 #endif
+}
+__device__ __forceinline__ int opaque_int(int x)
+{
+#ifndef PFV_HIPEMU
+    asm volatile("" : "+v"(x));
+#endif
+    return x;
 }
 template <bool FLT, bool REUNPACK = false, class Store>
 __device__ __forceinline__ uint4 penc_half(const uint4 &srow, const uint4 &prow, int *xw, int m, int i, const LaneQ &lq, float qmagic, bool want_recon,
@@ -1565,10 +1604,24 @@
     }
 }
 
-template <int LPM = 8, bool LISTS = false>
-__global__ __launch_bounds__(kThreads) void k_dec_iframe(FrameGeom g, const int16_t *__restrict__ coef, CoefLists cl,
+constexpr int kDecIWaves = 7, kDecPWaves = 6;
+__device__ __forceinline__ uint8_t *dec_row_ptr(uint8_t *strip, int lane_offset) { return strip + (unsigned)opaque_int(lane_offset); }
+__device__ __forceinline__ uint8_t *wave_uniform(uint8_t *p)
+{
+    const uintptr_t a = (uintptr_t)p;
+    const unsigned lo = (unsigned)__builtin_amdgcn_readfirstlane((int)(unsigned)a), hi = (unsigned)__builtin_amdgcn_readfirstlane((int)(unsigned)(a >> 32));
+    return (uint8_t *)(((uintptr_t)hi << 32) | lo);
+}
+#ifdef PFV_HIPEMU
+#define PFV_DEC_WAVES_PER_EU(flt, n)
+#else
+#define PFV_DEC_WAVES_PER_EU(flt, n) __attribute__((amdgpu_waves_per_eu((flt) ? (n) : 1, (flt) ? (n) : 8)))
+#endif
+
+template <int LPM = 8, bool LISTS = false, bool FLT = false>
+__global__ __launch_bounds__(kThreads) PFV_DEC_WAVES_PER_EU(FLT, kDecIWaves) void k_dec_iframe(FrameGeom g, const int16_t *__restrict__ coef, CoefLists cl,
                                                           uint8_t *__restrict__ out, const QTab *__restrict__ qtabs,
-                                                          uint8_t *__restrict__ frames_out)
+                                                          uint8_t *__restrict__ frames_out, int *__restrict__ int_path_waves)
 {
     __shared__ __attribute__((aligned(16))) int xchg[kStripsPerWG][kXchgDwords];
     __shared__ __attribute__((aligned(16))) int qtab_lds[kStripsPerWG][kQTabDwords];
@@ -1581,6 +1634,8 @@
     const StripPos sp = locate_strip(g, gstrip);
     if (half_strip * 4 >= sp.n_mb) return;
     const PlaneGeom &p = g.p[sp.plane];
+    const int pw_u = FLT ? __builtin_amdgcn_readfirstlane(p.pw) : 0;
+    const auto pw = [&]() { return FLT ? pw_u : p.pw; };
     const int slot = lane >> 3, i = lane & 7;
     const int m = LPM == 8 ? slot : half_strip * 4 + (slot >> 1);
     int *xw = xchg[wave];
@@ -1601,36 +1656,62 @@
     }
     fill_qtable<false>(qtab_lds[wave], qtabs + p.qsel, lane);
     wave_lds_sync();
-    const LaneQ lq{qtab_lds[wave], i};
-    uint8_t *dst = out + (long)sp.stream * g.pad_frame_bytes + p.pad_off + (long)(sp.y0 + i) * p.pw + sp.x0 + m * 16;
+    uint8_t *dst = FLT ? nullptr : out + (long)sp.stream * g.pad_frame_bytes + p.pad_off + (long)(sp.y0 + i) * pw() + sp.x0 + m * 16;
+    uint8_t *out_strip = FLT ? wave_uniform(out + (long)sp.stream * g.pad_frame_bytes + p.pad_off + (long)sp.y0 * pw() + sp.x0) : nullptr;
+    bool int_pass = false;
 #pragma unroll
     for (int pass = 0; pass < kPasses; pass++) {
         const int h = LPM == 8 ? pass : (slot & 1);
-        if (LISTS) stage_list_half<LPM>(xw, span, lane, sp.mb_first + half_strip * 4, pass);
-        else stage_coef_half(xw, cbuf[pass], lane);
+        int ip = i, slotp = slot, lanep = lane;
+        if (FLT && pass) {
+            ip = opaque_int(i); slotp = opaque_int(slot); lanep = opaque_int(lane);
+            if (LISTS) { span.e0 = (uint32_t)opaque_int((int)span.e0); span.e1 = (uint32_t)opaque_int((int)span.e1); }
+        }
+        if (LISTS) stage_list_half<LPM>(xw, span, lanep, sp.mb_first + half_strip * 4, pass);
+        else stage_coef_half(xw, cbuf[pass], lanep);
         wave_lds_sync();
         int v[2][8];
-        gather_half(v, xw, slot, lq);
-        inverse_half(v, xw, slot, i, lq);
-#pragma unroll
-        for (int s = 0; s < 2; s++)
-#pragma unroll
-            for (int k = 0; k < 8; k++) v[s][k] = min(max(v[s][k] + 128, 0), 255);
-        if (m < sp.n_mb) {
-            const uint4 o = pack_row(v);
-            *reinterpret_cast<uint4 *>(dst + (long)(8 * h) * p.pw) = o;
+        const LaneQ lq{qtab_lds[wave], ip};
+        gather_half(v, xw, slotp, lq);
+        dequant_half(v, lq);
+        uint4 o;
+        if (FLT && dec_float_guard(v, true)) {
+            f2 c[8];
+            dequantised_to_f(v, c);
+            inverse_transform_half_f<true>(c, xw, slotp, ip);
+            o = pack_row_f(c);
+        } else {
+            int_pass = FLT;
+            if (FLT) inverse_transform_half(v, xw, opaque_int(slot), opaque_int(i));
+            else inverse_transform_half(v, xw, slot, i);
+#pragma unroll
+            for (int s = 0; s < 2; s++)
+#pragma unroll
+                for (int k = 0; k < 8; k++) v[s][k] = min(max(v[s][k] + 128, 0), 255);
+            o = pack_row(v);
+        }
+        int is = i, hs = h, ms = m;
+        if (FLT) {
+            const int l = opaque_int(lane);
+            is = l & 7;
+            hs = LPM == 8 ? pass : ((l >> 3) & 1);
+            ms = LPM == 8 ? l >> 3 : half_strip * 4 + (l >> 4);
+        }
+        if (ms < sp.n_mb) {
+            *reinterpret_cast<uint4 *>(FLT ? dec_row_ptr(out_strip, (is + 8 * hs) * pw() + ms * 16) : dst + (long)(8 * h) * pw()) = o;
             if (frames_out)
-                store_cropped16(frames_out + (long)sp.stream * g.src_frame_bytes + p.src_off, p, sp.x0 + m * 16, sp.y0 + i + 8 * h, o);
-        }
-    }
-}
-
-template <int LPM = 8, bool LISTS = false>
-__global__ __launch_bounds__(kThreads) void k_dec_pframe(FrameGeom g, const int8_t *__restrict__ mv,
+                store_cropped16(frames_out + (long)sp.stream * g.src_frame_bytes + p.src_off, p, sp.x0 + ms * 16, sp.y0 + is + 8 * hs, o);
+        }
+    }
+    if (FLT && int_pass && int_path_waves && lane == 0) atomicAdd(int_path_waves, 1);
+}
+
+template <int LPM = 8, bool LISTS = false, bool FLT = false>
+__global__ __launch_bounds__(kThreads) PFV_DEC_WAVES_PER_EU(FLT, kDecPWaves) void k_dec_pframe(FrameGeom g, const int8_t *__restrict__ mv,
                                                           const uint8_t *__restrict__ has, const int16_t *__restrict__ coef, CoefLists cl,
                                                           const uint8_t *__restrict__ ref, uint8_t *__restrict__ out,
                                                           const QTab *__restrict__ qtabs, int *__restrict__ err_flag,
-                                                          uint8_t *__restrict__ frames_out)
+                                                          uint8_t *__restrict__ frames_out, int *__restrict__ int_path_waves)
 {
     __shared__ __attribute__((aligned(16))) int xchg[kStripsPerWG][kXchgDwords];
     __shared__ __attribute__((aligned(16))) int qtab_lds[kStripsPerWG][kQTabDwords];
@@ -1643,6 +1724,8 @@
     const StripPos sp = locate_strip(g, gstrip);
     if (half_strip * 4 >= sp.n_mb) return;
     const PlaneGeom &p = g.p[sp.plane];
+    const int pw_u = FLT ? __builtin_amdgcn_readfirstlane(p.pw) : 0;
+    const auto pw = [&]() { return FLT ? pw_u : p.pw; };
     const int slot = lane >> 3, i = lane & 7;
     const int m = LPM == 8 ? slot : half_strip * 4 + (slot >> 1);
     int *xw = xchg[wave];
@@ -1664,7 +1747,7 @@
     const int mbx = sp.x0 + m * 16, mby = sp.y0;
     if (mb_valid) {
         int sx = mbx + mx, sy = mby + my;
-        if (sx < 0 || sx > p.pw - 16 || sy < 0 || sy > p.ph - 16) {
+        if (sx < 0 || sx > pw() - 16 || sy < 0 || sy > p.ph - 16) {
             if (i == 0) atomicOr(err_flag + sp.stream, 1);
             mx = 0; my = 0;
         }
@@ -1687,44 +1770,73 @@
 #pragma unroll
     for (int pass = 0; pass < kPasses; pass++) patch[pass] = make_uint4(0, 0, 0, 0);
     if (mb_valid) {
-        const uint8_t *rp = ref + (long)sp.stream * g.pad_frame_bytes + p.pad_off + (long)(mby + my + i) * p.pw + (mbx + mx);
-#pragma unroll
-        for (int pass = 0; pass < kPasses; pass++) patch[pass] = load_unaligned16(rp + 8 * (long)(LPM == 8 ? pass : (slot & 1)) * p.pw);
-    }
-    uint8_t *dst = out + (long)sp.stream * g.pad_frame_bytes + p.pad_off + (long)(sp.y0 + i) * p.pw + mbx;
+        const uint8_t *rp = ref + (long)sp.stream * g.pad_frame_bytes + p.pad_off + (long)(mby + my + i) * pw() + (mbx + mx);
+#pragma unroll
+        for (int pass = 0; pass < kPasses; pass++) patch[pass] = load_unaligned16(rp + 8 * (long)(LPM == 8 ? pass : (slot & 1)) * pw());
+    }
+    uint8_t *dst = FLT ? nullptr : out + (long)sp.stream * g.pad_frame_bytes + p.pad_off + (long)(sp.y0 + i) * pw() + mbx;
+    uint8_t *out_strip = FLT ? wave_uniform(out + (long)sp.stream * g.pad_frame_bytes + p.pad_off + (long)sp.y0 * pw() + sp.x0) : nullptr;
     uint8_t *crop = frames_out ? frames_out + (long)sp.stream * g.src_frame_bytes + p.src_off : nullptr;
 
     if (any_coded) {
         wave_lds_sync();
-        const LaneQ lq{qtab_lds[wave], i};
+        bool int_pass = false;
 #pragma unroll
         for (int pass = 0; pass < kPasses; pass++) {
             const int h = LPM == 8 ? pass : (slot & 1);
-            if (LISTS) stage_list_half<LPM>(xw, span, lane, sp.mb_first + half_strip * 4, pass);
-            else stage_coef_half(xw, cbuf[pass], lane);
+            int ip = i, slotp = slot, lanep = lane;
+            if (FLT && pass) {
+                ip = opaque_int(i); slotp = opaque_int(slot); lanep = opaque_int(lane);
+                if (LISTS) { span.e0 = (uint32_t)opaque_int((int)span.e0); span.e1 = (uint32_t)opaque_int((int)span.e1); }
+            }
+            if (LISTS) stage_list_half<LPM>(xw, span, lanep, sp.mb_first + half_strip * 4, pass);
+            else stage_coef_half(xw, cbuf[pass], lanep);
             wave_lds_sync();
-            int v[2][8], pp[2][8];
-            const int codedmask = coded ? -1 : 0;
-            gather_half(v, xw, slot, lq);
-            inverse_half(v, xw, slot, i, lq);
-            unpack_row(patch[pass], pp);
-#pragma unroll
-            for (int s = 0; s < 2; s++)
-#pragma unroll
-                for (int k = 0; k < 8; k++)
-                    pp[s][k] = min(max(pp[s][k] + 2 * (v[s][k] & codedmask), 0), 255);
+            int v[2][8];
+            const LaneQ lq{qtab_lds[wave], ip};
+            gather_half(v, xw, slotp, lq);
+            dequant_half(v, lq);
+            uint4 o;
+            if (FLT && dec_float_guard(v, coded)) {
+                f2 c[8], pp[8];
+                dequantised_to_f(v, c);
+                inverse_transform_half_f<false>(c, xw, slotp, ip);
+                uint4 prow = patch[pass];
+                opaque_row(prow);
+                unpack_row_f(prow, pp);
+                const f2 twice = f2s((float)opaque_int(coded ? 2 : 0));
+#pragma unroll
+                for (int k = 0; k < 8; k++) {
+                    const f2 t = f2{__builtin_fminf(c[k][0], 127.0f), __builtin_fminf(c[k][1], 127.0f)};
+                    pp[k] = pp[k] + t * twice;
+                }
+                o = pack_row_f(pp);
+            } else {
+                int_pass = FLT;
+                int pp[2][8];
+                const int codedmask = coded ? -1 : 0;
+                if (FLT) inverse_transform_half(v, xw, opaque_int(slot), opaque_int(i));
+                else inverse_transform_half(v, xw, slot, i);
+                unpack_row(patch[pass], pp);
+#pragma unroll
+                for (int s = 0; s < 2; s++)
+#pragma unroll
+                    for (int k = 0; k < 8; k++)
+                        pp[s][k] = min(max(pp[s][k] + 2 * (v[s][k] & codedmask), 0), 255);
+                o = pack_row(pp);
+            }
             if (mb_valid) {
-                const uint4 o = pack_row(pp);
-                *reinterpret_cast<uint4 *>(dst + (long)(8 * h) * p.pw) = o;
-                if (crop) store_cropped16(crop, p, mbx, sp.y0 + i + 8 * h, o);
-            }
-        }
+                *reinterpret_cast<uint4 *>(FLT ? dec_row_ptr(out_strip, (i + 8 * h) * pw() + m * 16) : dst + (long)(8 * h) * pw()) = o;
+                if (crop) store_cropped16(crop, p, FLT ? sp.x0 + opaque_int(m) * 16 : mbx, sp.y0 + i + 8 * h, o);
+            }
+        }
+        if (FLT && int_pass && int_path_waves && lane == 0) atomicAdd(int_path_waves, 1);
     } else if (mb_valid) {
 #pragma unroll
         for (int pass = 0; pass < kPasses; pass++) {
             const int h = LPM == 8 ? pass : (slot & 1);
-            *reinterpret_cast<uint4 *>(dst + (long)(8 * h) * p.pw) = patch[pass];
-            if (crop) store_cropped16(crop, p, mbx, sp.y0 + i + 8 * h, patch[pass]);
+            *reinterpret_cast<uint4 *>(FLT ? dec_row_ptr(out_strip, (i + 8 * h) * pw() + m * 16) : dst + (long)(8 * h) * pw()) = patch[pass];
+            if (crop) store_cropped16(crop, p, FLT ? sp.x0 + opaque_int(m) * 16 : mbx, sp.y0 + i + 8 * h, patch[pass]);
         }
     }
 }
diff --git a/pretty-fast-video_amd/csrc/pfv_launch.hip b/pretty-fast-video_amd/csrc/pfv_launch.hip
--- a/pretty-fast-video_amd/csrc/pfv_launch.hip
+++ b/pretty-fast-video_amd/csrc/pfv_launch.hip
@@ -200,28 +200,52 @@
         return c;
     }
 };
-static void launch_dec_iframe(pfv_ctx *ctx, bool small, const FrameGeom &g, const DecCoefs &c, uint8_t *out, const QTab *qt, uint8_t *frames_out)
-{
-    const dim3 grid(small ? half_strip_blocks(g) : strip_blocks(g)), block(kThreads);
+template <int LPM, bool LISTS>
+static void launch_dec_iframe_as(pfv_ctx *ctx, bool flt, dim3 grid, const FrameGeom &g, const DecCoefs &c, uint8_t *out, const QTab *qt, uint8_t *frames_out,
+                                 int *int_path_waves)
+{
+    if (flt) hipLaunchKernelGGL((k_dec_iframe<LPM, LISTS, true>), grid, dim3(kThreads), 0, ctx->stream, g, c.dense, c.lists, out, qt, frames_out, int_path_waves);
+    else hipLaunchKernelGGL((k_dec_iframe<LPM, LISTS, false>), grid, dim3(kThreads), 0, ctx->stream, g, c.dense, c.lists, out, qt, frames_out, (int *)nullptr);
+}
+static void launch_dec_iframe(pfv_ctx *ctx, bool flt, bool small, const FrameGeom &g, const DecCoefs &c, uint8_t *out, const QTab *qt, uint8_t *frames_out,
+                              int *int_path_waves = nullptr)
+{
+    const dim3 grid(small ? half_strip_blocks(g) : strip_blocks(g));
     if (c.is_lists()) {
-        if (small) hipLaunchKernelGGL((k_dec_iframe<16, true>), grid, block, 0, ctx->stream, g, c.dense, c.lists, out, qt, frames_out);
-        else hipLaunchKernelGGL((k_dec_iframe<8, true>), grid, block, 0, ctx->stream, g, c.dense, c.lists, out, qt, frames_out);
+        if (small) launch_dec_iframe_as<16, true>(ctx, flt, grid, g, c, out, qt, frames_out, int_path_waves);
+        else launch_dec_iframe_as<8, true>(ctx, flt, grid, g, c, out, qt, frames_out, int_path_waves);
     } else {
-        if (small) hipLaunchKernelGGL((k_dec_iframe<16, false>), grid, block, 0, ctx->stream, g, c.dense, c.lists, out, qt, frames_out);
-        else hipLaunchKernelGGL((k_dec_iframe<8, false>), grid, block, 0, ctx->stream, g, c.dense, c.lists, out, qt, frames_out);
-    }
-}
-static void launch_dec_pframe(pfv_ctx *ctx, bool small, const FrameGeom &g, const int8_t *mv, const uint8_t *has, const DecCoefs &c, const uint8_t *ref,
-                              uint8_t *out, const QTab *qt, int *flag, uint8_t *frames_out)
-{
-    const dim3 grid(small ? half_strip_blocks(g) : strip_blocks(g)), block(kThreads);
+        if (small) launch_dec_iframe_as<16, false>(ctx, flt, grid, g, c, out, qt, frames_out, int_path_waves);
+        else launch_dec_iframe_as<8, false>(ctx, flt, grid, g, c, out, qt, frames_out, int_path_waves);
+    }
+}
+template <int LPM, bool LISTS>
+static void launch_dec_pframe_as(pfv_ctx *ctx, bool flt, dim3 grid, const FrameGeom &g, const int8_t *mv, const uint8_t *has, const DecCoefs &c, const uint8_t *ref,
+                                 uint8_t *out, const QTab *qt, int *flag, uint8_t *frames_out, int *int_path_waves)
+{
+    if (flt) hipLaunchKernelGGL((k_dec_pframe<LPM, LISTS, true>), grid, dim3(kThreads), 0, ctx->stream, g, mv, has, c.dense, c.lists, ref, out, qt, flag, frames_out, int_path_waves);
+    else hipLaunchKernelGGL((k_dec_pframe<LPM, LISTS, false>), grid, dim3(kThreads), 0, ctx->stream, g, mv, has, c.dense, c.lists, ref, out, qt, flag, frames_out, (int *)nullptr);
+}
+static void launch_dec_pframe(pfv_ctx *ctx, bool flt, bool small, const FrameGeom &g, const int8_t *mv, const uint8_t *has, const DecCoefs &c, const uint8_t *ref,
+                              uint8_t *out, const QTab *qt, int *flag, uint8_t *frames_out, int *int_path_waves = nullptr)
+{
+    const dim3 grid(small ? half_strip_blocks(g) : strip_blocks(g));
     if (c.is_lists()) {
-        if (small) hipLaunchKernelGGL((k_dec_pframe<16, true>), grid, block, 0, ctx->stream, g, mv, has, c.dense, c.lists, ref, out, qt, flag, frames_out);
-        else hipLaunchKernelGGL((k_dec_pframe<8, true>), grid, block, 0, ctx->stream, g, mv, has, c.dense, c.lists, ref, out, qt, flag, frames_out);
+        if (small) launch_dec_pframe_as<16, true>(ctx, flt, grid, g, mv, has, c, ref, out, qt, flag, frames_out, int_path_waves);
+        else launch_dec_pframe_as<8, true>(ctx, flt, grid, g, mv, has, c, ref, out, qt, flag, frames_out, int_path_waves);
     } else {
-        if (small) hipLaunchKernelGGL((k_dec_pframe<16, false>), grid, block, 0, ctx->stream, g, mv, has, c.dense, c.lists, ref, out, qt, flag, frames_out);
-        else hipLaunchKernelGGL((k_dec_pframe<8, false>), grid, block, 0, ctx->stream, g, mv, has, c.dense, c.lists, ref, out, qt, flag, frames_out);
-    }
+        if (small) launch_dec_pframe_as<16, false>(ctx, flt, grid, g, mv, has, c, ref, out, qt, flag, frames_out, int_path_waves);
+        else launch_dec_pframe_as<8, false>(ctx, flt, grid, g, mv, has, c, ref, out, qt, flag, frames_out, int_path_waves);
+    }
+}
+static long dec_launch_waves(bool small, const FrameGeom &g)
+{
+    long per_frame = 0;
+    for (int i = 0; i < g.n_planes; i++) {
+        const PlaneGeom &p = g.p[i];
+        per_frame += (long)p.bh * (small ? (p.bw + 3) / 4 : p.strips_x);
+    }
+    return per_frame * g.n_streams;
 }
 
 static int launch_check(pfv_ctx *ctx, const char *what)
diff --git a/pretty-fast-video_amd/csrc/pfv_plane_ops.hip b/pretty-fast-video_amd/csrc/pfv_plane_ops.hip
--- a/pretty-fast-video_amd/csrc/pfv_plane_ops.hip
+++ b/pretty-fast-video_amd/csrc/pfv_plane_ops.hip
@@ -70,7 +70,7 @@
     if ((rc = ensure_scratch(ctx, 1, coef_bytes, &d_coef))) return rc;
     if ((rc = ensure_scratch(ctx, 5, pad_bytes, &d_out))) return rc;
     HIP_TRY(ctx, hipMemcpyAsync(d_coef, coef, coef_bytes, hipMemcpyHostToDevice, ctx->stream));
-    launch_dec_iframe(ctx, use_small_grid(ctx->opt_lane_mapping, g), g, (const int16_t *)d_coef, (uint8_t *)d_out, ctx->qtab_dev, nullptr);
+    launch_dec_iframe(ctx, ctx->opt_dec_transform != PFV_DEC_TRANSFORM_INT, use_small_grid(ctx->opt_lane_mapping, g), g, (const int16_t *)d_coef, (uint8_t *)d_out, ctx->qtab_dev, nullptr);
     if ((rc = launch_check(ctx, "k_dec_iframe"))) return rc;
     HIP_TRY(ctx, hipMemcpyAsync(target, d_out, pad_bytes, hipMemcpyDeviceToHost, ctx->stream));
     HIP_TRY(ctx, hipStreamSynchronize(ctx->stream));
@@ -100,7 +100,7 @@
     HIP_TRY(ctx, hipMemcpyAsync(d_mv, mv, n * 2, hipMemcpyHostToDevice, ctx->stream));
     HIP_TRY(ctx, hipMemcpyAsync(d_has, has_coef, n, hipMemcpyHostToDevice, ctx->stream));
     HIP_TRY(ctx, hipMemsetAsync(ctx->flag_dev, 0, sizeof(int), ctx->stream));
-    launch_dec_pframe(ctx, use_small_grid(ctx->opt_lane_mapping, g), g, (const int8_t *)d_mv, (const uint8_t *)d_has, (const int16_t *)d_coef, (const uint8_t *)d_ref,
+    launch_dec_pframe(ctx, ctx->opt_dec_transform != PFV_DEC_TRANSFORM_INT, use_small_grid(ctx->opt_lane_mapping, g), g, (const int8_t *)d_mv, (const uint8_t *)d_has, (const int16_t *)d_coef, (const uint8_t *)d_ref,
                       (uint8_t *)d_out, ctx->qtab_dev, ctx->flag_dev, nullptr);
     if ((rc = launch_check(ctx, "k_dec_pframe"))) return rc;
     int flag = 0;
diff --git a/pretty-fast-video_amd/csrc/pfv_sessions.hip b/pretty-fast-video_amd/csrc/pfv_sessions.hip
--- a/pretty-fast-video_amd/csrc/pfv_sessions.hip
+++ b/pretty-fast-video_amd/csrc/pfv_sessions.hip
@@ -130,6 +130,9 @@
     QTab *qtab_dev = nullptr;
     uint8_t *fb[2] = {nullptr, nullptr};
     int lane_mapping = PFV_LANES_AUTO;
+    bool flt = true;
+    int *path_dev = nullptr;
+    long path_total = 0;
     int cur = 0;
     int *flag_dev = nullptr;
     std::vector<int> flags_host;
@@ -719,6 +722,7 @@
     s->ctx = ctx; s->width = width; s->height = height; s->n_streams = n_streams; s->n_qtables = n_qtables;
     s->win_count = n_streams;
     s->lane_mapping = ctx->opt_lane_mapping;
+    s->flt = ctx->opt_dec_transform != PFV_DEC_TRANSFORM_INT;
     s->geom = frame_geom(width, height, n_streams);
     s->db_table.resize((size_t)n_dev);
     for (int i = 0; i < n_dev; i++) s->db_table[(size_t)i] = (uint8_t)pfv_deblock_strength(qtables + (size_t)i * 64);
@@ -746,7 +750,7 @@
     if (!s) return;
     (void)hipSetDevice(s->ctx->device);
     (void)hipStreamSynchronize(s->ctx->stream);
-    void *bufs[] = {s->qtab_dev, s->fb[0], s->fb[1], s->flag_dev, s->st_coef, s->st_mv, s->st_has, s->st_frames, s->st_idx, s->st_val, s->q_map, s->ssim_map, s->db_scratch, s->st_rgb};
+    void *bufs[] = {s->qtab_dev, s->fb[0], s->fb[1], s->flag_dev, s->st_coef, s->st_mv, s->st_has, s->st_frames, s->st_idx, s->st_val, s->q_map, s->ssim_map, s->db_scratch, s->st_rgb, s->path_dev};
     for (void *b : bufs)
         if (b) (void)hipFree(b);
     delete s;
@@ -773,6 +777,35 @@
     if (!s) return fail(nullptr, PFV_ERR_BAD_ARG, "null session");
     if (first < 0 || count <= 0 || first > s->n_streams - count) return fail(s->ctx, PFV_ERR_BAD_ARG, "pfv_dec_session_set_window: window outside [0, n_streams)");
     s->win_first = first; s->win_count = count;
+    return PFV_OK;
+}
+PFV_API int pfv_dec_session_enable_path_stats(pfv_dec_session *s, int on)
+{
+    if (!s) return fail(nullptr, PFV_ERR_BAD_ARG, "null session");
+    pfv_ctx *ctx = s->ctx;
+    HIP_TRY(ctx, hipSetDevice(ctx->device));
+    HIP_TRY(ctx, hipStreamSynchronize(ctx->stream));
+    if (!on) {
+        if (s->path_dev) HIP_TRY(ctx, hipFree(s->path_dev));
+        s->path_dev = nullptr;
+        return PFV_OK;
+    }
+    if (!s->path_dev) HIP_TRY(ctx, hipMalloc((void **)&s->path_dev, sizeof(int)));
+    HIP_TRY(ctx, hipMemset(s->path_dev, 0, sizeof(int)));
+    s->path_total = 0;
+    return PFV_OK;
+}
+PFV_API int pfv_dec_session_path_stats(pfv_dec_session *s, int64_t *int_waves, int64_t *total_waves)
+{
+    if (!s || !int_waves || !total_waves) return fail(s ? s->ctx : nullptr, PFV_ERR_BAD_ARG, "pfv_dec_session_path_stats: bad argument");
+    pfv_ctx *ctx = s->ctx;
+    if (!s->path_dev) return fail(ctx, PFV_ERR_STATE, "pfv_dec_session_path_stats: not enabled (pfv_dec_session_enable_path_stats)");
+    HIP_TRY(ctx, hipSetDevice(ctx->device));
+    HIP_TRY(ctx, hipStreamSynchronize(ctx->stream));
+    int n = 0;
+    HIP_TRY(ctx, hipMemcpy(&n, s->path_dev, sizeof(int), hipMemcpyDeviceToHost));
+    *int_waves = n;
+    *total_waves = s->path_total;
     return PFV_OK;
 }
 static bool dec_full_window(const pfv_dec_session *s) { return s->win_first == 0 && s->win_count == s->n_streams && s->out_stride == 0; }
@@ -820,12 +853,14 @@
     g = dec_out_geom(s, g, s->frames_out);
     g.n_streams = count;
     const int nxt = s->cur ^ 1;
+    const bool small = use_small_grid(s->lane_mapping, g);
+    if (s->path_dev) s->path_total += dec_launch_waves(small, g);
     if (pframe) {
-        launch_dec_pframe(ctx, use_small_grid(s->lane_mapping, g), g, mv_dev + mb0 * 2, has_dev + mb0, coefs.shifted((size_t)first, (size_t)s->geom.mbs_per_frame),
-                          s->fb[s->cur] + pad0, s->fb[nxt] + pad0, s->qtab_dev, s->flag_dev + first, crop);
+        launch_dec_pframe(ctx, s->flt, small, g, mv_dev + mb0 * 2, has_dev + mb0, coefs.shifted((size_t)first, (size_t)s->geom.mbs_per_frame),
+                          s->fb[s->cur] + pad0, s->fb[nxt] + pad0, s->qtab_dev, s->flag_dev + first, crop, s->path_dev);
         rc = launch_check(ctx, "k_dec_pframe");
     } else {
-        launch_dec_iframe(ctx, use_small_grid(s->lane_mapping, g), g, coefs.shifted((size_t)first, (size_t)s->geom.mbs_per_frame), s->fb[nxt] + pad0, s->qtab_dev, crop);
+        launch_dec_iframe(ctx, s->flt, small, g, coefs.shifted((size_t)first, (size_t)s->geom.mbs_per_frame), s->fb[nxt] + pad0, s->qtab_dev, crop, s->path_dev);
         rc = launch_check(ctx, "k_dec_iframe");
     }
     return rc;
diff --git a/pretty-fast-video_amd/session.py b/pretty-fast-video_amd/session.py
--- a/pretty-fast-video_amd/session.py
+++ b/pretty-fast-video_amd/session.py
@@ -379,6 +379,14 @@
     def check(self):
         self.ctx.check(self.ctx._lib.pfv_dec_check(self.handle))
 
+    def enable_path_stats(self, on: bool = True):
+        self.ctx.check(self.ctx._lib.pfv_dec_session_enable_path_stats(self.handle, 1 if on else 0))
+
+    def path_stats(self):
+        a, b = ctypes.c_int64(0), ctypes.c_int64(0)
+        self.ctx.check(self.ctx._lib.pfv_dec_session_path_stats(self.handle, ctypes.byref(a), ctypes.byref(b)))
+        return int(a.value), int(b.value)
+
     def get_frame(self) -> np.ndarray:
         out = np.empty((self.n_streams, self.frame_bytes), dtype=np.uint8)
         self.ctx.check(self.ctx._lib.pfv_dec_get_frame(self.handle, ptr(out)))
```

Result: faster. 1.455 billion, median of 6 (+2.0%).
